# regicide211212/multi-style-transfer-gan

Hardware: AMD Instinct MI355X
Metric: train-step images/sec (fwd+bwd+loss), 256x256 batch32 (higher is better)
Workload: dtype f32; 1 GPU; config 3: reference CycleGAN train_step (2x EnhancedGenerator + 2x EnhancedDiscriminator, channels=16, num_transformer_blocks=0), 32 image pairs/GPU at 256x256, fwd+bwd+loss+Adam; per_gpu_batch=32, size=256, channels=16, parallelism=dp1, collective=none, losses_finite=True

## Files before the change

### include/mstg_hip.h

```cpp
#ifndef MSTG_HIP_H
#define MSTG_HIP_H

#include <stddef.h>
#include <stdint.h>

#ifdef __cplusplus
extern "C" {
#endif

#define MSTG_OK 0
#define MSTG_E_BADARG (-1)
#define MSTG_E_ALIGN (-2)
#define MSTG_E_LAUNCH (-3)
#define MSTG_E_WORKSPACE (-4)
#define MSTG_E_UNSUPPORTED (-5)

#define MSTG_ACT_NONE 0
#define MSTG_ACT_RELU 1
#define MSTG_ACT_LEAKY02 2
#define MSTG_ACT_TANH 3
#define MSTG_ACT_GELU 4

const char* mstg_version(void);
const char* mstg_arch(void);
const char* mstg_last_error(void);
void mstg_env_refresh(void);

int mstg_prof_enable(int on);
int mstg_prof_count(void);
int mstg_prof_get(int i, char* name, size_t name_cap, float* ms);

typedef struct mstg_conv_desc {
    int32_t N, H, W, Cin;
    int32_t Ho, Wo, Cout;
    int32_t KH, KW, stride, pad, dil;
    int32_t transposed;
    int32_t x_nchw, y_nchw;
    int32_t x_ctot, x_coff;
    int32_t y_ctot, y_coff;
    int32_t act;
    int32_t accumulate;
} mstg_conv_desc;

int mstg_conv2d_dgrad_bsums_supported(const mstg_conv_desc* d);
size_t mstg_conv2d_dgrad_bsums_workspace_bytes(const mstg_conv_desc* d);
int mstg_conv2d_dgrad_bsums(const mstg_conv_desc* d, const float* dy, const float* w, float* dx, const float* x_raw, const float* x_stats,
                            float* sums, void* workspace, size_t workspace_bytes, int workspace_packed, void* stream);

int mstg_conv2d_fwd_cached(const mstg_conv_desc* d, const float* x, const float* w, const float* bias, float* y, void* workspace,
                           size_t workspace_bytes, int workspace_packed, void* stream);
int mstg_conv2d_fwd_norm_cached(const mstg_conv_desc* d, const float* x, const float* in_stats, const float* w, const float* bias,
                                float* y, float* out_stats, void* workspace, size_t workspace_bytes, int workspace_packed, void* stream);
int mstg_conv2d_dgrad_cached(const mstg_conv_desc* d, const float* dy, const float* w, float* dx, void* workspace, size_t workspace_bytes,
                             int workspace_packed, void* stream);
int mstg_msblock_fwd_cached(const float* x, const float* w1, const float* b1, const float* w2, const float* b2, const float* w3,
                            const float* b3, const float* w4, const float* b4, float* y, int N, int H, int W, int CH, void* workspace,
                            size_t workspace_bytes, int workspace_packed, void* stream);
int mstg_msblock_dgrad_cached(const float* dy, const float* w1, const float* w2, const float* w3, const float* w4, const float* dres,
                              float* dx, int N, int H, int W, int CH, void* workspace, size_t workspace_bytes, int workspace_packed,
                              void* stream);

const char* mstg_conv2d_kernel_name(const mstg_conv_desc* d, int pass);
size_t mstg_conv2d_workspace_bytes(const mstg_conv_desc* d);
int mstg_conv2d_fwd(const mstg_conv_desc* d, const float* x, const float* w, const float* bias ,
                    float* y, void* workspace, size_t workspace_bytes, void* stream);
int mstg_conv2d_wgrad_norm_supported(const mstg_conv_desc* d);
int mstg_conv2d_wgrad_norm(const mstg_conv_desc* d, const float* x_raw, const float* in_stats, const float* dy, float* dw, float* dbias,
                           void* workspace, size_t workspace_bytes, void* stream);
int mstg_conv2d_fwd_norm_supported(const mstg_conv_desc* d);
int mstg_conv2d_fwd_stats_pays(const mstg_conv_desc* d);
size_t mstg_conv2d_fwd_norm_workspace_bytes(const mstg_conv_desc* d);
int mstg_conv2d_fwd_norm(const mstg_conv_desc* d, const float* x, const float* in_stats, const float* w, const float* bias, float* y,
                         float* out_stats, void* workspace, size_t workspace_bytes, void* stream);
int mstg_conv2d_dgrad(const mstg_conv_desc* d, const float* dy, const float* w, float* dx, void* workspace,
                      size_t workspace_bytes, void* stream);
size_t mstg_conv2d_wgrad_workspace_bytes(const mstg_conv_desc* d);
int mstg_conv2d_wgrad(const mstg_conv_desc* d, const float* x, const float* dy, float* dw, float* dbias ,
                      void* workspace, size_t workspace_bytes, void* stream);

size_t mstg_norm_workspace_bytes(int N, int HW, int C);
int mstg_norm_act_fwd(const float* x, const float* residual , float* y, float* stats ,
                      int N, int HW, int C, int act, int batch_stats, const float* gamma, const float* beta,
                      float* running_mean, float* running_var, void* workspace, size_t workspace_bytes, void* stream);
int mstg_norm_act_bwd(const float* x, const float* stats, const float* dy, float* dx, int N, int HW, int C, int act,
                      int batch_stats, const float* gamma, const float* beta, float* dgamma, float* dbeta,
                      void* workspace, size_t workspace_bytes, void* stream);
int mstg_norm_apply_fwd(const float* x, const float* stats, const float* residual , float* y, int N, int HW, int C, int act,
                        void* stream);
int mstg_norm_stats(const float* x, float* stats, int N, int HW, int C, void* workspace, size_t workspace_bytes, void* stream);
int mstg_norm_bwd_apply(const float* x, const float* stats, const float* dy, const float* sums ,
                        int sums_split, float* dx, int N, int HW, int C, int act, void* stream);

int mstg_window_attn_core_fwd(const float* qkv, float* o, int N, int H, int W, int C, void* stream);
int mstg_window_attn_core_bwd(const float* qkv, const float* d_o, float* dqkv, int N, int H, int W, int C, void* stream);

int mstg_window_attn_ws_supported(int C, int ws);
int mstg_window_attn_ws_fwd(const float* qkv, float* o, int N, int H, int W, int C, int ws, void* stream);
int mstg_window_attn_ws_bwd(const float* qkv, const float* d_o, float* dqkv, int N, int H, int W, int C, int ws, void* stream);

int mstg_window_attn_fused_supported(int C);
int mstg_window_attn_fwd(const float* x, const float* wqkv, const float* bqkv, const float* wproj, const float* bproj,
                         float* y, int N, int H, int W, int C, void* stream);
int mstg_window_attn_bwd_direct(const float* x, const float* wqkv, const float* bqkv, const float* wproj, const float* bproj, const float* dy,
                                float* dx, float* dwqkv, float* dbqkv, float* dwproj, float* dbproj, int accumulate, int N, int H, int W, int C,
                                void* workspace, size_t workspace_bytes, void* stream);
int mstg_window_attn_norm_bwd_direct(const float* x_raw, const float* in_stats, const float* wqkv, const float* bqkv, const float* wproj,
                                     const float* bproj, const float* dy, float* dz, float* dwqkv, float* dbqkv, float* dwproj,
                                     float* dbproj, int accumulate, float* norm_sums, int N, int H, int W, int C, void* workspace,
                                     size_t workspace_bytes, void* stream);
int mstg_window_attn_norm_sums_split(void);
int mstg_window_attn_norm_fwd(const float* x_raw, const float* in_stats, const float* wqkv, const float* bqkv, const float* wproj,
                              const float* bproj, float* y, int N, int H, int W, int C, void* stream);
size_t mstg_window_attn_norm_bwd_workspace_bytes(int N, int H, int W, int C);
int mstg_window_attn_norm_bwd(const float* x_raw, const float* in_stats, const float* wqkv, const float* bqkv, const float* wproj,
                              const float* bproj, const float* dy, float* dz, float* dparams, float* norm_sums, int N, int H, int W,
                              int C, void* workspace, size_t workspace_bytes, void* stream);
size_t mstg_window_attn_bwd_workspace_bytes(int N, int H, int W, int C);
int mstg_window_attn_bwd(const float* x, const float* wqkv, const float* bqkv, const float* wproj, const float* bproj,
                         const float* dy, float* dx, float* dparams, int N, int H, int W, int C, void* workspace,
                         size_t workspace_bytes, void* stream);

int mstg_act_fwd(const float* x, float* y, size_t n, int act, void* stream);
int mstg_act_bwd(const float* x_or_y, const float* dy, float* dx, size_t n, int act, void* stream);
size_t mstg_loss_workspace_bytes(size_t n);
int mstg_loss_mean_fwd(const float* a, const float* b, float bconst, size_t n, int kind, float* out, void* workspace,
                       size_t workspace_bytes, void* stream);
int mstg_loss_mean_bwd(const float* a, const float* b, float bconst, size_t n, int kind, const float* gscale, float scale,
                       float* da, float* db, void* stream);
int mstg_add(const float* a, const float* b, float* y, size_t n, void* stream);
int mstg_weighted_sum_fwd(const float* const* terms, const float* weights, int n, int nout, float* out, void* stream);
int mstg_weighted_sum_bwd(const float* g, const float* weights, int n, float* dterms, void* stream);
int mstg_masked_l1_mean_fwd(const float* a, const float* b, const float* m, size_t n, float* out, void* workspace,
                            size_t workspace_bytes, void* stream);
int mstg_masked_l1_mean_bwd(const float* a, const float* b, const float* m, size_t n, const float* gscale, float* da, void* stream);
int mstg_clip_grad_norm(float* g, size_t n, float max_norm, float* norm_out, void* workspace, size_t workspace_bytes, void* stream);
size_t mstg_channel_sum_workspace_bytes(size_t P, int C);
int mstg_channel_sum(const float* x, size_t P, int ctot, int coff, int C, float scale, float* out, void* workspace,
                     size_t workspace_bytes, void* stream);
size_t mstg_plane_sum_workspace_bytes(int N, int C, size_t HW);
int mstg_plane_sum(const float* x, int N, int C, size_t HW, float scale, float* out, void* workspace,
                   size_t workspace_bytes, void* stream);
int mstg_segment_mean_fwd(const float* x, int S, size_t P, int C, float* out, void* stream);
int mstg_segment_mean_bwd(const float* dy, int S, size_t P, int C, float* dx, void* stream);
int mstg_adam_step_flat(float* p, const float* g, float* m, float* v, size_t n, float lr, float beta1, float beta2,
                        float eps, int step, const unsigned char* mask , void* stream);

int mstg_msblock_fused_supported(int CH);
size_t mstg_msblock_fwd_workspace_bytes(int CH);
int mstg_msblock_fwd(const float* x, const float* w1, const float* b1, const float* w2, const float* b2, const float* w3,
                     const float* b3, const float* w4, const float* b4, float* y, int N, int H, int W, int CH, void* workspace,
                     size_t workspace_bytes, void* stream);
size_t mstg_msblock_dgrad_workspace_bytes(int CH);
int mstg_msblock_dgrad(const float* dy, const float* w1, const float* w2, const float* w3, const float* w4, const float* dres,
                       float* dx, int N, int H, int W, int CH, void* workspace, size_t workspace_bytes, void* stream);
size_t mstg_msblock_wgrad_workspace_bytes(int N, int H, int W, int CH);
int mstg_msblock_wgrad(const float* x, const float* dy, float* dw1, float* db1, float* dw2, float* db2, float* dw3, float* db3,
                       float* dw4, float* db4, int accumulate , int N, int H, int W,
                       int CH, void* workspace, size_t workspace_bytes, void* stream);

size_t mstg_spectral_norm_workspace_bytes(int M, int K);
int mstg_spectral_norm_fwd(const float* w, float* u, float* v, float* w_out, float* sigma, float* u_save, float* v_save, int M,
                           int K, float eps, int training, void* workspace, size_t workspace_bytes, void* stream);
int mstg_spectral_norm_bwd(const float* dwn, const float* w, const float* u, const float* v, const float* sigma, float* dw,
                           int accumulate , int M, int K, void* workspace, size_t workspace_bytes, void* stream);
int mstg_spectral_norm_group_max(void);
size_t mstg_spectral_norm_group_workspace_bytes(int count, const int* M, const int* K);
int mstg_spectral_norm_group_fwd(int count, const float* const* w, float* const* u, float* const* v, float* const* w_out, float* sigma,
                                 float* const* u_save, float* const* v_save, const int* M, const int* K, float eps, int training,
                                 void* workspace, size_t workspace_bytes, void* stream);
int mstg_spectral_norm_group_bwd(int count, const float* const* dwn, const float* const* w, const float* const* u,
                                 const float* const* v, const float* const* sigma, float* const* dw, const int* accumulate, const int* M,
                                 const int* K, void* workspace, size_t workspace_bytes, void* stream);

int mstg_maxpool2x2_fwd(const float* x, float* y, unsigned char* idx, int N, int H, int W, int C, void* stream);
int mstg_maxpool2x2_bwd(const float* dy, const unsigned char* idx, float* dx, int N, int H, int W, int C, void* stream);
size_t mstg_gram_workspace_bytes(int N, int HW, int C);
int mstg_gram_fwd(const float* f, float* g, int N, int HW, int C, float scale, void* workspace, size_t workspace_bytes,
                  void* stream);
int mstg_gram_bwd(const float* f, const float* dg, float* df, int N, int HW, int C, float scale, void* stream);

typedef struct mstg_f16_conv_desc {
    int32_t kind;
    int32_t N, H, W, Cin;
    int32_t Ho, Wo, Cout;
    int32_t K, stride, pad, dil;
    int32_t src_nchw_f32;
    int32_t dst_nchw;
    int32_t act;
} mstg_f16_conv_desc;
size_t mstg_f16_conv_plan_bytes(const mstg_f16_conv_desc* d);
int mstg_f16_conv_pack(const mstg_f16_conv_desc* d, const float* w0, const float* b0, const float* w1, const float* b1,
                       const float* w2, const float* b2, const float* w3, const float* b3, void* blob, size_t blob_bytes,
                       void* stream);
size_t mstg_f16_conv_partial_bytes(const mstg_f16_conv_desc* d);
int mstg_f16_conv_fwd(const mstg_f16_conv_desc* d, const void* blob, const void* x, const float* in_stats , void* y,
                      float* out_stats , void* workspace, size_t workspace_bytes, void* stream);
int mstg_f16_conv_fwd_res(const mstg_f16_conv_desc* d, const void* blob, const void* x, const float* in_stats,
                          const void* residual , void* y, float* out_stats , void* workspace,
                          size_t workspace_bytes, void* stream);
int mstg_f16_norm_residual(const void* x, const void* residual, const float* stats, void* y, int N, int HW, int C, void* stream);
size_t mstg_f16_attn_plan_bytes(int C);
int mstg_f16_attn_pack(const float* wqkv, const float* bqkv, const float* wproj, const float* bproj, int C, void* blob,
                       size_t blob_bytes, void* stream);
int mstg_f16_attn_fwd(const void* x, const float* in_stats , const void* blob, void* y, int N, int H, int W, int C,
                      void* stream);

typedef struct mstg_f16_plain_desc {
// ... 259 lines not shown
```

### multi-style-transfer-gan_amd/mstg_hip/_lib.py

```python
from __future__ import annotations

import ctypes as C
import os

HERE = os.path.dirname(os.path.abspath(__file__))
LIB_PATH = os.environ.get("MSTG_LIB") or os.path.join(HERE, "libmstg_hip.so")

ACT_NONE, ACT_RELU, ACT_LEAKY02, ACT_TANH, ACT_GELU = 0, 1, 2, 3, 4
LOSS_L1, LOSS_MSE = 0, 1


class ConvDesc(C.Structure):
    _fields_ = [(n, C.c_int32) for n in (
        "N", "H", "W", "Cin", "Ho", "Wo", "Cout", "KH", "KW", "stride", "pad", "dil", "transposed",
        "x_nchw", "y_nchw", "x_ctot", "x_coff", "y_ctot", "y_coff", "act", "accumulate")]


class F16ConvDesc(C.Structure):
    _fields_ = [(n, C.c_int32) for n in (
        "kind", "N", "H", "W", "Cin", "Ho", "Wo", "Cout", "K", "stride", "pad", "dil", "src_nchw_f32", "dst_nchw", "act")]


class F16PlainDesc(C.Structure):
    _fields_ = [(n, C.c_int32) for n in (
        "kind", "N", "H", "W", "Cin", "Ho", "Wo", "Cout", "K", "src_nchw_f32", "dst_nchw", "act")]


class ImgDesc(C.Structure):
    _fields_ = ([("src", C.c_void_p)] + [(n, C.c_int32) for n in (
        "src_h", "src_w", "box_y", "box_x", "box_h", "box_w", "rs_h", "rs_w", "filter", "win_y", "win_x", "win_h", "win_w",
        "dst_y", "dst_x", "fill", "ks_h", "ks_v", "y_first", "irows", "ipitch")] + [(n, C.c_int64) for n in (
            "kk_h", "bounds_h", "kk_v", "bounds_v", "inter_off", "out_off")] + [("grid", C.c_uint64)])


IMG_PASS_H, IMG_PASS_V_TENSOR, IMG_PASS_V_U8 = 0, 1, 2

_vp, _fp, _sz, _i, _f = C.c_void_p, C.c_void_p, C.c_size_t, C.c_int, C.c_float
_dp = C.POINTER(ConvDesc)
_hp = C.POINTER(F16ConvDesc)
_pp = C.POINTER(F16PlainDesc)

SIGNATURES = {
    "mstg_version": (C.c_char_p, []),
    "mstg_arch": (C.c_char_p, []),
    "mstg_last_error": (C.c_char_p, []),
    "mstg_env_refresh": (None, []),
    "mstg_prof_enable": (_i, [_i]),
    "mstg_prof_count": (_i, []),
    "mstg_prof_get": (_i, [_i, C.c_char_p, _sz, C.POINTER(C.c_float)]),
    "mstg_conv2d_kernel_name": (C.c_char_p, [_dp, _i]),
    "mstg_conv2d_workspace_bytes": (_sz, [_dp]),
    "mstg_conv2d_fwd": (_i, [_dp, _fp, _fp, _fp, _fp, _vp, _sz, _vp]),
    "mstg_conv2d_dgrad": (_i, [_dp, _fp, _fp, _fp, _vp, _sz, _vp]),
    "mstg_conv2d_dgrad_bsums_supported": (_i, [_dp]),
    "mstg_conv2d_dgrad_bsums_workspace_bytes": (_sz, [_dp]),
    "mstg_conv2d_dgrad_bsums": (_i, [_dp, _fp, _fp, _fp, _fp, _fp, _fp, _vp, _sz, _i, _vp]),
    "mstg_conv2d_fwd_cached": (_i, [_dp, _fp, _fp, _fp, _fp, _vp, _sz, _i, _vp]),
    "mstg_conv2d_fwd_norm_cached": (_i, [_dp, _fp, _fp, _fp, _fp, _fp, _fp, _vp, _sz, _i, _vp]),
    "mstg_conv2d_dgrad_cached": (_i, [_dp, _fp, _fp, _fp, _vp, _sz, _i, _vp]),
    "mstg_msblock_fwd_cached": (_i, [_fp] * 10 + [_i, _i, _i, _i, _vp, _sz, _i, _vp]),
    "mstg_msblock_dgrad_cached": (_i, [_fp] * 7 + [_i, _i, _i, _i, _vp, _sz, _i, _vp]),
    "mstg_conv2d_wgrad_workspace_bytes": (_sz, [_dp]),
    "mstg_conv2d_wgrad": (_i, [_dp, _fp, _fp, _fp, _fp, _vp, _sz, _vp]),
    "mstg_norm_workspace_bytes": (_sz, [_i, _i, _i]),
    "mstg_norm_act_fwd": (_i, [_fp, _fp, _fp, _fp, _i, _i, _i, _i, _i, _fp, _fp, _fp, _fp, _vp, _sz, _vp]),
    "mstg_norm_act_bwd": (_i, [_fp, _fp, _fp, _fp, _i, _i, _i, _i, _i, _fp, _fp, _fp, _fp, _vp, _sz, _vp]),
    "mstg_window_attn_core_fwd": (_i, [_fp, _fp, _i, _i, _i, _i, _vp]),
    "mstg_window_attn_core_bwd": (_i, [_fp, _fp, _fp, _i, _i, _i, _i, _vp]),
    "mstg_window_attn_ws_supported": (_i, [_i, _i]),
    "mstg_window_attn_ws_fwd": (_i, [_fp, _fp, _i, _i, _i, _i, _i, _vp]),
    "mstg_window_attn_ws_bwd": (_i, [_fp, _fp, _fp, _i, _i, _i, _i, _i, _vp]),
    "mstg_window_attn_fused_supported": (_i, [_i]),
    "mstg_window_attn_fwd": (_i, [_fp, _fp, _fp, _fp, _fp, _fp, _i, _i, _i, _i, _vp]),
    "mstg_window_attn_bwd_workspace_bytes": (_sz, [_i, _i, _i, _i]),
    "mstg_conv2d_wgrad_norm_supported": (_i, [_dp]),
    "mstg_conv2d_wgrad_norm": (_i, [_dp, _fp, _fp, _fp, _fp, _fp, _vp, _sz, _vp]),
    "mstg_conv2d_fwd_norm_supported": (_i, [_dp]),
    "mstg_conv2d_fwd_stats_pays": (_i, [_dp]),
    "mstg_conv2d_fwd_norm_workspace_bytes": (_sz, [_dp]),
    "mstg_conv2d_fwd_norm": (_i, [_dp, _fp, _fp, _fp, _fp, _fp, _fp, _vp, _sz, _vp]),
    "mstg_window_attn_norm_fwd": (_i, [_fp, _fp, _fp, _fp, _fp, _fp, _fp, _i, _i, _i, _i, _vp]),
    "mstg_window_attn_norm_bwd_workspace_bytes": (_sz, [_i, _i, _i, _i]),
    "mstg_window_attn_norm_bwd": (_i, [_fp, _fp, _fp, _fp, _fp, _fp, _fp, _fp, _fp, _fp, _i, _i, _i, _i, _vp, _sz, _vp]),
    "mstg_norm_apply_fwd": (_i, [_fp, _fp, _fp, _fp, _i, _i, _i, _i, _vp]),
    "mstg_norm_stats": (_i, [_fp, _fp, _i, _i, _i, _vp, _sz, _vp]),
    "mstg_norm_bwd_apply": (_i, [_fp, _fp, _fp, _fp, _i, _fp, _i, _i, _i, _i, _vp]),
    "mstg_window_attn_norm_sums_split": (_i, []),
    "mstg_window_attn_bwd_direct": (_i, [_fp] * 11 + [_i, _i, _i, _i, _i, _vp, _sz, _vp]),
    "mstg_window_attn_norm_bwd_direct": (_i, [_fp] * 12 + [_i, _fp, _i, _i, _i, _i, _vp, _sz, _vp]),
    "mstg_window_attn_bwd": (_i, [_fp, _fp, _fp, _fp, _fp, _fp, _fp, _fp, _i, _i, _i, _i, _vp, _sz, _vp]),
    "mstg_act_fwd": (_i, [_fp, _fp, _sz, _i, _vp]),
    "mstg_act_bwd": (_i, [_fp, _fp, _fp, _sz, _i, _vp]),
    "mstg_loss_workspace_bytes": (_sz, [_sz]),
    "mstg_loss_mean_fwd": (_i, [_fp, _fp, _f, _sz, _i, _fp, _vp, _sz, _vp]),
    "mstg_loss_mean_bwd": (_i, [_fp, _fp, _f, _sz, _i, _fp, _f, _fp, _fp, _vp]),
    "mstg_channel_sum_workspace_bytes": (_sz, [_sz, _i]),
    "mstg_channel_sum": (_i, [_fp, _sz, _i, _i, _i, _f, _fp, _vp, _sz, _vp]),
    "mstg_plane_sum_workspace_bytes": (_sz, [_i, _i, _sz]),
    "mstg_plane_sum": (_i, [_fp, _i, _i, _sz, _f, _fp, _vp, _sz, _vp]),
    "mstg_segment_mean_fwd": (_i, [_fp, _i, _sz, _i, _fp, _vp]),
    "mstg_segment_mean_bwd": (_i, [_fp, _i, _sz, _i, _fp, _vp]),
    "mstg_maxpool2x2_fwd": (_i, [_fp, _fp, _vp, _i, _i, _i, _i, _vp]),
    "mstg_maxpool2x2_bwd": (_i, [_fp, _vp, _fp, _i, _i, _i, _i, _vp]),
    "mstg_gram_workspace_bytes": (_sz, [_i, _i, _i]),
    "mstg_gram_fwd": (_i, [_fp, _fp, _i, _i, _i, _f, _vp, _sz, _vp]),
    "mstg_gram_bwd": (_i, [_fp, _fp, _fp, _i, _i, _i, _f, _vp]),
    "mstg_adam_step_flat": (_i, [_fp, _fp, _fp, _fp, _sz, _f, _f, _f, _f, _i, _vp, _vp]),
    "mstg_msblock_fused_supported": (_i, [_i]),
    "mstg_msblock_fwd_workspace_bytes": (_sz, [_i]),
    "mstg_msblock_fwd": (_i, [_fp] * 10 + [_i, _i, _i, _i, _vp, _sz, _vp]),
    "mstg_msblock_dgrad_workspace_bytes": (_sz, [_i]),
    "mstg_msblock_dgrad": (_i, [_fp] * 7 + [_i, _i, _i, _i, _vp, _sz, _vp]),
    "mstg_msblock_wgrad_workspace_bytes": (_sz, [_i, _i, _i, _i]),
    "mstg_msblock_wgrad": (_i, [_fp] * 10 + [_i, _i, _i, _i, _i, _vp, _sz, _vp]),
    "mstg_spectral_norm_workspace_bytes": (_sz, [_i, _i]),
    "mstg_spectral_norm_fwd": (_i, [_fp] * 7 + [_i, _i, _f, _i, _vp, _sz, _vp]),
    "mstg_spectral_norm_bwd": (_i, [_fp, _fp, _fp, _fp, _fp, _fp, _i, _i, _i, _vp, _sz, _vp]),
    "mstg_spectral_norm_group_max": (_i, []),
    "mstg_spectral_norm_group_workspace_bytes": (_sz, [_i, _vp, _vp]),
    "mstg_spectral_norm_group_fwd": (_i, [_i, _vp, _vp, _vp, _vp, _fp, _vp, _vp, _vp, _vp, _f, _i, _vp, _sz, _vp]),
    "mstg_spectral_norm_group_bwd": (_i, [_i, _vp, _vp, _vp, _vp, _vp, _vp, _vp, _vp, _vp, _vp, _sz, _vp]),
    "mstg_f16_conv_plan_bytes": (_sz, [_hp]),
    "mstg_f16_conv_pack": (_i, [_hp] + [_fp] * 8 + [_vp, _sz, _vp]),
    "mstg_f16_conv_partial_bytes": (_sz, [_hp]),
    "mstg_f16_conv_fwd": (_i, [_hp, _vp, _vp, _fp, _vp, _fp, _vp, _sz, _vp]),
    "mstg_f16_conv_fwd_res": (_i, [_hp, _vp, _vp, _fp, _vp, _vp, _fp, _vp, _sz, _vp]),
    "mstg_f16_norm_residual": (_i, [_vp, _vp, _fp, _vp, _i, _i, _i, _vp]),
    "mstg_f16_attn_plan_bytes": (_sz, [_i]),
    "mstg_f16_attn_pack": (_i, [_fp, _fp, _fp, _fp, _i, _vp, _sz, _vp]),
    "mstg_f16_attn_fwd": (_i, [_vp, _fp, _vp, _vp, _i, _i, _i, _i, _vp]),
    "mstg_f16_plain_plan_bytes": (_sz, [_pp]),
    "mstg_f16_plain_pack": (_i, [_pp, _fp, _fp, _fp, _vp, _sz, _vp]),
    "mstg_f16_plain_fwd": (_i, [_pp, _vp, _vp, _vp, _vp]),
    "mstg_f16_train_image_nhwc8": (_i, [_fp, _vp, _i, _i, _i, _vp]),
    "mstg_f16_train_bn_workspace_bytes": (_sz, [_sz, _i]),
    "mstg_f16_train_bn_fwd": (_i, [_vp, _fp, _fp, _sz, _i, _i, _f, _f, _fp, _fp, _fp, _fp, _vp, _vp, _sz, _vp]),
    "mstg_f16_train_bn_bwd": (_i, [_vp, _vp, _fp, _fp, _fp, _fp, _sz, _i, _i, _fp, _fp, _fp, _vp, _vp, _sz, _vp]),
    "mstg_f16_train_act_bwd": (_i, [_vp, _vp, _vp, _sz, _i, _vp]),
    "mstg_f16_train_loss_workspace_bytes": (_sz, [_i, _i, _i]),
    "mstg_f16_train_head_loss_bwd": (_i, [_vp, _fp, _fp, _i, _i, _i, _fp, _fp, _vp, _vp, _sz, _vp]),
    "mstg_f16_train_wgrad_workspace_bytes": (_sz, [_i, _i, _i, _i, _i, _i]),
    "mstg_f16_train_wgrad": (_i, [_vp, _vp, _i, _i, _i, _i, _i, _i, _fp, _fp, _vp, _sz, _vp]),
    "mstg_f16_train_bias_grad": (_i, [_vp, _sz, _i, _i, _fp, _fp, _vp, _sz, _vp]),
    "mstg_f16_train_scale_update": (_i, [_fp, _fp, _vp, _vp]),
    "mstg_f16_train_adam": (_i, [_fp, _fp, _fp, _fp, _sz, _f, _f, _f, _f, _i, _vp, _vp]),
    "mstg_f16_linear_plan_bytes": (_sz, [_i, _i]),
    "mstg_f16_linear_pack": (_i, [_fp, _fp, _i, _i, _vp, _sz, _vp]),
    "mstg_f16_linear_fwd": (_i, [_vp, _vp, _fp, _vp, _i, _i, _i, _i, _i, _i, _vp]),
    "mstg_f16_ln_mod_fwd": (_i, [_vp, _i, _fp, _fp, _fp, _fp, _fp, _fp, _fp, _vp, _i, _i, _i, _f, _vp]),
    "mstg_f16_token_mean_workspace_bytes": (_sz, [_i, _i, _i]),
    "mstg_f16_token_mean": (_i, [_vp, _fp, _i, _i, _i, _vp, _sz, _vp]),
    "mstg_f16_flash_attn_fwd": (_i, [_vp, _vp, _i, _i, _i, _i, _vp]),
    "mstg_add": (_i, [_fp, _fp, _fp, _sz, _vp]),
    "mstg_weighted_sum_fwd": (_i, [C.POINTER(C.c_void_p), C.POINTER(C.c_float), _i, _i, _fp, _vp]),
    "mstg_weighted_sum_bwd": (_i, [_fp, C.POINTER(C.c_float), _i, _fp, _vp]),
    "mstg_masked_l1_mean_fwd": (_i, [_fp, _fp, _fp, _sz, _fp, _vp, _sz, _vp]),
    "mstg_masked_l1_mean_bwd": (_i, [_fp, _fp, _fp, _sz, _fp, _fp, _vp]),
    "mstg_clip_grad_norm": (_i, [_fp, _sz, _f, _fp, _vp, _sz, _vp]),
    "mstg_structure_map": (_i, [_fp, _fp, _i, _i, _i, _vp]),
    "mstg_ln_mod_fwd": (_i, [_fp] * 7 + [_i, _i, _i, _f, _vp]),
    "mstg_ln_mod_bwd_workspace_bytes": (_sz, [_i, _i, _i]),
    "mstg_ln_mod_bwd": (_i, [_fp] * 11 + [_i, _i, _i, _i, _vp, _sz, _vp]),
    "mstg_flash_attn_fwd": (_i, [_fp, _fp, _fp, _i, _i, _i, _i, _vp]),
    "mstg_flash_attn_bwd": (_i, [_fp, _fp, _fp, _fp, _fp, _fp, _i, _i, _i, _i, _vp]),
    "mstg_resample_ksize": (_i, [_i, _i, _i]),
    "mstg_resample_coeffs": (_i, [_i, _i, _i, _vp, _vp]),
    "mstg_resample_h_u8": (_i, [_vp, _vp, _i, _i, _i, _i, _i, _vp, _vp, _vp]),
    "mstg_resample_v_u8": (_i, [_vp, _vp, _i, _i, _i, _vp, _vp, _vp]),
    "mstg_paste_u8": (_i, [_vp, _i, _i, _i, _i, _i, _i, _vp, _i, _i, _i, _i, _i, _vp]),
    "mstg_u8_to_tensor": (_i, [_vp, _i, _i, _i, _i, _i, _i, _fp, _fp, _fp, C.c_ulonglong, _i, _vp]),
    "mstg_tensor_to_u8": (_i, [_fp, _i, _i, _vp, _vp]),
    "mstg_blend_u8": (_i, [_vp, _vp, C.c_double, C.c_double, _vp, _vp, _i, _i, _vp]),
    "mstg_img_batch_validate": (_i, [_vp, _i, _vp, _sz, _sz, _i, _sz]),
    "mstg_img_batch_tiles": (_i, [_vp, _i, _vp, _sz, _i, _i, _vp, _sz]),
    "mstg_img_batch_resample_h": (_i, [_vp, _i, _vp, _sz, _vp, _vp, _i, _vp, _vp, _sz, _vp]),
    "mstg_img_batch_resample_v_tensor": (_i, [_vp, _i, _vp, _sz, _vp, _vp, _i, _vp, _vp, _sz, _i, _fp, _fp, _fp, _vp, _i, _vp]),
    "mstg_img_batch_resample_v_u8": (_i, [_vp, _i, _vp, _sz, _vp, _vp, _i, _vp, _vp, _sz, _vp, _sz, _vp]),
    "mstg_img_batch_tensor_to_u8": (_i, [_vp, _i, _i, _i, _i, _vp, _vp]),
    "mstg_image_metrics_workspace_bytes": (_sz, [_i, _i, _i]),
    "mstg_image_metrics_u8": (_i, [_vp, _vp, _i, _i, _i, _vp, _vp, _sz, _vp]),
    "mstg_local_style_workspace_bytes": (_sz, [_i, _i, _i]),
    "mstg_local_style_prepare": (_i, [_vp, _i, _i, _i, _vp, _vp, _vp, _vp, _vp]),
    "mstg_local_style_hysteresis": (_i, [_vp, _i, _i, _i, _vp, _vp]),
    "mstg_local_style_weights": (_i, [_vp, _vp, _vp, _i, _i, _i, C.c_double, C.c_double, C.c_double, _vp, _vp, _vp]),
    "mstg_local_style_weight_map": (_i, [_vp, _i, _i, _i, C.c_double, C.c_double, C.c_double, _vp, _vp, _sz, _vp]),
    "mstg_local_style_finish": (_i, [_vp, _vp, _vp, _vp, _i, _i, _i, _i, _i, _vp, _vp]),
    "mstg_local_style_enhanced_workspace_bytes": (_sz, [_i, _i, _i]),
    "mstg_local_style_enhanced": (_i, [_vp, _vp, _i, _i, _i, C.c_double, C.c_double, C.c_double, _i, _i, _vp, _vp, _sz, _vp]),
    "mstg_bilateral_tables": (_i, [_i, C.c_double, C.c_double, _vp]),
    "mstg_standard_color_lut": (_i, [_i, _vp]),
    "mstg_median3_u8": (_i, [_vp, _i, _i, _i, _vp, _vp]),
    "mstg_bilateral_u8": (_i, [_vp, _i, _i, _i, _i, _vp, _vp, _vp]),
    "mstg_lut_u8": (_i, [_vp, _i, _i, _i, _vp, _vp, _vp]),
    "mstg_gaussian_u8": (_i, [_vp, _i, _i, _i, _i, _vp, _vp]),
    "mstg_standard_finish_workspace_bytes": (_sz, [_i, _i, _i]),
    "mstg_standard_finish": (_i, [_vp, _vp, _i, _i, _i, C.c_double, C.c_double, _i, _i, _vp, _vp, _i, _vp, _vp, _sz, _vp]),
    "mstg_gaussian_kernel_f64": (_i, [_i, C.c_double, _vp]),
    "mstg_app_sky_mask": (_i, [_vp, _i, _i, _i, _vp, _vp]),
    "mstg_app_edge_weight": (_i, [_vp, _i, _i, _i, _vp, C.c_double, _vp, _vp]),
    "mstg_app_chain": (_i, [_vp, _vp, _i, _i, _i, _vp, _vp, _i, C.c_double, C.c_double, _vp, _vp, _vp]),
    "mstg_app_local_style_workspace_bytes": (_sz, [_i, _i, _i]),
    "mstg_app_local_style_finish": (_i, [_vp, _vp, _i, _i, _i, _i, _i, _i, _i, C.c_double, C.c_double, C.c_double, _vp, _vp, _vp, _vp, _vp,
                                         _sz, _vp]),
    "mstg_lab_tables": (_i, [_vp]),
    "mstg_bilateral_wide_tables": (_i, [_i, C.c_double, C.c_double, _vp]),
    "mstg_color_block_mask": (_i, [_vp, _i, _i, _i, _vp, _f, _i, _vp, _vp, _sz, _vp]),
    "mstg_color_correct_u8": (_i, [_vp, _vp, _i, _i, _i, _i, _vp, _vp, _sz, _vp]),
    "mstg_bilateral_wide_u8": (_i, [_vp, _i, _i, _i, _i, _vp, _vp, _vp]),
    "mstg_detail_blend_u8": (_i, [_vp, _vp, _i, _i, _i, _vp, _i, C.c_double, C.c_double, C.c_double, _vp, _vp, _sz, _vp]),
    "mstg_color_block_fix_workspace_bytes": (_sz, [_i, _i, _i, _i]),
    "mstg_color_block_fix": (_i, [_vp, _vp, _i, _i, _i, _vp, _f, _i, _i, _i, _vp, _vp, _i, C.c_double, C.c_double, C.c_double, _vp, _vp,
                                  _sz, _vp]),
# ... 78 lines not shown
```

### multi-style-transfer-gan_amd/mstg_hip/csrc/conv_igemm.hip

```cpp
#include "common.h"
#include "igemm_args.h"
#include <stdlib.h>

namespace mstg {


constexpr int TILE_H = 8, TILE_W = 16;

#ifdef MSTG_STAMPS
__device__ unsigned long long g_dbg_stamps[64 * 8];
#define MSTG_STAMP(k)                                                                                      \
    if (threadIdx.x == 0 && (blockIdx.x % 11) == 0 && blockIdx.x / 11 < 64 && blockIdx.y == 0 && blockIdx.z == 0) \
        g_dbg_stamps[(blockIdx.x / 11) * 8 + (k)] = __builtin_amdgcn_s_memtime();
#else
#define MSTG_STAMP(k)
#endif
constexpr int W_BUDGET_FLOATS = 6144;

template <int V> struct Frag;
template <> struct Frag<1> { typedef float T; };
template <> struct Frag<2> { typedef f32x2 T; };
template <> struct Frag<4> { typedef f32x4 T; };
template <int V> __device__ __forceinline__ float frag_get(const typename Frag<V>::T& f, int j);
template <> __device__ __forceinline__ float frag_get<1>(const float& f, int) { return f; }
template <> __device__ __forceinline__ float frag_get<2>(const f32x2& f, int j) { return f[j]; }
template <> __device__ __forceinline__ float frag_get<4>(const f32x4& f, int j) { return f[j]; }

template <int V> __host__ __device__ constexpr int ckp_of() { return V == 4 ? 20 : (V == 2 ? 12 : 4); }
template <int V> __host__ __device__ constexpr int ckp_heavy_of() { return V == 4 ? 24 : ckp_of<V>(); }

__global__ void pack_filter_kernel(const IGemmArgs a, float* __restrict__ wp, int CK, int CoP, int nchunks, int ncls) {
    const int total = ncls * nchunks * a.ntaps * CoP * CK;
    for (int idx = blockIdx.x * blockDim.x + threadIdx.x; idx < total; idx += gridDim.x * blockDim.x) {
        const int ci = idx % CK;
        int rest = idx / CK;
        const int co = rest % CoP; rest /= CoP;
        const int t = rest % a.ntaps; rest /= a.ntaps;
        const int chunk = rest % nchunks, cls = rest / nchunks;
        int widx, oc = co;
        bool ok = true;
        if (a.phase) {
            const int pa = cls >> 1, pb = cls & 1, u = t >> 1, v = t & 1;
            widx = ((1 - pa) + 2 * u) * 4 + ((1 - pb) + 2 * v);
        } else if (a.dpack) {
            const int delta = co >> 2, kx = 4 * (t % a.tapsx) + 3 - delta, real = (t / a.tapsx) * a.KW + kx;
            oc = co & 3;
            ok = co < 16 && kx >= 0 && kx < a.KW;
            widx = a.flip ? (a.KH * a.KW - 1 - real) : real;
        } else {
            widx = a.flip ? (a.ntaps - 1 - t) : t;
        }
        const int cr = chunk * CK + ci;
        wp[idx] = (ok && oc < a.Co && cr < a.Cr) ? a.w[(size_t)oc * a.w_so + (size_t)cr * a.w_sr + widx] : 0.f;
    }
}

__device__ __forceinline__ int tap_patch_offset(const IGemmArgs& a, int t, int pa, int pb, int ckp) {
    int pro, pco;
    if (a.phase) {
        pro = 1 + pa - (t >> 1);
        pco = 1 + pb - (t & 1);
    } else if (a.dpack) {
        pro = t / a.tapsx;
        pco = 4 * (t % a.tapsx) + 3;
    } else {
        pro = (t / a.KW) * a.dil;
        pco = (t % a.KW) * a.dil;
    }
    return (pro * a.PW + pco) * ckp;
}

template <int NFW, int PF = 2>
__device__ __forceinline__ void igemm_epilogue(const IGemmArgs& a, const f32x4 (&acc)[NFW][PF], int n, int ty0, int tx0, int co0, int pa,
                                               int pb, int wave, int i, int g) {
#pragma unroll
    for (int pf = 0; pf < PF; ++pf) {
        const int gy = ty0 * (4 * PF) + PF * wave + pf, gx = tx0 * TILE_W + i;
        if (gy >= a.Gh || gx >= a.Gw) continue;
        const int oy = a.phase ? 2 * gy + pa : gy, ox = a.phase ? 2 * gx + pb : gx;
#pragma unroll
        for (int wf = 0; wf < NFW; ++wf) {
            const int co = co0 + 16 * wf + 4 * g;
            if (co >= a.Co) continue;
            f32x4 v = acc[wf][pf];
            if (!a.y_nchw && co + 3 < a.Co && ((a.y_ctot | a.y_coff) & 3) == 0) {
                float* p = a.y + (((size_t)n * a.Ho + oy) * a.Wo + ox) * a.y_ctot + a.y_coff + co;
                if (a.bias) v += *reinterpret_cast<const f32x4*>(a.bias + co);
                if (a.accumulate) v += *reinterpret_cast<const f32x4*>(p);
                if (a.act != MSTG_ACT_NONE) {
#pragma unroll
                    for (int e = 0; e < 4; ++e) v[e] = apply_act(v[e], a.act);
                }
                *reinterpret_cast<f32x4*>(p) = v;
            } else {
#pragma unroll
                for (int e = 0; e < 4; ++e) {
                    if (co + e >= a.Co) continue;
                    float* p = a.y_nchw ? a.y + (((size_t)n * a.y_ctot + a.y_coff + co + e) * a.Ho + oy) * a.Wo + ox
                                        : a.y + (((size_t)n * a.Ho + oy) * a.Wo + ox) * a.y_ctot + a.y_coff + co + e;
                    float val = v[e] + (a.bias ? a.bias[co + e] : 0.f);
                    if (a.accumulate) val += *p;
                    *p = apply_act(val, a.act);
                }
            }
        }
    }
}

template <int V, int NFW, int PF>
__global__ __launch_bounds__(256) void igemm_light_kernel(const IGemmArgs a, const float* __restrict__ wp, const int CoP) {
    constexpr int CK = 4 * V, CKP = ckp_of<V>(), BN = 16 * NFW, TH = 4 * PF;
    typedef typename Frag<V>::T frag_t;
    extern __shared__ __attribute__((aligned(16))) float smem[];
    float* patch = smem;
    float* wl = smem + ((a.PH * a.PW * CKP + 3) & ~3);
    int* tapo = reinterpret_cast<int*>(wl + (a.wglob ? 0 : a.TG * BN * CKP));

    const int tid = threadIdx.x, lane = tid & 63, wave = tid >> 6, i = lane & 15, g = lane >> 4;
    const int tile = xcd_swizzle(blockIdx.x, gridDim.x);
    const int tx0 = tile % a.tiles_x, ty0 = (tile / a.tiles_x) % a.tiles_y, n = tile / (a.tiles_x * a.tiles_y);
    const int co0 = blockIdx.y * BN;
    const int cls = blockIdx.z, pa = cls >> 1, pb = cls & 1;
    const int s = a.phase ? 1 : a.stride;
    const int y0 = a.phase ? ty0 * TH - 1 : ty0 * TH * s - a.pad;
    const int x0 = a.phase ? tx0 * TILE_W - 1 : (a.dpack ? tx0 * 13 - 3 - a.pad : tx0 * TILE_W * s - a.pad);
    const int nchunks = (a.Cr + CK - 1) / CK;
    const unsigned m_pw = magic_u32(a.PW);
    MSTG_STAMP(0)
    if (tid < a.ntaps) tapo[tid] = tap_patch_offset(a, tid, pa, pb, CKP);

    f32x4 acc[NFW][PF];
#pragma unroll
    for (int wf = 0; wf < NFW; ++wf)
#pragma unroll
        for (int pf = 0; pf < PF; ++pf) acc[wf][pf] = f32x4{0.f, 0.f, 0.f, 0.f};

    for (int chunk = 0; chunk < nchunks; ++chunk) {
        if (chunk) __syncthreads();
        if (a.x_nchw) {
            stage_window_c4(a.x + ((size_t)n * a.x_ctot + a.x_coff) * a.H * a.W, patch, a.PH, a.PW, m_pw, y0, x0, a.H, a.W, (unsigned)a.W, 1u,
                            (unsigned)(a.H * a.W), a.Cr, tid);
        } else if (((a.x_ctot | a.x_coff | a.Cr) & 3) == 0) {
            stage_window(a.x + (size_t)n * a.H * a.W * a.x_ctot + a.x_coff + chunk * CK, patch, a.PH, a.PW, V, m_pw, 0xFFFFFFFFu / V + 1u, y0,
                         x0, a.H, a.W, a.x_ctot, min(V, (a.Cr - chunk * CK) >> 2), CKP, tid);
        } else {
            for (int pr = wave; pr < a.PH; pr += 4) {
                const int iy = y0 + pr;
                for (int e = lane; e < a.PW * V; e += 64) {
                    const int pc = e / V, q = e % V;
                    const int ix = x0 + pc;
                    const bool inb = (unsigned)iy < (unsigned)a.H && (unsigned)ix < (unsigned)a.W;
                    f32x4 v = {0.f, 0.f, 0.f, 0.f};
                    const int c0 = chunk * CK + 4 * q;
                    if (inb && c0 < a.Cr) {
                        const float* src = a.x + (((size_t)n * a.H + iy) * a.W + ix) * a.x_ctot + a.x_coff + c0;
#pragma unroll
                        for (int c = 0; c < 4; ++c)
                            if (c0 + c < a.Cr) v[c] = src[c];
                    }
                    *reinterpret_cast<f32x4*>(&patch[(pr * a.PW + pc) * CKP + 4 * q]) = v;
                }
            }
        }
        MSTG_STAMP(1)
        if (a.wglob) {
            __syncthreads();
            const float* wb = wp + ((size_t)((cls * nchunks + chunk) * a.ntaps) * CoP + co0 + i) * CK + V * g;
            const int wts = CoP * CK;
            const int bbase0 = ((PF * wave) * s * a.PW + i * s) * CKP + V * g, bstep = s * a.PW * CKP;
            frag_t a0[NFW], a1[NFW], a2[NFW], bf[PF], bfn[PF];
#pragma unroll
            for (int wf = 0; wf < NFW; ++wf) {
                a0[wf] = *reinterpret_cast<const frag_t*>(wb + 16 * wf * CK);
                a1[wf] = *reinterpret_cast<const frag_t*>(wb + min(1, a.ntaps - 1) * wts + 16 * wf * CK);
            }
            {
                const int po = tapo[0];
#pragma unroll
                for (int pf = 0; pf < PF; ++pf) bf[pf] = *reinterpret_cast<const frag_t*>(&patch[bbase0 + pf * bstep + po]);
            }
            for (int tl = 0; tl < a.ntaps; ++tl) {
                const int t2 = min(tl + 2, a.ntaps - 1), t1 = min(tl + 1, a.ntaps - 1);
#pragma unroll
                for (int wf = 0; wf < NFW; ++wf) a2[wf] = *reinterpret_cast<const frag_t*>(wb + t2 * wts + 16 * wf * CK);
                const int po = tapo[t1];
#pragma unroll
                for (int pf = 0; pf < PF; ++pf) bfn[pf] = *reinterpret_cast<const frag_t*>(&patch[bbase0 + pf * bstep + po]);
#pragma unroll
                for (int j = 0; j < V; ++j)
#pragma unroll
                    for (int wf = 0; wf < NFW; ++wf)
#pragma unroll
                        for (int pf = 0; pf < PF; ++pf)
                            acc[wf][pf] = mfma16(frag_get<V>(a0[wf], j), frag_get<V>(bf[pf], j), acc[wf][pf]);
#pragma unroll
                for (int wf = 0; wf < NFW; ++wf) { a0[wf] = a1[wf]; a1[wf] = a2[wf]; }
#pragma unroll
                for (int pf = 0; pf < PF; ++pf) bf[pf] = bfn[pf];
            }
            continue;
        }
        for (int t0 = 0; t0 < a.ntaps; t0 += a.TG) {
            __syncthreads();
            MSTG_STAMP(2)
            const int tn = min(a.TG, a.ntaps - t0);
            const float* base = wp + ((size_t)((cls * nchunks + chunk) * a.ntaps + t0) * CoP + co0) * CK;
            for (int e0 = 0; e0 < tn * BN * V; e0 += 1024) {
                f32x4 wv[4];
#pragma unroll
                for (int k = 0; k < 4; ++k) {
                    const int e = min(e0 + 256 * k + tid, tn * BN * V - 1);
                    const int row = e / V, q = e % V, tl = row / BN, col = row % BN;
                    wv[k] = *reinterpret_cast<const f32x4*>(base + (unsigned)((tl * CoP + col) * CK + 4 * q));
                }
#pragma unroll
                for (int k = 0; k < 4; ++k) {
                    const int e = e0 + 256 * k + tid;
                    if (e < tn * BN * V) *reinterpret_cast<f32x4*>(&wl[(e / V) * CKP + 4 * (e % V)]) = wv[k];
                }
            }
            MSTG_STAMP(3)
            __syncthreads();
            MSTG_STAMP(4)
            const int bbase0 = ((PF * wave) * s * a.PW + i * s) * CKP + V * g, bstep = s * a.PW * CKP;
            frag_t af[NFW], bf[PF], afn[NFW], bfn[PF];
            {
                const int po = tapo[t0];
#pragma unroll
                for (int wf = 0; wf < NFW; ++wf) af[wf] = *reinterpret_cast<const frag_t*>(&wl[(16 * wf + i) * CKP + V * g]);
#pragma unroll
                for (int pf = 0; pf < PF; ++pf) bf[pf] = *reinterpret_cast<const frag_t*>(&patch[bbase0 + pf * bstep + po]);
            }
            for (int tl = 0; tl < ((a.dbg & 1) ? 1 : tn); ++tl) {
                const int tnx = min(tl + 1, tn - 1);
                const int po = tapo[t0 + tnx];
#pragma unroll
                for (int wf = 0; wf < NFW; ++wf) afn[wf] = *reinterpret_cast<const frag_t*>(&wl[(tnx * BN + 16 * wf + i) * CKP + V * g]);
#pragma unroll
                for (int pf = 0; pf < PF; ++pf) bfn[pf] = *reinterpret_cast<const frag_t*>(&patch[bbase0 + pf * bstep + po]);
#pragma unroll
                for (int j = 0; j < V; ++j)
#pragma unroll
                    for (int wf = 0; wf < NFW; ++wf)
#pragma unroll
                        for (int pf = 0; pf < PF; ++pf)
                            acc[wf][pf] = mfma16(frag_get<V>(af[wf], j), frag_get<V>(bf[pf], j), acc[wf][pf]);
#pragma unroll
                for (int wf = 0; wf < NFW; ++wf) af[wf] = afn[wf];
#pragma unroll
                for (int pf = 0; pf < PF; ++pf) bf[pf] = bfn[pf];
            }
        }
    }
    MSTG_STAMP(5)
    if (!a.dpack) {
        igemm_epilogue<NFW, PF>(a, acc, n, ty0, tx0, co0, pa, pb, wave, i, g);
        MSTG_STAMP(6)
        return;
    }
    __syncthreads();
    float* comb = smem + wave * (256 * PF);
#pragma unroll
    for (int pf = 0; pf < PF; ++pf) *reinterpret_cast<f32x4*>(&comb[((pf * 4 + g) * 16 + i) * 4]) = acc[0][pf];
    __syncthreads();
    if (g < PF && i < 13) {
        const int pf = g;
        f32x4 v = {0.f, 0.f, 0.f, 0.f};
#pragma unroll
        for (int d = 0; d < 4; ++d) v += *reinterpret_cast<const f32x4*>(&comb[((pf * 4 + d) * 16 + i + 3 - d) * 4]);
        const int oy = ty0 * TH + PF * wave + pf, ox = tx0 * 13 + i;
        if (oy < a.Gh && ox < a.Gw) {
            if (!a.y_nchw && a.Co == 4 && ((a.y_ctot | a.y_coff) & 3) == 0) {
                float* p = a.y + (((size_t)n * a.Ho + oy) * a.Wo + ox) * a.y_ctot + a.y_coff;
                if (a.bias) v += *reinterpret_cast<const f32x4*>(a.bias);
                if (a.accumulate) v += *reinterpret_cast<const f32x4*>(p);
#pragma unroll
                for (int e = 0; e < 4; ++e) v[e] = apply_act(v[e], a.act);
                *reinterpret_cast<f32x4*>(p) = v;
            } else {
#pragma unroll
                for (int e = 0; e < 4; ++e) {
                    if (e >= a.Co) continue;
                    float* p = a.y_nchw ? a.y + (((size_t)n * a.y_ctot + a.y_coff + e) * a.Ho + oy) * a.Wo + ox
                                        : a.y + (((size_t)n * a.Ho + oy) * a.Wo + ox) * a.y_ctot + a.y_coff + e;
                    float val = v[e] + (a.bias ? a.bias[e] : 0.f);
                    if (a.accumulate) val += *p;
                    *p = apply_act(val, a.act);
                }
            }
        }
    }
    MSTG_STAMP(6)
}

constexpr int SNB = 8;

template <int V, int NFW, int PF, int SRC>
__global__ __launch_bounds__(256) void igemm_stream_kernel(const IGemmArgs a, const float* __restrict__ wp, const int CoP) {
    constexpr int CK = 4 * V, CKP = ckp_of<V>(), BN = 16 * NFW, TH = 4 * PF;
    typedef typename Frag<V>::T frag_t;
    extern __shared__ __attribute__((aligned(16))) float smem[];
    const int nchunks = (a.Cr + CK - 1) / CK;
    const int wsz = nchunks * a.ntaps * BN * CKP;
    float* patch = smem;
    float* wl = smem + a.psz;
    int* tapo = reinterpret_cast<int*>(wl + wsz);

    const int tid = threadIdx.x, lane = tid & 63, wave = tid >> 6, i = lane & 15, g = lane >> 4;
    const int co0 = blockIdx.y * BN;
    const int cls = blockIdx.z, pa = cls >> 1, pb = cls & 1;
    const int s = a.phase ? 1 : a.stride;
    const int ntiles = a.N * a.tiles_x * a.tiles_y;
    const int my_tiles = ((int)blockIdx.x < ntiles) ? (ntiles - 1 - (int)blockIdx.x) / (int)gridDim.x + 1 : 0;
    const int total = my_tiles * nchunks;
    if (total == 0) return;

    if (tid < a.ntaps) tapo[tid] = tap_patch_offset(a, tid, pa, pb, CKP);
    {
        const int nrow = nchunks * a.ntaps * BN;
        const float* base = wp + (size_t)cls * nchunks * a.ntaps * CoP * CK + (size_t)co0 * CK;
        for (int e0 = 0; e0 < nrow * V; e0 += 1024) {
            f32x4 wv[4];
#pragma unroll
            for (int k = 0; k < 4; ++k) {
                const int e = min(e0 + 256 * k + tid, nrow * V - 1);
                const int row = e / V, q = e % V, ct = row / BN, col = row % BN;
                wv[k] = *reinterpret_cast<const f32x4*>(base + (unsigned)((ct * CoP + col) * CK + 4 * q));
            }
#pragma unroll
            for (int k = 0; k < 4; ++k) {
                const int e = e0 + 256 * k + tid;
                if (e < nrow * V) *reinterpret_cast<f32x4*>(&wl[(e / V) * CKP + 4 * (e % V)]) = wv[k];
            }
        }
    }
    const int npatch = a.PH * a.PW * V;
    const unsigned m_pw = magic_u32(a.PW);
    int p_lds[SNB], p_rc[SNB];
    unsigned p_off[SNB], used = 0;
#pragma unroll
    for (int j = 0; j < SNB; ++j) {
        const int e = tid + 256 * j;
        const int pp = e / V, q = e % V;
        const int r = (int)__umulhi((unsigned)pp, m_pw), c = pp - r * a.PW;
        const bool u = e < npatch;
        p_lds[j] = u ? pp * CKP + 4 * q : -1;
        p_rc[j] = r | (c << 8) | (q << 16);
        p_off[j] = !u ? 0u : (SRC == 2 ? (unsigned)(r * a.W + c) : (unsigned)(r * a.W + c) * (unsigned)a.x_ctot + 4u * q);
        used |= u ? (1u << j) : 0u;
    }
    const unsigned plane = (unsigned)(a.H * a.W);
    f32x4 breg[NFW];
    unsigned cok = 0;
#pragma unroll
    for (int wf = 0; wf < NFW; ++wf) {
        const int co = a.dpack ? 0 : co0 + 16 * wf + 4 * g;
#pragma unroll
        for (int e = 0; e < 4; ++e) breg[wf][e] = (a.bias && co + e < a.Co) ? a.bias[co + e] : 0.f;
        cok |= (co + 3 < a.Co) ? (1u << wf) : 0u;
    }
    const bool yvec = !a.y_nchw && ((a.y_ctot | a.y_coff) & 3) == 0;
    const int yrs = a.phase ? 2 * a.Wo : a.Wo, ycs = a.phase ? 2 : 1;
    const unsigned y_lane = (unsigned)((PF * wave) * yrs + i * ycs) * (unsigned)a.y_ctot + 4u * g;

    auto tile_of = [&](int seq, int& tx0, int& ty0, int& n) {
        const int tile = xcd_swizzle((int)blockIdx.x + seq * (int)gridDim.x, ntiles);
        tx0 = tile % a.tiles_x;
        ty0 = (tile / a.tiles_x) % a.tiles_y;
        n = tile / (a.tiles_x * a.tiles_y);
    };
    f32x4 preg[SNB];
    unsigned pmask = 0;
    auto load_stage = [&](int seq, int chunk) {
        int tx0, ty0, n;
        tile_of(seq, tx0, ty0, n);
        const int y0 = a.phase ? ty0 * TH - 1 : ty0 * TH * s - a.pad;
        const int x0 = a.phase ? tx0 * TILE_W - 1 : (a.dpack ? tx0 * 13 - 3 - a.pad : tx0 * TILE_W * s - a.pad);
        pmask = 0;
        const bool interior = y0 >= 0 && x0 >= 0 && y0 + a.PH <= a.H && x0 + a.PW <= a.W;
        if (interior && SRC == 2) {
            const float* base = a.x + ((size_t)n * a.x_ctot + a.x_coff) * plane + (unsigned)(y0 * a.W + x0);
            pmask = used;
#pragma unroll
            for (int j = 0; j < SNB; ++j) {
#pragma unroll
                for (int ch = 0; ch < 4; ++ch) preg[j][ch] = base[p_off[j] + (ch < a.Cr ? ch * plane : 0u)];
            }
        } else if (interior && SRC == 0 && (a.Cr - chunk * CK) >= CK) {
            const float* base = a.x + ((size_t)n * plane + (unsigned)(y0 * a.W + x0)) * a.x_ctot + a.x_coff + chunk * CK;
            pmask = used;
#pragma unroll
            for (int j = 0; j < SNB; ++j) preg[j] = *reinterpret_cast<const f32x4*>(base + p_off[j]);
        } else if (SRC == 2) {
            const float* img = a.x + ((size_t)n * a.x_ctot + a.x_coff) * plane;
#pragma unroll
            for (int j = 0; j < SNB; ++j) {
                const int iy = y0 + (p_rc[j] & 255), ix = x0 + ((p_rc[j] >> 8) & 255);
                const bool ok = p_lds[j] >= 0 && (unsigned)iy < (unsigned)a.H && (unsigned)ix < (unsigned)a.W;
                const unsigned off = ok ? (unsigned)(iy * a.W + ix) : 0u;
                pmask |= ok ? (1u << j) : 0u;
#pragma unroll
                for (int ch = 0; ch < 4; ++ch) preg[j][ch] = img[off + (ch < a.Cr ? ch * plane : 0u)];
            }
        } else {
            const float* img = a.x + (size_t)n * plane * a.x_ctot + a.x_coff + chunk * CK;
            const int nqv = min(V, (a.Cr - chunk * CK) >> 2);
#pragma unroll
            for (int j = 0; j < SNB; ++j) {
                const int iy = y0 + (p_rc[j] & 255), ix = x0 + ((p_rc[j] >> 8) & 255), q = p_rc[j] >> 16;
                const bool ok = p_lds[j] >= 0 && (unsigned)iy < (unsigned)a.H && (unsigned)ix < (unsigned)a.W && q < nqv;
                const unsigned off = ok ? (unsigned)(iy * a.W + ix) * (unsigned)a.x_ctot + 4u * q : 0u;
                pmask |= ok ? (1u << j) : 0u;
                preg[j] = *reinterpret_cast<const f32x4*>(img + off);
            }
        }
    };
    auto store_stage = [&]() {
#pragma unroll
        for (int j = 0; j < SNB; ++j) {
            if (p_lds[j] >= 0) {
                f32x4 v = preg[j];
                if (!((pmask >> j) & 1u)) v = f32x4{0.f, 0.f, 0.f, 0.f};
// ... 417 lines not shown
    }
    if (p.heavy) {
        p.TG = a.TG = tgh;
        p.CKP = ckp_heavy;
        p.lds = lds_heavy;
    } else {
        p.stream = 0;
        {
            const char* e = env_get(ENV_STREAM);
            const bool allow = (e && e[0] == '1') && (p.src == 0 || (p.src == 2 && p.V == 1));
            const size_t wsz = (size_t)p.nchunks * a.ntaps * p.BN * p.CKP;
            const int ny = p.CoP / p.BN;
            const char* epf = env_get(ENV_PF);
            const int force = epf ? atoi(epf) : 0;
            for (int th = 16; allow && th >= 8 && !p.stream; th -= 8) {
                if ((th == 16 && force == 2) || (th == 8 && force == 4)) continue;
                if (a.Gh < th) continue;
                igemm_geometry(a, th);
                const int pf = th / 4;
                size_t psz = (size_t)((a.PH * a.PW * p.CKP + 3) & ~3);
                if (a.dpack && psz < (size_t)1024 * pf) psz = (size_t)1024 * pf;
                const size_t lds = (psz + wsz + 64) * sizeof(float);
                const long ntiles = (long)a.N * a.tiles_x * a.tiles_y;
                int per_cu = (int)((160 * 1024) / lds);
                if (per_cu > 6) per_cu = 6;
                if (a.PH * a.PW * p.V > SNB * 256 || a.PH > 255 || a.PW > 255 || wsz * sizeof(float) > 28 * 1024 || per_cu < 3) continue;
                int gx = (256 * per_cu) / (ny * p.ncls);
                gx = gx < 8 ? 8 : (gx & ~7);
                if (ntiles < 3L * gx && !(e && e[1] == 'f')) continue;
                p.stream = 1; p.pf = pf; p.gx = gx; a.psz = (int)psz; p.lds = lds;
            }
            if (!p.stream) igemm_geometry(a, TILE_H);
        }
        if (p.stream) return MSTG_OK;
        {
            const char* e = env_get(ENV_PF);
            const int force = e ? atoi(e) : 0;
            const int ph16 = a.phase ? 18 : (a.dpack ? 15 + a.KH : 15 * a.stride + (a.KH - 1) * a.dil + 1);
            const char* ew = env_get(ENV_WGLOB);
            const int wg16 = ew ? atoi(ew) : (p.V == 4 ? 1 : 0);
            const size_t lds16 = ((size_t)((ph16 * a.PW * p.CKP + 3) & ~3) + (wg16 ? 0 : (size_t)tg * p.BN * p.CKP) + 64) * sizeof(float);
            const long blocks16 = (long)a.N * a.tiles_x * cdiv(a.Gh, 16) * (p.CoP / p.BN) * p.ncls;
            if (force == 4 || (force != 2 && lds16 <= 52 * 1024 && blocks16 >= 1024 && a.Gh >= 16)) {
                p.pf = 4;
                igemm_geometry(a, 16);
            }
        }
        const size_t patch_floats_l = (size_t)((a.PH * a.PW * p.CKP + 3) & ~3);
        p.TG = a.TG = tg;
        {
            const char* e = env_get(ENV_WGLOB);
            a.wglob = e ? atoi(e) : (p.V == 4 ? 1 : 0);
        }
        p.lds = (patch_floats_l + (a.wglob ? 0 : (size_t)tg * p.BN * p.CKP) + 64) * sizeof(float);
        if (a.dpack && p.lds < (size_t)4 * 256 * p.pf * sizeof(float)) p.lds = (size_t)4 * 256 * p.pf * sizeof(float);
        if (p.lds > 160 * 1024) return fail_arg(MSTG_E_UNSUPPORTED, "conv: LDS patch too large for this geometry");
    }
    return MSTG_OK;
}

static int launch_pack(IGemmArgs& a, const IGemmPlan& p, float* wp, hipStream_t st) {
    const int npack = p.ncls * p.nchunks * a.ntaps * p.CoP * p.CK;
    const int nb = cdiv(npack, 256) > 256 ? 256 : cdiv(npack, 256);
    MSTG_PACK_LAUNCH(pack_filter_kernel, dim3(nb), dim3(256), 0, st, a, wp, p.CK, p.CoP, p.nchunks, p.ncls);
    MSTG_CHECK_LAUNCH("pack_filter_kernel");
    return MSTG_OK;
}

template <int V, int NFW, int PF>
static int launch_light_t(IGemmArgs& a, const IGemmPlan& p, float* wp, hipStream_t st) {
    static bool attr_set = false;
    if (!attr_set) {
        hipError_t e = hipFuncSetAttribute(reinterpret_cast<const void*>(&igemm_light_kernel<V, NFW, PF>),
                                           hipFuncAttributeMaxDynamicSharedMemorySize, 160 * 1024);
        if (e != hipSuccess) return fail_launch(e, "hipFuncSetAttribute(igemm_light)");
        attr_set = true;
    }
    dim3 grid(a.N * a.tiles_x * a.tiles_y, p.CoP / p.BN, p.ncls);
    MSTG_LAUNCH((igemm_light_kernel<V, NFW, PF>), grid, dim3(256), p.lds, st, a, (const float*)wp, p.CoP);
    MSTG_CHECK_LAUNCH("igemm_light_kernel");
    return MSTG_OK;
}

template <int V, int NFW, int PF, int SRC>
static int launch_stream_t(IGemmArgs& a, const IGemmPlan& p, float* wp, hipStream_t st) {
    static bool attr_set = false;
    if (!attr_set) {
        hipError_t e = hipFuncSetAttribute(reinterpret_cast<const void*>(&igemm_stream_kernel<V, NFW, PF, SRC>),
                                           hipFuncAttributeMaxDynamicSharedMemorySize, 160 * 1024);
        if (e != hipSuccess) return fail_launch(e, "hipFuncSetAttribute(igemm_stream)");
        attr_set = true;
    }
    dim3 grid(p.gx, p.CoP / p.BN, p.ncls);
    MSTG_LAUNCH((igemm_stream_kernel<V, NFW, PF, SRC>), grid, dim3(256), p.lds, st, a, (const float*)wp, p.CoP);
    MSTG_CHECK_LAUNCH("igemm_stream_kernel");
    return MSTG_OK;
}

template <int V, int NFW, int SRC>
static int launch_heavy_t(IGemmArgs& a, const IGemmPlan& p, float* wp, hipStream_t st) {
    static bool attr_set = false;
    if (!attr_set) {
        hipError_t e = hipFuncSetAttribute(reinterpret_cast<const void*>(&igemm_heavy_kernel<V, NFW, SRC>),
                                           hipFuncAttributeMaxDynamicSharedMemorySize, 160 * 1024);
        if (e != hipSuccess) return fail_launch(e, "hipFuncSetAttribute(igemm_heavy)");
        attr_set = true;
    }
    const int ntiles = a.N * a.tiles_x * a.tiles_y, ny = p.CoP / p.BN, nz = p.ncls;
    int per_cu = p.lds <= 80 * 1024 ? 2 : 1;
    { const char* e = env_get(ENV_HEAVY_PER_CU); if (e) per_cu = atoi(e); }
    int gx = (256 * per_cu) / (ny * nz);
    gx = gx < 8 ? 8 : (gx & ~7);
    if (gx > ntiles) gx = ntiles;
    dim3 grid(gx, ny, nz);
    MSTG_LAUNCH((igemm_heavy_kernel<V, NFW, SRC>), grid, dim3(256), p.lds, st, a, (const float*)wp, p.CoP);
    MSTG_CHECK_LAUNCH("igemm_heavy_kernel");
    return MSTG_OK;
}

enum IGemmKind {
    IG_NONE,
    IG_IMG_DGRAD,
    IG_P32,
    IG_IGEMM
};
struct IGemmRoute {
    IGemmKind kind;
    int rc;
    P32Route p32;
    IGemmPlan plan;
    size_t ws_bytes;
};

static IGemmRoute route_igemm(IGemmArgs& a) {
    IGemmRoute r;
    r.p32 = p32_route(a);
    r.rc = plan_igemm(a, r.plan);
    r.ws_bytes = r.rc ? 0 : (r.plan.ws_bytes > r.p32.pack_bytes ? r.plan.ws_bytes : r.p32.pack_bytes);
    r.kind = img_dgrad_eligible(a) ? IG_IMG_DGRAD : (r.p32.kind != P32_NONE ? IG_P32 : (r.rc ? IG_NONE : IG_IGEMM));
    return r;
}

int launch_igemm(IGemmArgs& a, void* workspace, size_t workspace_bytes, hipStream_t st) {
    IGemmRoute r = route_igemm(a);
    if (r.kind == IG_IMG_DGRAD) return launch_img_dgrad(a, st);
    if (r.kind == IG_P32) return launch_p32(a, r.p32, nullptr, nullptr, nullptr, nullptr, workspace, workspace_bytes, st);
    if (r.kind == IG_NONE) return r.rc;
    a.dbg = 0;
    IGemmPlan& p = r.plan;
    { const char* e = env_get(ENV_DBG); if (e) a.dbg = atoi(e); }
    { const char* e = env_get(ENV_DBG_LDS_KB); if (e && !p.heavy) p.lds += (size_t)atoi(e) * 1024; }
    if (!workspace || workspace_bytes < p.ws_bytes) return fail_arg(MSTG_E_WORKSPACE, "conv: workspace too small for the packed filter");
    float* wp = (float*)workspace;
    if (int rc = launch_pack(a, p, wp, st)) return rc;
#define MSTG_DISPATCH(VV, NN)                                                              \
    if (p.V == VV && p.nfw == NN) {                                                        \
        if (p.stream && p.src == 0 && p.pf == 4) return launch_stream_t<VV, NN, 4, 0>(a, p, wp, st); \
        if (p.stream && p.src == 0) return launch_stream_t<VV, NN, 2, 0>(a, p, wp, st);   \
        if (VV == 1 && p.stream && p.src == 2 && p.pf == 4) return launch_stream_t<1, NN, 4, 2>(a, p, wp, st); \
        if (VV == 1 && p.stream && p.src == 2) return launch_stream_t<1, NN, 2, 2>(a, p, wp, st); \
        if (!p.heavy && p.pf == 4) return launch_light_t<VV, NN, 4>(a, p, wp, st);          \
        if (!p.heavy) return launch_light_t<VV, NN, 2>(a, p, wp, st);                      \
        if (p.src == 0) return launch_heavy_t<VV, NN, 0>(a, p, wp, st);                    \
        if (p.src == 1) return launch_heavy_t<VV, NN, 1>(a, p, wp, st);                    \
        if (VV == 1 && p.src == 2) return launch_heavy_t<1, NN, 2>(a, p, wp, st);          \
    }
    MSTG_DISPATCH(1, 1) MSTG_DISPATCH(1, 2) MSTG_DISPATCH(1, 4)
    MSTG_DISPATCH(2, 1) MSTG_DISPATCH(2, 2) MSTG_DISPATCH(2, 4)
    MSTG_DISPATCH(4, 1) MSTG_DISPATCH(4, 2) MSTG_DISPATCH(4, 4)
#undef MSTG_DISPATCH
    return fail_arg(MSTG_E_UNSUPPORTED, "conv: no kernel variant");
}

int check_desc(const mstg_conv_desc* d) {
    if (!d) return fail_arg(MSTG_E_BADARG, "conv: null descriptor");
    if (d->N <= 0 || d->H <= 0 || d->W <= 0 || d->Cin <= 0 || d->Cout <= 0 || d->KH <= 0 || d->KW <= 0 || d->stride <= 0 ||
        d->dil <= 0 || d->pad < 0)
        return fail_arg(MSTG_E_BADARG, "conv: non-positive dimension");
    if (d->transposed) {
        if (d->KH != 4 || d->KW != 4 || d->stride != 2 || d->pad != 1 || d->dil != 1)
            return fail_arg(MSTG_E_UNSUPPORTED, "conv_transpose: only k4 s2 p1 is implemented");
        if (d->Ho != 2 * d->H || d->Wo != 2 * d->W) return fail_arg(MSTG_E_BADARG, "conv_transpose: Ho,Wo must be 2H,2W");
    } else {
        const int ho = (d->H + 2 * d->pad - d->dil * (d->KH - 1) - 1) / d->stride + 1;
        const int wo = (d->W + 2 * d->pad - d->dil * (d->KW - 1) - 1) / d->stride + 1;
        if (ho != d->Ho || wo != d->Wo) return fail_arg(MSTG_E_BADARG, "conv: Ho,Wo inconsistent with H,W,k,s,p,d");
        if (d->stride != 1 && !(d->stride == 2 && d->KH == 4 && d->KW == 4 && d->pad == 1 && d->dil == 1 && d->H % 2 == 0 &&
                                d->W % 2 == 0))
            return fail_arg(MSTG_E_UNSUPPORTED, "conv: strided convolution only as k4 s2 p1 on even H,W");
    }
    if (d->x_ctot < d->x_coff + d->Cin || d->y_ctot < d->y_coff + d->Cout) return fail_arg(MSTG_E_BADARG, "conv: channel slice out of range");
    if ((uint64_t)d->H * d->W * d->x_ctot >= (1ull << 30) || (uint64_t)d->Ho * d->Wo * d->y_ctot >= (1ull << 30))
        return fail_arg(MSTG_E_UNSUPPORTED, "conv: one image must stay below 2^30 elements");
    return MSTG_OK;
}

}

using namespace mstg;

void fill_fwd_args(const mstg_conv_desc* d, IGemmArgs& a) {
    const int T = d->KH * d->KW;
    a.N = d->N;
    a.H = d->H; a.W = d->W; a.x_ctot = d->x_ctot; a.x_coff = d->x_coff; a.x_nchw = d->x_nchw; a.Cr = d->Cin;
    a.Ho = d->Ho; a.Wo = d->Wo; a.y_ctot = d->y_ctot; a.y_coff = d->y_coff; a.y_nchw = d->y_nchw; a.Co = d->Cout;
    a.KH = d->KH; a.KW = d->KW; a.stride = d->stride; a.pad = d->pad; a.dil = d->dil; a.flip = 0;
    a.act = d->act; a.accumulate = d->accumulate;
    if (d->transposed) {
        a.phase = 1; a.Gh = d->H; a.Gw = d->W;
        a.w_so = T; a.w_sr = d->Cout * T;
    } else {
        a.phase = 0; a.Gh = d->Ho; a.Gw = d->Wo;
        a.w_so = d->Cin * T; a.w_sr = T;
    }
}

int fill_dgrad_args(const mstg_conv_desc* d, IGemmArgs& a) {
    const int T = d->KH * d->KW;
    a.N = d->N;
    a.H = d->Ho; a.W = d->Wo; a.x_ctot = d->y_ctot; a.x_coff = d->y_coff; a.x_nchw = d->y_nchw; a.Cr = d->Cout;
    a.Ho = d->H; a.Wo = d->W; a.y_ctot = d->x_ctot; a.y_coff = d->x_coff; a.y_nchw = d->x_nchw; a.Co = d->Cin;
    a.KH = d->KH; a.KW = d->KW; a.dil = d->dil;
    a.act = MSTG_ACT_NONE; a.accumulate = d->accumulate;
    if (d->transposed) {
        a.phase = 0; a.Gh = d->H; a.Gw = d->W; a.stride = 2; a.pad = 1; a.flip = 0;
        a.w_so = d->Cout * T; a.w_sr = T;
    } else if (d->stride == 1) {
        a.phase = 0; a.Gh = d->H; a.Gw = d->W; a.stride = 1; a.pad = d->dil * (d->KH - 1) - d->pad; a.flip = 1;
        if (d->KH != d->KW) return fail_arg(MSTG_E_UNSUPPORTED, "conv_dgrad: square kernels only");
        if (a.pad < 0) return fail_arg(MSTG_E_UNSUPPORTED, "conv_dgrad: pad larger than dil*(k-1)");
        a.w_so = T; a.w_sr = d->Cin * T;
    } else {
        a.phase = 1; a.Gh = d->Ho; a.Gw = d->Wo; a.stride = 2; a.pad = 1; a.flip = 0;
        a.w_so = T; a.w_sr = d->Cin * T;
    }
    return MSTG_OK;
}

namespace {
struct PackedScope {
    explicit PackedScope(int packed) { mstg::t_ws_packed = packed != 0; }
    ~PackedScope() { mstg::t_ws_packed = false; }
};
}

extern "C" size_t mstg_conv2d_workspace_bytes(const mstg_conv_desc* d) {
    if (check_desc(d)) return 0;
    IGemmArgs f{}, b{};
    fill_fwd_args(d, f);
    if (fill_dgrad_args(d, b)) return 0;
    const size_t wf = route_igemm(f).ws_bytes, wb = route_igemm(b).ws_bytes;
    return wf > wb ? wf : wb;
}

extern "C" int mstg_conv2d_fwd(const mstg_conv_desc* d, const float* x, const float* w, const float* bias, float* y,
                               void* workspace, size_t workspace_bytes, void* stream) {
    if (int rc = check_desc(d)) return rc;
    if (!x || !w || !y) return fail_arg(MSTG_E_BADARG, "conv_fwd: null pointer");
    IGemmArgs a{};
    fill_fwd_args(d, a);
    a.x = x; a.y = y; a.w = w; a.bias = bias;
    return launch_igemm(a, workspace, workspace_bytes, (hipStream_t)stream);
}

static P32Route fwd_norm_route(const mstg_conv_desc* d, IGemmArgs& a) {
    if (check_desc(d)) return P32Route{};
    fill_fwd_args(d, a);
    const IGemmRoute r = route_igemm(a);
    return r.kind == IG_P32 && r.p32.kind == P32_GENERIC ? r.p32 : P32Route{};
}

extern "C" int mstg_conv2d_fwd_norm_supported(const mstg_conv_desc* d) {
    IGemmArgs a{};
    return fwd_norm_route(d, a).kind == P32_GENERIC ? 1 : 0;
}

extern "C" int mstg_conv2d_fwd_stats_pays(const mstg_conv_desc* d) {
    IGemmArgs a{};
    const P32Route r = fwd_norm_route(d, a);
    const char* e = env_get(ENV_BSUMS_ALL);
    return r.kind == P32_GENERIC && ((e && e[0] == '1') || r.stats_pays()) ? 1 : 0;
}

extern "C" size_t mstg_conv2d_fwd_norm_workspace_bytes(const mstg_conv_desc* d) {
    IGemmArgs a{};
    return fwd_norm_route(d, a).stats_bytes;
}

extern "C" int mstg_conv2d_fwd_norm(const mstg_conv_desc* d, const float* x, const float* in_stats, const float* w, const float* bias,
                                    float* y, float* out_stats, void* workspace, size_t workspace_bytes, void* stream) {
    if (int rc = check_desc(d)) return rc;
    if (!x || !w || !y) return fail_arg(MSTG_E_BADARG, "conv_fwd_norm: null pointer");
    IGemmArgs a{};
    const P32Route r = fwd_norm_route(d, a);
    a.x = x; a.y = y; a.w = w; a.bias = bias;
    if (r.kind != P32_GENERIC) return fail_arg(MSTG_E_UNSUPPORTED, "conv_fwd_norm: only the layers mstg_conv2d_fwd_norm_supported() reports");
    return launch_p32(a, r, in_stats, out_stats, nullptr, nullptr, workspace, workspace_bytes, (hipStream_t)stream);
}

extern "C" int mstg_conv2d_dgrad(const mstg_conv_desc* d, const float* dy, const float* w, float* dx, void* workspace,
                                 size_t workspace_bytes, void* stream) {
    if (int rc = check_desc(d)) return rc;
    if (!dy || !w || !dx) return fail_arg(MSTG_E_BADARG, "conv_dgrad: null pointer");
    IGemmArgs a{};
    if (int rc = fill_dgrad_args(d, a)) return rc;
    a.x = dy; a.y = dx; a.w = w; a.bias = nullptr;
    return launch_igemm(a, workspace, workspace_bytes, (hipStream_t)stream);
}

static P32Route dgrad_bsums_route(const mstg_conv_desc* d, IGemmArgs& a) {
    if (check_desc(d) || fill_dgrad_args(d, a)) return P32Route{};
    const IGemmRoute r = route_igemm(a);
    if (!(r.kind == IG_P32 && r.p32.kind == P32_GENERIC && !d->accumulate && d->x_ctot == d->Cin && d->x_coff == 0)) return P32Route{};
    const char* e = env_get(ENV_BSUMS_ALL);
    return (e && e[0] == '1') || r.p32.bsums_pays() ? r.p32 : P32Route{};
}

extern "C" int mstg_conv2d_dgrad_bsums_supported(const mstg_conv_desc* d) {
    IGemmArgs a{};
    return dgrad_bsums_route(d, a).kind == P32_GENERIC ? 1 : 0;
}

extern "C" size_t mstg_conv2d_dgrad_bsums_workspace_bytes(const mstg_conv_desc* d) {
    IGemmArgs a{};
    return dgrad_bsums_route(d, a).stats_bytes;
}

extern "C" int mstg_conv2d_dgrad_bsums(const mstg_conv_desc* d, const float* dy, const float* w, float* dx, const float* x_raw,
                                       const float* x_stats, float* sums, void* workspace, size_t workspace_bytes, int workspace_packed,
                                       void* stream) {
    if (int rc = check_desc(d)) return rc;
    if (!dy || !w || !dx || !x_raw || !x_stats || !sums) return fail_arg(MSTG_E_BADARG, "conv_dgrad_bsums: null pointer");
    IGemmArgs a{};
    const P32Route r = dgrad_bsums_route(d, a);
    if (r.kind != P32_GENERIC) return fail_arg(MSTG_E_UNSUPPORTED, "conv_dgrad_bsums: only the layers mstg_conv2d_dgrad_bsums_supported() reports");
    a.x = dy; a.y = dx; a.w = w; a.bias = nullptr;
    PackedScope scope(workspace_packed);
    return launch_p32(a, r, nullptr, sums, x_raw, x_stats, workspace, workspace_bytes, (hipStream_t)stream);
}

extern "C" int mstg_conv2d_fwd_cached(const mstg_conv_desc* d, const float* x, const float* w, const float* bias, float* y, void* workspace,
                                      size_t workspace_bytes, int workspace_packed, void* stream) {
    PackedScope scope(workspace_packed);
    return mstg_conv2d_fwd(d, x, w, bias, y, workspace, workspace_bytes, stream);
}
extern "C" int mstg_conv2d_fwd_norm_cached(const mstg_conv_desc* d, const float* x, const float* in_stats, const float* w, const float* bias,
                                           float* y, float* out_stats, void* workspace, size_t workspace_bytes, int workspace_packed,
                                           void* stream) {
    PackedScope scope(workspace_packed);
    return mstg_conv2d_fwd_norm(d, x, in_stats, w, bias, y, out_stats, workspace, workspace_bytes, stream);
}
extern "C" int mstg_conv2d_dgrad_cached(const mstg_conv_desc* d, const float* dy, const float* w, float* dx, void* workspace,
                                        size_t workspace_bytes, int workspace_packed, void* stream) {
    PackedScope scope(workspace_packed);
    return mstg_conv2d_dgrad(d, dy, w, dx, workspace, workspace_bytes, stream);
}

const char* igemm_kernel_name(const mstg_conv_desc* d, int pass) {
    static thread_local char name[64];
    IGemmArgs a{};
    if (check_desc(d)) return "";
    if (pass == 0) fill_fwd_args(d, a);
    else if (fill_dgrad_args(d, a)) return "";
    const IGemmRoute r = route_igemm(a);
    const IGemmPlan& p = r.plan;
    if (r.kind == IG_NONE) return "";
    if (r.kind == IG_P32) return p32_kernel_name(r.p32);
    if (r.kind == IG_IMG_DGRAD) snprintf(name, sizeof(name), "conv_img_dgrad_kernel<%d>", a.Co);
    else if (p.stream) snprintf(name, sizeof(name), "igemm_stream_kernel<%d, %d, %d, %d>", p.V, p.nfw, p.pf, p.src);
    else if (p.heavy) snprintf(name, sizeof(name), "igemm_heavy_kernel<%d, %d, %d>", p.V, p.nfw, p.src);
    else snprintf(name, sizeof(name), "igemm_light_kernel<%d, %d, %d>", p.V, p.nfw, p.pf);
    return name;
}

#ifdef MSTG_STAMPS
extern "C" int mstg_debug_stamps(unsigned long long* out) {
    return (int)hipMemcpyFromSymbol(out, HIP_SYMBOL(mstg::g_dbg_stamps), sizeof(unsigned long long) * 64 * 8);
}
#endif
```

### multi-style-transfer-gan_amd/mstg_hip/csrc/conv_img.hip

```cpp
#include "common.h"
#include "igemm_args.h"

namespace mstg {

constexpr int IMG_T = 16;

template <int CI>
__global__ __launch_bounds__(256) void conv_img_dgrad_kernel(const float* __restrict__ dy, const float* __restrict__ w, float* __restrict__ dx,
                                                             int N, int Ho, int Wo, int Cr, int x_ctot, int x_coff, int w_so, int w_sr) {
    extern __shared__ __attribute__((aligned(16))) float wl[];
    const int tid = threadIdx.x;
    for (int e = tid; e < IMG_T * CI * Cr; e += 256) {
        const int cr = e % Cr, r = e / Cr, ci = r % CI, t = r / CI;
        wl[e] = w[(size_t)cr * w_sr + (size_t)ci * w_so + t];
    }
    __syncthreads();
    const long total = (long)N * Ho * Wo;
    const int H = 2 * Ho, W = 2 * Wo;
    const size_t plane = (size_t)H * W;
    for (long idx = (long)blockIdx.x * 256 + tid; idx < total; idx += (long)gridDim.x * 256) {
        const int qx = (int)(idx % Wo), qy = (int)((idx / Wo) % Ho), n = (int)(idx / ((long)Wo * Ho));
        float acc[2][2][CI];
#pragma unroll
        for (int a = 0; a < 2; ++a)
#pragma unroll
            for (int b = 0; b < 2; ++b)
#pragma unroll
                for (int ci = 0; ci < CI; ++ci) acc[a][b][ci] = 0.f;
#pragma unroll
        for (int dr = 0; dr < 3; ++dr) {
            const int oy = qy + dr - 1;
#pragma unroll
            for (int dc = 0; dc < 3; ++dc) {
                const int ox = qx + dc - 1;
                const bool ok = (unsigned)oy < (unsigned)Ho && (unsigned)ox < (unsigned)Wo;
                if (!ok) continue;
                const float* src = dy + (((size_t)n * Ho + oy) * Wo + ox) * x_ctot + x_coff;
                for (int c4 = 0; c4 < Cr; c4 += 4) {
                    const f32x4 v = *reinterpret_cast<const f32x4*>(src + c4);
#pragma unroll
                    for (int a = 0; a < 2; ++a) {
                        const int ky = a == 0 ? (dr == 0 ? 3 : (dr == 1 ? 1 : -1)) : (dr == 1 ? 2 : (dr == 2 ? 0 : -1));
                        if (ky < 0) continue;
#pragma unroll
                        for (int b = 0; b < 2; ++b) {
                            const int kx = b == 0 ? (dc == 0 ? 3 : (dc == 1 ? 1 : -1)) : (dc == 1 ? 2 : (dc == 2 ? 0 : -1));
                            if (kx < 0) continue;
#pragma unroll
                            for (int ci = 0; ci < CI; ++ci) {
                                const f32x4 wv = *reinterpret_cast<const f32x4*>(&wl[((4 * ky + kx) * CI + ci) * Cr + c4]);
                                acc[a][b][ci] += (v[0] * wv[0] + v[1] * wv[1]) + (v[2] * wv[2] + v[3] * wv[3]);
                            }
                        }
                    }
                }
            }
        }
        float* img = dx + (size_t)n * CI * plane + (size_t)(2 * qy) * W + 2 * qx;
#pragma unroll
        for (int ci = 0; ci < CI; ++ci)
#pragma unroll
            for (int a = 0; a < 2; ++a) {
                float2 o;
                o.x = acc[a][0][ci];
                o.y = acc[a][1][ci];
                *reinterpret_cast<float2*>(img + ci * plane + (size_t)a * W) = o;
            }
    }
}

static bool img_on() {
    const char* e = env_get(ENV_CONV_IMG);
    return !(e && e[0] == '0');
}

static bool img_k4s2(const IGemmArgs& a) {
    return a.KH == 4 && a.KW == 4 && a.stride == 2 && a.pad == 1 && a.dil == 1 && !a.flip && !a.accumulate;
}

bool img_dgrad_eligible(const IGemmArgs& a) {
    return img_on() && img_k4s2(a) && a.phase && !a.x_nchw && a.y_nchw && a.Co >= 1 && a.Co <= 3 && a.y_coff == 0 && a.y_ctot == a.Co &&
           a.Cr % 4 == 0 && a.Cr <= 64 && (a.x_coff & 3) == 0 && (a.x_ctot & 3) == 0 && a.act == MSTG_ACT_NONE && !a.bias &&
           a.Ho == 2 * a.H && a.Wo == 2 * a.W && (a.Wo & 1) == 0;
}

static unsigned img_grid(long total) {
    long g = (total + 255) / 256;
    const long cap = 256L * 16;
    return (unsigned)(g > cap ? cap : (g < 1 ? 1 : g));
}

int launch_img_dgrad(const IGemmArgs& a, hipStream_t st) {
    const long total = (long)a.N * a.H * a.W;
    const size_t lds = (size_t)IMG_T * a.Co * a.Cr * sizeof(float);
#define MSTG_IMG_DGRAD(CI_)                                                                                                   \
    MSTG_LAUNCH(conv_img_dgrad_kernel<CI_>, dim3(img_grid(total)), dim3(256), lds, st, a.x, a.w, a.y, a.N, a.H, a.W, a.Cr, a.x_ctot, \
                a.x_coff, a.w_so, a.w_sr)
    if (a.Co == 3) MSTG_IMG_DGRAD(3);
    else if (a.Co == 2) MSTG_IMG_DGRAD(2);
    else MSTG_IMG_DGRAD(1);
#undef MSTG_IMG_DGRAD
    MSTG_CHECK_LAUNCH("conv_img_dgrad_kernel");
    return MSTG_OK;
}

}
```

### multi-style-transfer-gan_amd/mstg_hip/csrc/conv_p32.hip

```cpp
#include <stdlib.h>

#include "igemm_args.h"
#include "lanes.h"

namespace mstg {

struct P32True { static constexpr bool value = true; };
struct P32False { static constexpr bool value = false; };

constexpr int P32_TW = 16;
constexpr int P32_TABLE_BYTES = P32_MAX_STEPS * 4 + P32_MAX_SEG * 16;

struct P32Args {
    const float* x;
    float* y;
    const float* wpk;
    const float* bias;
    const float* in_stats;
    float* partial;
    const float* aux;
    const float* aux_stats;
    int N, H, W, Cin, Ho, Wo, Cout, Gh, Gw, tiles_x, tiles_y, dbg;
};

__global__ void p32_pack_kernel(const P32Plan p, const float* __restrict__ w, const float* __restrict__ bias, int w_so, int w_sr,
                                int Cout, int Cin, float* __restrict__ wpk, float* __restrict__ bpk) {
    const int total = p.nsteps * p.NF * 64 * 4;
    for (int e = blockIdx.x * blockDim.x + threadIdx.x; e < total; e += gridDim.x * blockDim.x) {
        const int j = e & 3, lane = (e >> 2) & 63, sf = e >> 8, f = sf % p.NF, s = sf / p.NF;
        const int co = 16 * f + (lane & 15), ci = p.tcb[s] + 4 * (lane >> 4) + j;
        float v = 0.f;
        if (co < Cout && ci < Cin) v = w[(size_t)co * w_so + (size_t)ci * w_sr + p.tky[s] * p.KW + p.tkx[s]];
        wpk[e] = v;
    }
    for (int c = blockIdx.x * blockDim.x + threadIdx.x; c < 16 * p.NF; c += gridDim.x * blockDim.x) bpk[c] = (bias && c < Cout) ? bias[c] : 0.f;
}

template <int NPF>
struct P32Regs {
    f32x4 v[NPF];
    unsigned okmask;
};

__device__ __forceinline__ int p32_tile(int it, int b, int G) { return it * G + (b & 7) * (G >> 3) + (b >> 3); }

template <int NPF>
__device__ __forceinline__ void p32_fetch(const P32Args& a, const P32Plan& p, int t, int TH, int tid, const unsigned (&rel)[NPF],
                                          unsigned vmask, P32Regs<NPF>& R) {
    const int ntile = a.tiles_x * a.tiles_y;
    const int n = ntile == 1 ? t : (int)__umulhi((unsigned)t, p.m_ntile), tt = t - n * ntile;
    const int ty = a.tiles_x == 1 ? tt : (int)__umulhi((unsigned)tt, p.m_tx), tx = tt - ty * a.tiles_x;
    const int sy0 = ty * TH * p.stride + p.oy0, sx0 = tx * P32_TW * p.stride + p.ox0;
    const bool interior = sy0 >= 0 && sx0 >= 0 && sy0 + p.PH <= a.H && sx0 + p.PW <= a.W;
    const char* img = reinterpret_cast<const char*>(a.x) + (size_t)n * a.H * a.W * a.Cin * 4;
    if (interior) {
        const char* org = img + ((size_t)sy0 * a.W + sx0) * a.Cin * 4;
        R.okmask = vmask;
#pragma unroll
        for (int k = 0; k < NPF; ++k) R.v[k] = *reinterpret_cast<const f32x4*>(org + (((vmask >> k) & 1) ? rel[k] : 0u));
    } else {
        R.okmask = 0;
        const long org = ((long)sy0 * a.W + sx0) * a.Cin * 4;
        const int quads = a.Cin >> 2, sh = quads == 4 ? 2 : (quads == 8 ? 3 : 4);
#pragma unroll
        for (int k = 0; k < NPF; ++k) {
            const int pix = (256 * k + tid) >> sh;
            const int r = (int)__umulhi((unsigned)pix, p.m_pw), c = pix - r * p.PW;
            const int iy = sy0 + r, ix = sx0 + c;
            const bool ok = ((vmask >> k) & 1) && (unsigned)iy < (unsigned)a.H && (unsigned)ix < (unsigned)a.W;
            R.okmask |= (unsigned)ok << k;
            R.v[k] = *reinterpret_cast<const f32x4*>(img + (ok ? org + (long)rel[k] : 0L));
        }
    }
}

template <int RPW, int NF, int NPF, bool WLDS, int STATS>
__global__ __launch_bounds__(256) void conv_p32_kernel(const P32Args a, const P32Plan p) {
    extern __shared__ __attribute__((aligned(16))) unsigned char smem[];
    constexpr int TH = 4 * RPW;
    const int tid = threadIdx.x, lane = tid & 63, wv = tid >> 6, nl = lane & 15, g = lane >> 4;
    const int ntile = a.tiles_x * a.tiles_y, total_tiles = a.N * ntile, G = gridDim.x;
    unsigned char* wl = smem + P32_TABLE_BYTES;
    unsigned char* patch = wl + (WLDS ? (size_t)p.nsteps * NF * 1024 : 0);
    if (tid < P32_MAX_STEPS) {
        reinterpret_cast<unsigned*>(smem)[tid] = p.koff[tid];
    } else if (tid < P32_MAX_STEPS + P32_MAX_SEG) {
        const int c = tid - P32_MAX_STEPS;
        int* e = reinterpret_cast<int*>(smem + 4 * P32_MAX_STEPS + 16 * c);
        e[0] = p.seg[c].s0; e[1] = p.seg[c].s1; e[2] = p.seg[c].oy; e[3] = p.seg[c].ox;
    }
    if (WLDS) {
        const int nchunk = p.nsteps * NF * 64;
        for (int e = tid; e < nchunk; e += 256) reinterpret_cast<f32x4*>(wl)[e] = reinterpret_cast<const f32x4*>(a.wpk)[e];
    }
    const f32x4* wglob = reinterpret_cast<const f32x4*>(a.wpk) + lane;
    const unsigned char* wlds_lane = wl + 16 * lane;
    const int nseg = p.nseg, up = p.up;
    unsigned base[RPW];
#pragma unroll
    for (int r = 0; r < RPW; ++r) base[r] = (unsigned)(((RPW * wv + r) * p.stride * p.PW + nl * p.stride) * p.pixstride + 16 * g);
    f32x4 b4[NF];
#pragma unroll
    for (int f = 0; f < NF; ++f) b4[f] = *reinterpret_cast<const f32x4*>(a.bias + 16 * f + 4 * g);

    const int quads = a.Cin >> 2, o = tid & (quads - 1), sh = quads == 4 ? 2 : (quads == 8 ? 3 : 4);
    unsigned rel[NPF], vmask = 0;
    {
        const int total = p.PH * p.PW * quads;
#pragma unroll
        for (int k = 0; k < NPF; ++k) {
            const int e = 256 * k + tid, pix = e >> sh;
            const int r = (int)__umulhi((unsigned)pix, p.m_pw), c = pix - r * p.PW;
            if (e < total) vmask |= 1u << k;
            rel[k] = (unsigned)(((r * a.W + c) * a.Cin + 4 * o) * 4);
        }
    }
    float ssum[STATS ? NF : 1][4], ssq[STATS ? NF : 1][4];
#pragma unroll
    for (int f = 0; f < (STATS ? NF : 1); ++f)
#pragma unroll
        for (int q = 0; q < 4; ++q) ssum[f][q] = ssq[f][q] = 0.f;
    const int lb = STATS ? xcd_swizzle((int)blockIdx.x, G) : (int)blockIdx.x;
    auto flush_stats = [&](int n_img) {
        float* red = reinterpret_cast<float*>(patch);
#pragma unroll
        for (int f = 0; f < (STATS ? NF : 1); ++f)
#pragma unroll
            for (int q = 0; q < 4; ++q) {
                const float s1 = row16_sum(ssum[f][q]), s2 = row16_sum(ssq[f][q]);
                if (nl == 0) {
                    red[(wv * 2 + 0) * 16 * NF + 16 * f + 4 * g + q] = s1;
                    red[(wv * 2 + 1) * 16 * NF + 16 * f + 4 * g + q] = s2;
                }
                ssum[f][q] = ssq[f][q] = 0.f;
            }
        __syncthreads();
        if (tid < 2 * 16 * NF)
            a.partial[((size_t)n_img * G + lb) * 2 * 16 * NF + tid] = red[tid] + red[2 * 16 * NF + tid] + red[4 * 16 * NF + tid] + red[6 * 16 * NF + tid];
        __syncthreads();
    };
    int cur_n = -1;
    f32x4 amu[STATS == 2 ? NF : 1], ars[STATS == 2 ? NF : 1];
    float nsc[4], nnb[4];
    int cur_in = -1;
    const size_t out_row = (size_t)(up ? 2 : 1) * a.Wo * a.Cout * 4;
    P32Regs<NPF> R;
    int it = 0;
    const int chunk = STATS ? (total_tiles + G - 1) / G : 0;
    const int t_end = STATS ? min(total_tiles, (lb + 1) * chunk) : total_tiles;
    auto tile_of = [&](int i) { return STATS ? lb * chunk + i : p32_tile(i, blockIdx.x, G); };
    int t = tile_of(it);
    if (t < t_end) p32_fetch<NPF>(a, p, t, TH, tid, rel, vmask, R);
    while (t < t_end) {
        const int n = ntile == 1 ? t : (int)__umulhi((unsigned)t, p.m_ntile), tt = t - n * ntile;
        const int ty = a.tiles_x == 1 ? tt : (int)__umulhi((unsigned)tt, p.m_tx), tx = tt - ty * a.tiles_x;
        const int gy0 = ty * TH, gx0 = tx * P32_TW;
        if (STATS && n != cur_n) {
            if (cur_n >= 0) flush_stats(cur_n);
            cur_n = n;
            if (STATS == 2) {
#pragma unroll
                for (int f = 0; f < (STATS == 2 ? NF : 1); ++f) {
                    const float* st = a.aux_stats + ((size_t)n * a.Cout + 16 * f + 4 * g) * 2;
                    const f32x4 s0 = *reinterpret_cast<const f32x4*>(st), s1_ = *reinterpret_cast<const f32x4*>(st + 4);
                    amu[f] = f32x4{s0[0], s0[2], s1_[0], s1_[2]};
                    ars[f] = f32x4{s0[1], s0[3], s1_[1], s1_[3]};
                }
            }
        }
        if (a.in_stats && n != cur_in) {
            const float* st = a.in_stats + ((size_t)n * a.Cin + 4 * o) * 2;
#pragma unroll
            for (int c = 0; c < 4; ++c) { nsc[c] = st[2 * c + 1]; nnb[c] = st[2 * c]; }
            cur_in = n;
        }
#pragma unroll
        for (int k = 0; k < NPF; ++k)
            if (((vmask >> k) & 1) && !(a.dbg & 8)) {
                f32x4 w = R.v[k];
                if (a.in_stats) {
#pragma unroll
                    for (int c = 0; c < 4; ++c) w[c] = fmaxf((w[c] - nnb[c]) * nsc[c], 0.f);
                }
                if (!((R.okmask >> k) & 1)) w = f32x4{0.f, 0.f, 0.f, 0.f};
                *reinterpret_cast<f32x4*>(patch + (unsigned)(((256 * k + tid) >> sh) * p.pixstride + 16 * o)) = w;
            }
        __syncthreads();
        const int tnext = tile_of(it + 1);
        if (tnext < t_end && !(a.dbg & 4)) p32_fetch<NPF>(a, p, tnext, TH, tid, rel, vmask, R);

        for (int sg = 0; sg < nseg; ++sg) {
            const int4 ci = *reinterpret_cast<const int4*>(smem + 4 * P32_MAX_STEPS + 16 * sg);
            const int s0 = __builtin_amdgcn_readfirstlane(ci.x), s1 = __builtin_amdgcn_readfirstlane(ci.y);
            const int oyc = __builtin_amdgcn_readfirstlane(ci.z), oxc = __builtin_amdgcn_readfirstlane(ci.w);
            f32x4 acc[RPW][NF];
            const int mul = up ? 2 : 1;
            const bool full_tile = gy0 + TH <= a.Gh && gx0 + P32_TW <= a.Gw && (a.Cout & 15) == 0;
            const size_t ybyte = ((((size_t)n * a.Ho + gy0 * mul + oyc) * a.Wo + gx0 * mul + oxc) * a.Cout) * 4;
            const unsigned out_off0 = (unsigned)(((RPW * wv * mul) * a.Wo + nl * mul) * a.Cout + 4 * g) * 4u;
            f32x4 av[STATS == 2 ? RPW : 1][STATS == 2 ? NF : 1];
            if (STATS == 2 && full_tile && !(a.dbg & 2)) {
                const char* abase = reinterpret_cast<const char*>(a.aux) + ybyte;
#pragma unroll
                for (int r = 0; r < RPW; ++r)
#pragma unroll
                    for (int f = 0; f < NF; ++f) av[STATS == 2 ? r : 0][STATS == 2 ? f : 0] = *reinterpret_cast<const f32x4*>(abase + r * out_row + out_off0 + 64 * f);
            }
            auto load_ko = [&](int s) -> unsigned { return reinterpret_cast<const unsigned*>(smem)[s]; };
            auto load_ops = [&](unsigned ko, int s, f32x4 (&bf)[RPW], f32x4 (&af)[NF]) {
#pragma unroll
                for (int r = 0; r < RPW; ++r) bf[r] = *reinterpret_cast<const f32x4*>(patch + base[r] + ko);
#pragma unroll
                for (int f = 0; f < NF; ++f) {
                    if (WLDS) af[f] = *reinterpret_cast<const f32x4*>(wlds_lane + (size_t)(s * NF + f) * 1024);
                    else af[f] = wglob[(size_t)(s * NF + f) * 64];
                }
            };
            auto mma_step = [&](const f32x4 (&bf)[RPW], const f32x4 (&af)[NF], auto from_bias) {
#pragma unroll
                for (int j = 0; j < 4; ++j)
#pragma unroll
                    for (int f = 0; f < NF; ++f)
#pragma unroll
                        for (int r = 0; r < RPW; ++r)
                            acc[r][f] = __builtin_amdgcn_mfma_f32_16x16x4f32(af[f][j], bf[r][j],
                                                                             (decltype(from_bias)::value && j == 0) ? b4[f] : acc[r][f], 0, 0, 0);
            };
            auto clip = [&](int s) { return s < s1 ? s : s1 - 1; };
            f32x4 bA[RPW], aA[NF], bB[RPW], aB[NF];
            unsigned k0 = load_ko(s0), k1 = load_ko(clip(s0 + 1));
            load_ops(k0, s0, bA, aA);
            k0 = load_ko(clip(s0 + 2));
            load_ops(k1, clip(s0 + 1), bB, aB);
            mma_step(bA, aA, P32True{});
            int s = s0 + 1;
            if (a.dbg & 1) s = s1;
            for (; s + 1 < s1; s += 2) {
                k1 = load_ko(clip(s + 2));
                load_ops(k0, s + 1, bA, aA);
                mma_step(bB, aB, P32False{});
                k0 = load_ko(clip(s + 3));
                load_ops(k1, clip(s + 2), bB, aB);
                mma_step(bA, aA, P32False{});
            }
            if (s < s1) mma_step(bB, aB, P32False{});
            if (a.dbg & 2) continue;
            if (full_tile) {
                char* ybase = reinterpret_cast<char*>(a.y) + ybyte;
#pragma unroll
                for (int r = 0; r < RPW; ++r)
#pragma unroll
                    for (int f = 0; f < NF; ++f) {
                        if (STATS == 1) {
#pragma unroll
                            for (int q = 0; q < 4; ++q) { const float dv = acc[r][f][q] - b4[f][q]; ssum[f][q] += dv; ssq[f][q] += dv * dv; }
                        }
                        *reinterpret_cast<f32x4*>(ybase + r * out_row + out_off0 + 64 * f) = acc[r][f];
                    }
                if (STATS == 2) {
#pragma unroll
                    for (int r = 0; r < RPW; ++r)
#pragma unroll
                        for (int f = 0; f < NF; ++f) {
                            const f32x4 xh = (av[STATS == 2 ? r : 0][STATS == 2 ? f : 0] - amu[STATS == 2 ? f : 0]) * ars[STATS == 2 ? f : 0];
#pragma unroll
                            for (int q = 0; q < 4; ++q) {
                                const float gg = xh[q] > 0.f ? acc[r][f][q] : 0.f;
                                ssum[f][q] += gg;
                                ssq[f][q] += gg * xh[q];
                            }
                        }
                }
            } else {
#pragma unroll
                for (int r = 0; r < RPW; ++r) {
                    const int gy = gy0 + RPW * wv + r, gx = gx0 + nl;
                    if (gy < a.Gh && gx < a.Gw) {
                        const int oy = gy * mul + oyc, ox = gx * mul + oxc;
#pragma unroll
                        for (int f = 0; f < NF; ++f)
                            if (16 * f + 4 * g < a.Cout) {
                                const size_t oe = (((size_t)n * a.Ho + oy) * a.Wo + ox) * a.Cout + 16 * f + 4 * g;
                                if (STATS == 1) {
#pragma unroll
                                    for (int q = 0; q < 4; ++q) { const float dv = acc[r][f][q] - b4[f][q]; ssum[f][q] += dv; ssq[f][q] += dv * dv; }
                                }
                                if (STATS == 2) {
                                    const f32x4 xh = (*reinterpret_cast<const f32x4*>(a.aux + oe) - amu[STATS == 2 ? f : 0]) * ars[STATS == 2 ? f : 0];
#pragma unroll
                                    for (int q = 0; q < 4; ++q) {
                                        const float gg = xh[q] > 0.f ? acc[r][f][q] : 0.f;
                                        ssum[f][q] += gg;
                                        ssq[f][q] += gg * xh[q];
                                    }
                                }
                                *reinterpret_cast<f32x4*>(a.y + oe) = acc[r][f];
                            }
                    }
                }
            }
        }
        __syncthreads();
        ++it;
        t = tnext;
    }
    if (STATS && cur_n >= 0) flush_stats(cur_n);
}

__global__ __launch_bounds__(256) void p32_norm_finalize_kernel(const float* __restrict__ partial, float* __restrict__ stats, int G, int CP,
                                                                int C, float count, int ntile, int chunk, const float* __restrict__ pivot) {
    __shared__ double red[256 * 2];
    const int n = blockIdx.x, tid = threadIdx.x;
    const int per_c = 256 / CP, c = tid % CP, sub = tid / CP;
    const int b_lo = (int)(((long)n * ntile) / chunk), b_hi = (int)((((long)n + 1) * ntile - 1) / chunk);
    double s1 = 0.0, s2 = 0.0;
    {
        const int b_end = (b_hi < G - 1 ? b_hi : G - 1) + 1;
        int b = b_lo + sub;
        for (; b + 7 * per_c < b_end; b += 8 * per_c) {
            float u[8], w[8];
#pragma unroll
            for (int k = 0; k < 8; ++k) {
                const float* pp = partial + ((size_t)n * G + b + k * per_c) * 2 * CP;
                u[k] = pp[c];
                w[k] = pp[CP + c];
            }
#pragma unroll
            for (int k = 0; k < 8; ++k) {
                s1 += (double)u[k];
                s2 += (double)w[k];
            }
        }
        for (; b < b_end; b += per_c) {
            const float* pp = partial + ((size_t)n * G + b) * 2 * CP;
            s1 += (double)pp[c];
            s2 += (double)pp[CP + c];
        }
    }
    red[tid * 2] = s1;
    red[tid * 2 + 1] = s2;
    __syncthreads();
    if (sub == 0 && c < C) {
        for (int k = 1; k < per_c; ++k) { s1 += red[(k * CP + c) * 2]; s2 += red[(k * CP + c) * 2 + 1]; }
        const double e1 = s1 / count;
        double var = s2 / count - e1 * e1;
        if (var < 0.0) var = 0.0;
        stats[((size_t)n * C + c) * 2] = (float)((double)pivot[c] + e1);
        stats[((size_t)n * C + c) * 2 + 1] = (float)(1.0 / sqrt(var + 1e-5));
    }
}

__global__ __launch_bounds__(256) void p32_bsum_finalize_kernel(const float* __restrict__ partial, float* __restrict__ sums, int G, int CP,
                                                                int C, int ntile, int chunk) {
    __shared__ double red[256 * 2];
    const int n = blockIdx.x, tid = threadIdx.x;
    const int per_c = 256 / CP, c = tid % CP, sub = tid / CP;
    const int b_lo = (int)(((long)n * ntile) / chunk), b_hi = (int)((((long)n + 1) * ntile - 1) / chunk);
    double s1 = 0.0, s2 = 0.0;
    {
        const int b_end = (b_hi < G - 1 ? b_hi : G - 1) + 1;
        int b = b_lo + sub;
        for (; b + 7 * per_c < b_end; b += 8 * per_c) {
            float u[8], w[8];
#pragma unroll
            for (int k = 0; k < 8; ++k) {
                const float* pp = partial + ((size_t)n * G + b + k * per_c) * 2 * CP;
                u[k] = pp[c];
                w[k] = pp[CP + c];
            }
#pragma unroll
            for (int k = 0; k < 8; ++k) {
                s1 += (double)u[k];
                s2 += (double)w[k];
            }
        }
        for (; b < b_end; b += per_c) {
            const float* pp = partial + ((size_t)n * G + b) * 2 * CP;
            s1 += (double)pp[c];
            s2 += (double)pp[CP + c];
        }
    }
    red[tid * 2] = s1;
    red[tid * 2 + 1] = s2;
    __syncthreads();
    if (sub == 0 && c < C) {
        for (int k = 1; k < per_c; ++k) { s1 += red[(k * CP + c) * 2]; s2 += red[(k * CP + c) * 2 + 1]; }
        sums[(size_t)n * 2 * C + c] = (float)s1;
        sums[(size_t)n * 2 * C + C + c] = (float)s2;
    }
}

constexpr int P32I_MAX_STEPS = 16, P32I_TH = 16, P32I_NPX = 2;

struct P32iPlan {
    int nsteps, K, pad, PH, PW, flip;
    unsigned koff[P32I_MAX_STEPS][4];
    unsigned m_pw, m_ntile, m_tx;
};

__global__ void p32i_pack_kernel(const P32iPlan p, const float* __restrict__ w, const float* __restrict__ bias, int w_so, int w_sr, int Cin,
                                 float* __restrict__ wpk, float* __restrict__ bpk) {
    const int total = p.nsteps * 64 * 4, T = p.K * p.K;
    for (int e = blockIdx.x * blockDim.x + threadIdx.x; e < total; e += gridDim.x * blockDim.x) {
        const int j = e & 3, lane = (e >> 2) & 63, s = e >> 8;
        const int co = lane & 15, t = 4 * s + (lane >> 4);
        float v = 0.f;
        if (t < T && j < Cin) v = w[(size_t)co * w_so + (size_t)j * w_sr + (p.flip ? T - 1 - t : t)];
        wpk[e] = v;
    }
    for (int c = blockIdx.x * blockDim.x + threadIdx.x; c < 16; c += gridDim.x * blockDim.x) bpk[c] = bias ? bias[c] : 0.f;
}

struct P32iRegs {
    float v[P32I_NPX][3];
    unsigned okmask;
};

__device__ __forceinline__ void p32i_fetch(const P32Args& a, const P32iPlan& p, int t, int tid, P32iRegs& R) {
    const int ntile = a.tiles_x * a.tiles_y;
    const int n = ntile == 1 ? t : (int)__umulhi((unsigned)t, p.m_ntile), tt = t - n * ntile;
    const int ty = a.tiles_x == 1 ? tt : (int)__umulhi((unsigned)tt, p.m_tx), tx = tt - ty * a.tiles_x;
    const int sy0 = ty * P32I_TH - p.pad, sx0 = tx * P32_TW - p.pad;
    const size_t plane = (size_t)a.H * a.W;
    const float* img = a.x + (size_t)n * a.Cin * plane;
    R.okmask = 0;
#pragma unroll
    for (int k = 0; k < P32I_NPX; ++k) {
        const int e = 256 * k + tid;
        const int r = (int)__umulhi((unsigned)e, p.m_pw), c = e - r * p.PW;
        const int iy = sy0 + r, ix = sx0 + c;
        const bool ok = e < p.PH * p.PW && (unsigned)iy < (unsigned)a.H && (unsigned)ix < (unsigned)a.W;
        R.okmask |= (unsigned)ok << k;
        const unsigned off = ok ? (unsigned)(iy * a.W + ix) : 0u;
#pragma unroll
        for (int ch = 0; ch < 3; ++ch) R.v[k][ch] = img[off + (ch < a.Cin ? ch * plane : 0)];
    }
}

__global__ __launch_bounds__(256) void conv_p32i_kernel(const P32Args a, const P32iPlan p) {
    extern __shared__ __attribute__((aligned(16))) unsigned char smem[];
    constexpr int RPW = P32I_TH / 4, TH = P32I_TH;
    const int tid = threadIdx.x, lane = tid & 63, wv = tid >> 6, nl = lane & 15, g = lane >> 4;
    const int ntile = a.tiles_x * a.tiles_y, total_tiles = a.N * ntile, G = gridDim.x;
    unsigned char* wl = smem + P32I_MAX_STEPS * 16;
    unsigned char* patch = wl + (size_t)p.nsteps * 1024;
    if (tid < P32I_MAX_STEPS * 4) reinterpret_cast<unsigned*>(smem)[tid] = p.koff[tid >> 2][tid & 3];
    for (int e = tid; e < p.nsteps * 64; e += 256) reinterpret_cast<f32x4*>(wl)[e] = reinterpret_cast<const f32x4*>(a.wpk)[e];
    const unsigned char* wlds_lane = wl + 16 * lane;
    unsigned base[RPW];
#pragma unroll
    for (int r = 0; r < RPW; ++r) base[r] = (unsigned)(((RPW * wv + r) * p.PW + nl) * 16);
    const f32x4 b4 = *reinterpret_cast<const f32x4*>(a.bias + 4 * g);
    const size_t out_row = (size_t)a.Wo * 16 * 4;
    P32iRegs R;
    int it = 0;
    int t = p32_tile(it, blockIdx.x, G);
    if (t < total_tiles) p32i_fetch(a, p, t, tid, R);
    const int nsteps = p.nsteps;
    while (t < total_tiles) {
// ... 109 lines not shown
template <int RPW, int NPF>
__global__ __launch_bounds__(256) void conv_p32d_kernel(const P32Args a, const P32dPlan p, const int act) {
    extern __shared__ __attribute__((aligned(16))) unsigned char smem[];
    constexpr int TH = 4 * RPW;
    const int tid = threadIdx.x, lane = tid & 63, wv = tid >> 6, nl = lane & 15, g = lane >> 4;
    const int ntile = a.tiles_x * a.tiles_y, total_tiles = a.N * ntile, G = gridDim.x;
    unsigned char* wl = smem + 4 * P32_MAX_STEPS;
    unsigned char* patch = wl + (size_t)p.nsteps * 1024;
    if (tid < P32_MAX_STEPS) reinterpret_cast<unsigned*>(smem)[tid] = p.koff[tid];
    for (int e = tid; e < p.nsteps * 64; e += 256) reinterpret_cast<f32x4*>(wl)[e] = reinterpret_cast<const f32x4*>(a.wpk)[e];
    const unsigned char* wlds_lane = wl + 16 * lane;
    unsigned base[RPW];
#pragma unroll
    for (int r = 0; r < RPW; ++r) base[r] = (unsigned)(((RPW * wv + r) * p.PW + nl) * p.pixstride + 16 * g);
    const int quads = a.Cin >> 2, o = tid & (quads - 1), sh = quads == 4 ? 2 : (quads == 8 ? 3 : 4), total = p.PH * p.PW * quads;
    const f32x4 b4 = *reinterpret_cast<const f32x4*>(a.bias);
    const int nsteps = p.nsteps;
    P32Regs<NPF> R;
    int it = 0;
    int t = p32_tile(it, blockIdx.x, G);
    if (t < total_tiles) p32d_fetch<NPF>(a, p, t, TH, tid, R);
    while (t < total_tiles) {
        const int n = ntile == 1 ? t : (int)__umulhi((unsigned)t, p.m_ntile), tt = t - n * ntile;
        const int ty = a.tiles_x == 1 ? tt : (int)__umulhi((unsigned)tt, p.m_tx), tx = tt - ty * a.tiles_x;
#pragma unroll
        for (int k = 0; k < NPF; ++k) {
            const int e = 256 * k + tid;
            if (e < total) *reinterpret_cast<f32x4*>(patch + (unsigned)((e >> sh) * p.pixstride + 16 * o)) = ((R.okmask >> k) & 1) ? R.v[k] : f32x4{0.f, 0.f, 0.f, 0.f};
        }
        __syncthreads();
        const int tnext = p32_tile(it + 1, blockIdx.x, G);
        if (tnext < total_tiles) p32d_fetch<NPF>(a, p, tnext, TH, tid, R);

        f32x4 acc[RPW];
#pragma unroll
        for (int r = 0; r < RPW; ++r) acc[r] = f32x4{0.f, 0.f, 0.f, 0.f};
        auto load_ko = [&](int s) -> unsigned { return reinterpret_cast<const unsigned*>(smem)[s]; };
        auto load_ops = [&](unsigned ko, int s, f32x4 (&bf)[RPW], f32x4& af) {
#pragma unroll
            for (int r = 0; r < RPW; ++r) bf[r] = *reinterpret_cast<const f32x4*>(patch + base[r] + ko);
            af = *reinterpret_cast<const f32x4*>(wlds_lane + (size_t)s * 1024);
        };
        auto mma_step = [&](const f32x4 (&bf)[RPW], const f32x4& af) {
#pragma unroll
            for (int j = 0; j < 4; ++j)
#pragma unroll
                for (int r = 0; r < RPW; ++r) acc[r] = __builtin_amdgcn_mfma_f32_16x16x4f32(af[j], bf[r][j], acc[r], 0, 0, 0);
        };
        auto clip = [&](int s) { return s < nsteps ? s : nsteps - 1; };
        f32x4 bA[RPW], bB[RPW], aA, aB;
        unsigned k0 = load_ko(0), k1 = load_ko(clip(1));
        load_ops(k0, 0, bA, aA);
        k0 = load_ko(clip(2));
        load_ops(k1, clip(1), bB, aB);
        mma_step(bA, aA);
        int s = 1;
        for (; s + 1 < nsteps; s += 2) {
            k1 = load_ko(clip(s + 2));
            load_ops(k0, s + 1, bA, aA);
            mma_step(bB, aB);
            k0 = load_ko(clip(s + 3));
            load_ops(k1, clip(s + 2), bB, aB);
            mma_step(bA, aA);
        }
        if (s < nsteps) mma_step(bB, aB);
        __syncthreads();
        float* comb = reinterpret_cast<float*>(patch) + wv * (256 * RPW);
#pragma unroll
        for (int r = 0; r < RPW; ++r) *reinterpret_cast<f32x4*>(&comb[((r * 4 + g) * 16 + nl) * 4]) = acc[r];
        __syncthreads();
        if (g < RPW && nl < 13) {
            f32x4 v = b4;
#pragma unroll
            for (int d = 0; d < 4; ++d) v += *reinterpret_cast<const f32x4*>(&comb[((g * 4 + d) * 16 + nl + 3 - d) * 4]);
            const int oy = ty * TH + RPW * wv + g, ox = tx * 13 + nl;
            if (oy < a.Ho && ox < a.Wo) {
#pragma unroll
                for (int e = 0; e < 4; ++e)
                    if (e < a.Cout) a.y[(((size_t)n * a.Cout + e) * a.Ho + oy) * a.Wo + ox] = apply_act(v[e], act);
            }
        }
        __syncthreads();
        ++it;
        t = tnext;
    }
}

static bool p32d_eligible(const IGemmArgs& a) {
    if (!(a.y_nchw && !a.x_nchw && a.Co <= 4 && a.y_coff == 0 && a.y_ctot == a.Co && a.x_coff == 0 && a.x_ctot == a.Cr && a.Cr == 16 &&
          a.KH == a.KW && a.KH >= 3 && a.KH <= 7 && a.stride == 1 && a.dil == 1 && !a.phase && !a.accumulate &&
          (a.act == MSTG_ACT_NONE || a.act == MSTG_ACT_TANH)))
        return false;
    const char* e = env_get(ENV_NO_DPACK);
    return !(e && e[0] == '1') && (size_t)a.H * a.W * a.Cr * 4 < ((size_t)1 << 32);
}

static void p32d_plan(const IGemmArgs& a, P32dPlan& p, int TH) {
    memset(&p, 0, sizeof(p));
    p.K = a.KH; p.pad = a.pad; p.flip = a.flip;
    p.tapsx = cdiv(p.K, 4);
    p.PH = TH + p.K - 1;
    p.PW = 15 + 4 * p.tapsx;
    p.pixstride = 4 * a.Cr + 32;
    int s = 0;
    for (int ky = 0; ky < p.K; ++ky)
        for (int j = 0; j < p.tapsx; ++j, ++s) {
            p.koff[s] = (unsigned)((ky * p.PW + 4 * j + 3) * p.pixstride);
            p.tky[s] = (int8_t)ky; p.tj[s] = (int8_t)j; p.tcb[s] = 0;
        }
    p.nsteps = s;
    p.m_pw = magic_u32((unsigned)p.PW);
    p.npf = cdiv(p.PH * p.PW * (a.Cr / 4), 256);
}

template <int RPW, int NPF>
static int p32d_launch_t(const P32Args& a, const P32dPlan& p, int act, size_t lds, long tiles, hipStream_t st) {
    auto kern = conv_p32d_kernel<RPW, NPF>;
    static OccCache occ;
    long g_ = 256L * persistent_occupancy(occ, reinterpret_cast<const void*>(kern), lds);
    if (g_ > tiles) g_ = (tiles + 7) & ~7L;
    MSTG_LAUNCH(kern, dim3((unsigned)g_), dim3(256), lds, st, a, p, act);
    MSTG_CHECK_LAUNCH("conv_p32d_kernel");
    return MSTG_OK;
}

static int launch_p32d(const IGemmArgs& g, const P32Route& r, void* workspace, size_t workspace_bytes, hipStream_t st) {
    const int TH = r.head_th;
    P32dPlan p;
    p32d_plan(g, p, TH);
    if (!workspace || workspace_bytes < r.pack_bytes) return fail_arg(MSTG_E_WORKSPACE, "conv_p32d: workspace too small for the packed filter");
    P32Args a{};
    a.x = g.x; a.y = g.y;
    a.bias = (const float*)workspace;
    a.wpk = (const float*)((const char*)workspace + 256);
    a.N = g.N; a.H = g.H; a.W = g.W; a.Cin = g.Cr; a.Ho = g.Ho; a.Wo = g.Wo; a.Cout = g.Co;
    a.tiles_y = cdiv(g.Ho, TH);
    a.tiles_x = cdiv(g.Wo, 13);
    const long tiles = (long)a.N * a.tiles_x * a.tiles_y;
    if ((unsigned long long)(tiles + 4096) * (unsigned long long)(a.tiles_x * a.tiles_y) >= (1ull << 32))
        return fail_arg(MSTG_E_UNSUPPORTED, "conv_p32d: tensor too large for the 32-bit tile arithmetic");
    p.m_ntile = magic_u32((unsigned)(a.tiles_x * a.tiles_y));
    p.m_tx = magic_u32((unsigned)a.tiles_x);
    MSTG_PACK_LAUNCH(p32d_pack_kernel, dim3(16), dim3(256), 0, st, p, g.w, g.bias, g.w_so, g.w_sr, g.Co, g.Cr, (float*)a.wpk, (float*)a.bias);
    MSTG_CHECK_LAUNCH("p32d_pack_kernel");
    size_t patch = (size_t)p.PH * p.PW * p.pixstride;
    if (patch < (size_t)4 * 256 * (TH / 4) * sizeof(float)) patch = (size_t)4 * 256 * (TH / 4) * sizeof(float);
    const size_t lds = 4 * P32_MAX_STEPS + (size_t)p.nsteps * 1024 + patch;
    if (TH == 16) return p.npf <= 8 ? p32d_launch_t<4, 8>(a, p, g.act, lds, tiles, st) : fail_arg(MSTG_E_UNSUPPORTED, "conv_p32d: patch too large");
    return p.npf <= 6 ? p32d_launch_t<2, 6>(a, p, g.act, lds, tiles, st) : fail_arg(MSTG_E_UNSUPPORTED, "conv_p32d: patch too large");
}

__global__ __launch_bounds__(256) void conv_co1_kernel(const float* __restrict__ x, const float* __restrict__ w, const float* __restrict__ bias,
                                                       float* __restrict__ y, int H, int W, int Cr, int Ho, int Wo, int KH, int KW, int pad,
                                                       int w_sr) {
    extern __shared__ __attribute__((aligned(16))) float sm[];
    const int T = KH * KW, tid = threadIdx.x;
    float* wl = sm;
    float* red = sm + T * Cr;
    for (int e = tid; e < T * Cr; e += 256) {
        const int t = e / Cr, ci = e - t * Cr;
        wl[e] = w[(size_t)ci * w_sr + t];
    }
    __syncthreads();
    const int oy = blockIdx.x, n = blockIdx.y;
    const int per = 256 / T, t = tid % T, slot = tid / T, ky = t / KW, kx = t - ky * KW;
    const float b = bias ? bias[0] : 0.f;
    for (int ox0 = 0; ox0 < Wo; ox0 += per) {
        const int ox = ox0 + slot, iy = oy - pad + ky, ix = ox - pad + kx;
        float acc = 0.f;
        if (slot < per && ox < Wo && (unsigned)iy < (unsigned)H && (unsigned)ix < (unsigned)W) {
            const f32x4* xp = reinterpret_cast<const f32x4*>(x + (((size_t)n * H + iy) * W + ix) * Cr);
            const f32x4* wp = reinterpret_cast<const f32x4*>(wl + t * Cr);
            f32x4 a4 = {0.f, 0.f, 0.f, 0.f};
#pragma unroll 4
            for (int c = 0; c < (Cr >> 2); ++c) a4 += xp[c] * wp[c];
            acc = (a4[0] + a4[1]) + (a4[2] + a4[3]);
        }
        red[tid] = acc;
        __syncthreads();
        if (t == 0 && slot < per && ox < Wo) {
            float sum = b;
            for (int k = 0; k < T; ++k) sum += red[tid + k];
            y[((size_t)n * Ho + oy) * Wo + ox] = sum;
        }
        __syncthreads();
    }
}

static bool co1_eligible(const IGemmArgs& a) {
    return a.Co == 1 && a.y_ctot == 1 && a.y_coff == 0 && !a.x_nchw && a.x_coff == 0 && a.x_ctot == a.Cr && (a.Cr & 3) == 0 && a.Cr >= 16 &&
           a.stride == 1 && a.dil == 1 && !a.phase && !a.flip && !a.accumulate && a.act == MSTG_ACT_NONE && a.KH * a.KW <= 16 &&
           (size_t)(a.KH * a.KW * a.Cr + 256) * sizeof(float) <= 64 * 1024 && a.Ho <= 65535 && a.N <= 65535;
}

static int launch_co1(const IGemmArgs& a, hipStream_t st) {
    const size_t lds = (size_t)(a.KH * a.KW * a.Cr + 256) * sizeof(float);
    MSTG_LAUNCH(conv_co1_kernel, dim3(a.Ho, a.N), dim3(256), lds, st, a.x, a.w, a.bias, a.y, a.H, a.W, a.Cr, a.Ho, a.Wo, a.KH, a.KW,
                       a.pad, a.w_sr);
    MSTG_CHECK_LAUNCH("conv_co1_kernel");
    return MSTG_OK;
}

static bool p32i_eligible(const IGemmArgs& a) {
    return a.x_nchw && !a.y_nchw && a.Cr <= 3 && a.x_coff == 0 && a.x_ctot == a.Cr && a.Co == 16 && a.y_ctot == 16 && a.y_coff == 0 &&
           a.KH == a.KW && a.KH >= 3 && a.KH * a.KW <= 4 * P32I_MAX_STEPS && a.stride == 1 && a.dil == 1 && !a.phase && !a.accumulate &&
           a.act == MSTG_ACT_NONE && (a.KH + P32I_TH - 1) * (a.KW + P32_TW - 1) <= 256 * P32I_NPX && (size_t)a.H * a.W < ((size_t)1 << 30);
}

static void p32i_plan(const IGemmArgs& a, P32iPlan& p) {
    memset(&p, 0, sizeof(p));
    p.K = a.KH; p.pad = a.pad; p.flip = a.flip;
    p.PH = P32I_TH + p.K - 1; p.PW = P32_TW + p.K - 1;
    p.nsteps = cdiv(p.K * p.K, 4);
    for (int s = 0; s < p.nsteps; ++s)
        for (int g = 0; g < 4; ++g) {
            const int t = 4 * s + g < p.K * p.K ? 4 * s + g : 0;
            p.koff[s][g] = (unsigned)(((t / p.K) * p.PW + t % p.K) * 16);
        }
    p.m_pw = magic_u32((unsigned)p.PW);
}

static int launch_p32i(const IGemmArgs& g, const P32Route& r, void* workspace, size_t workspace_bytes, hipStream_t st) {
    P32iPlan p;
    p32i_plan(g, p);
    if (!workspace || workspace_bytes < r.pack_bytes) return fail_arg(MSTG_E_WORKSPACE, "conv_p32i: workspace too small for the packed filter");
    P32Args a{};
    a.x = g.x; a.y = g.y;
    a.bias = (const float*)workspace;
    a.wpk = (const float*)((const char*)workspace + 256);
    a.N = g.N; a.H = g.H; a.W = g.W; a.Cin = g.Cr; a.Ho = g.Ho; a.Wo = g.Wo; a.Cout = g.Co;
    a.Gh = g.Ho; a.Gw = g.Wo;
    a.tiles_y = cdiv(a.Gh, P32I_TH);
    a.tiles_x = cdiv(a.Gw, P32_TW);
    const long tiles = (long)a.N * a.tiles_x * a.tiles_y;
    if ((unsigned long long)(tiles + 4096) * (unsigned long long)(a.tiles_x * a.tiles_y) >= (1ull << 32))
        return fail_arg(MSTG_E_UNSUPPORTED, "conv_p32i: tensor too large for the 32-bit tile arithmetic");
    p.m_ntile = magic_u32((unsigned)(a.tiles_x * a.tiles_y));
    p.m_tx = magic_u32((unsigned)a.tiles_x);
    MSTG_PACK_LAUNCH(p32i_pack_kernel, dim3(16), dim3(256), 0, st, p, g.w, g.bias, g.w_so, g.w_sr, g.Cr, (float*)a.wpk, (float*)a.bias);
    MSTG_CHECK_LAUNCH("p32i_pack_kernel");
    const size_t lds = (size_t)P32I_MAX_STEPS * 16 + (size_t)p.nsteps * 1024 + (size_t)p.PH * p.PW * 16;
    static OccCache occ;
    int occ_ = persistent_occupancy(occ, reinterpret_cast<const void*>(conv_p32i_kernel), lds);
    { const char* e = env_get(ENV_P32_OCC); if (e && atoi(e) >= 1 && atoi(e) < occ_) occ_ = atoi(e); }
    long g_ = 256L * occ_;
    if (g_ > tiles) g_ = (tiles + 7) & ~7L;
    MSTG_LAUNCH(conv_p32i_kernel, dim3((unsigned)g_), dim3(256), lds, st, a, p);
    MSTG_CHECK_LAUNCH("conv_p32i_kernel");
    return MSTG_OK;
}

static int p32_plan(const IGemmArgs& a, P32Plan& p) {
    memset(&p, 0, sizeof(p));
    const int Cin = a.Cr, nchunk = Cin / 16;
    p.NF = a.Co / 16;
    const bool one = a.KH == 1;
    p.KW = a.KW;
    p.up = a.phase ? 1 : 0;
    p.stride = (p.up || one) ? 1 : 2;
    p.pixstride = 4 * Cin + (p.stride == 1 ? 32 : 16);
    const int halo_lo = one ? 0 : -1, halo_hi = one ? 0 : (p.up ? 1 : 2);
    const int ext = halo_hi - halo_lo;
    p.PW = (P32_TW - 1) * p.stride + 1 + ext;
    p.oy0 = p.ox0 = halo_lo;
    int s = 0;
    if (one) {
        p.nseg = 1;
        p.seg[0].s0 = 0;
        for (int c = 0; c < nchunk; ++c, ++s) { p.koff[s] = (unsigned)(64 * c); p.tky[s] = p.tkx[s] = 0; p.tcb[s] = (int16_t)(16 * c); }
        p.seg[0].s1 = s;
    } else if (!p.up) {
        p.nseg = 1;
        p.seg[0].s0 = 0;
        for (int ky = 0; ky < 4; ++ky)
            for (int kx = 0; kx < 4; ++kx)
                for (int c = 0; c < nchunk; ++c, ++s) {
                    p.koff[s] = (unsigned)((ky * p.PW + kx) * p.pixstride + 64 * c);
                    p.tky[s] = (int8_t)ky; p.tkx[s] = (int8_t)kx; p.tcb[s] = (int16_t)(16 * c);
                }
        p.seg[0].s1 = s;
    } else {
        p.nseg = 4;
        for (int cls = 0; cls < 4; ++cls) {
            const int py = cls >> 1, px = cls & 1;
            p.seg[cls].s0 = s; p.seg[cls].oy = py; p.seg[cls].ox = px;
            for (int aa = 0; aa < 2; ++aa)
                for (int bb = 0; bb < 2; ++bb) {
                    const int dyy = py == 0 ? aa - 1 : aa, ky = py == 0 ? (aa == 0 ? 3 : 1) : (aa == 0 ? 2 : 0);
                    const int dxx = px == 0 ? bb - 1 : bb, kx = px == 0 ? (bb == 0 ? 3 : 1) : (bb == 0 ? 2 : 0);
                    for (int c = 0; c < nchunk; ++c, ++s) {
                        p.koff[s] = (unsigned)(((dyy + 1) * p.PW + dxx + 1) * p.pixstride + 64 * c);
                        p.tky[s] = (int8_t)ky; p.tkx[s] = (int8_t)kx; p.tcb[s] = (int16_t)(16 * c);
                    }
                }
            p.seg[cls].s1 = s;
        }
    }
    if (s > P32_MAX_STEPS) return fail_arg(MSTG_E_UNSUPPORTED, "conv_p32: too many K-steps");
    p.nsteps = s;
    const size_t wb = (size_t)p.nsteps * p.NF * 1024;
    auto patch_bytes_of = [&](int th) {
        const int ph = (th - 1) * p.stride + 1 + ext;
        return cdiv(ph * p.PW * (Cin / 4), 256) > 12 ? (size_t)1 << 30 : (size_t)ph * p.PW * p.pixstride;
    };
    int TH = 0, wlds = 0;
    const int cand[3] = {16, 8, 4};
    for (int pass = 0; pass < 2 && !TH; ++pass)
        for (int k = 0; k < 3 && !TH; ++k) {
            const size_t need = P32_TABLE_BYTES + patch_bytes_of(cand[k]) + (pass == 0 ? wb : 0);
            if (need <= 78 * 1024 && !(p.NF == 4 && cand[k] == 16)) { TH = cand[k]; wlds = pass == 0; }
        }
    if (!TH) { TH = 4; wlds = 0; }
    if (a.KH == 1 && a.KW == 1 && p.NF == 2 && TH == 16) TH = 8;
    { const char* e = env_get(ENV_P32_TH); if (e && (atoi(e) == 4 || atoi(e) == 8 || atoi(e) == 16) && !(p.NF == 4 && atoi(e) == 16)) TH = atoi(e); }
    { const char* e = env_get(ENV_P32_WLDS); if (e) wlds = atoi(e) != 0; }
    if (patch_bytes_of(TH) >= ((size_t)1 << 30)) return fail_arg(MSTG_E_UNSUPPORTED, "conv_p32: patch needs more than 12 prefetch registers");
    if (P32_TABLE_BYTES + patch_bytes_of(TH) + (wlds ? wb : 0) > 156 * 1024) return fail_arg(MSTG_E_UNSUPPORTED, "conv_p32: LDS budget");
    p.TH = TH; p.wlds = wlds;
    p.PH = (TH - 1) * p.stride + 1 + ext;
    p.m_pw = magic_u32((unsigned)p.PW);
    p.npf = cdiv(p.PH * p.PW * (Cin / 4), 256);
    return MSTG_OK;
}

P32Route p32_route(const IGemmArgs& a) {
    P32Route r{};
    const char* e = env_get(ENV_P32);
    if (e && e[0] == '0') return r;
    if (co1_eligible(a)) {
        r.kind = P32_CO1;
        r.pack_bytes = 16;
        return r;
    }
    if (p32i_eligible(a)) {
        r.kind = P32_IMG;
        r.pack_bytes = 256 + (size_t)cdiv(a.KH * a.KW, 4) * 1024;
        return r;
    }
    if (p32d_eligible(a)) {
        r.kind = P32_HEAD;
        r.head_th = a.Ho >= 16 ? 16 : 8;
        r.pack_bytes = 256 + (size_t)a.KH * cdiv(a.KW, 4) * 1024;
        return r;
    }
    auto ch_ok = [](int c) { return c == 16 || c == 32 || c == 64; };
    if (a.x_nchw || a.y_nchw || a.x_coff || a.y_coff || a.x_ctot != a.Cr || a.y_ctot != a.Co) return r;
    if (!ch_ok(a.Cr) || !ch_ok(a.Co)) return r;
    if (a.accumulate || a.act != MSTG_ACT_NONE) return r;
    if (a.KH == 1 && a.KW == 1) {
        if (a.phase || a.stride != 1 || a.pad != 0 || a.H != a.Ho || a.W != a.Wo) return r;
    } else {
        if (a.KH != 4 || a.KW != 4 || a.dil != 1 || a.flip) return r;
        if (a.phase ? !(a.Ho == 2 * a.H && a.Wo == 2 * a.W) : !(a.stride == 2 && a.pad == 1 && a.H == 2 * a.Ho && a.W == 2 * a.Wo)) return r;
    }
    if (p32_plan(a, r.plan)) return r;
    r.kind = P32_GENERIC;
    r.pack_bytes = 256 + (size_t)r.plan.nsteps * r.plan.NF * 1024;
    r.stats_bytes = ((r.pack_bytes + 255) & ~(size_t)255) + (size_t)a.N * 1024 * 2 * a.Co * sizeof(float);
    return r;
}

template <int RPW, int NF, int NPF>
static int p32_launch_t(P32Args& a, const P32Plan& p, size_t lds, long tiles, hipStream_t st, float* out_stats) {
    const int mode = !out_stats ? 0 : (a.aux ? 2 : 1);
    auto kern = mode == 2 ? (p.wlds ? conv_p32_kernel<RPW, NF, NPF, true, 2> : conv_p32_kernel<RPW, NF, NPF, false, 2>)
              : mode == 1 ? (p.wlds ? conv_p32_kernel<RPW, NF, NPF, true, 1> : conv_p32_kernel<RPW, NF, NPF, false, 1>)
                          : (p.wlds ? conv_p32_kernel<RPW, NF, NPF, true, 0> : conv_p32_kernel<RPW, NF, NPF, false, 0>);
    static OccCache occ_tab[6];
    int c_occ = persistent_occupancy(occ_tab[(p.wlds ? 1 : 0) + 2 * mode], reinterpret_cast<const void*>(kern), lds);
    { const char* e = env_get(ENV_P32_OCC); if (e && atoi(e) >= 1 && atoi(e) < c_occ) c_occ = atoi(e); }
    long g_ = 256L * c_occ;
    if (g_ > tiles) g_ = (tiles + 7) & ~7L;
    MSTG_LAUNCH(kern, dim3((unsigned)g_), dim3(256), lds, st, a, p);
    MSTG_CHECK_LAUNCH("conv_p32_kernel");
    if (mode == 2) {
        const int ntile = a.tiles_x * a.tiles_y;
        MSTG_LAUNCH(p32_bsum_finalize_kernel, dim3(a.N), dim3(256), 0, st, (const float*)a.partial, out_stats, (int)g_, 16 * NF, a.Cout, ntile,
                    (int)((tiles + g_ - 1) / g_));
        MSTG_CHECK_LAUNCH("p32_bsum_finalize_kernel");
    } else if (out_stats) {
        const int ntile = a.tiles_x * a.tiles_y;
        MSTG_LAUNCH(p32_norm_finalize_kernel, dim3(a.N), dim3(256), 0, st, (const float*)a.partial, out_stats, (int)g_, 16 * NF, a.Cout,
                           (float)((size_t)a.Ho * a.Wo), ntile, (int)((tiles + g_ - 1) / g_), a.bias);
        MSTG_CHECK_LAUNCH("p32_norm_finalize_kernel");
    }
    return MSTG_OK;
}

static int p32_npf_regs(const P32Plan& p) { return p.npf <= 6 ? 6 : (p.npf <= 8 ? 8 : 12); }

template <int RPW, int NF>
static int p32_launch_npf(P32Args& a, const P32Plan& p, size_t lds, long tiles, hipStream_t st, float* out_stats) {
    const int regs = p32_npf_regs(p);
    if (regs == 6) return p32_launch_t<RPW, NF, 6>(a, p, lds, tiles, st, out_stats);
    if (regs == 8) return p32_launch_t<RPW, NF, 8>(a, p, lds, tiles, st, out_stats);
    return p32_launch_t<RPW, NF, 12>(a, p, lds, tiles, st, out_stats);
}

int launch_p32(const IGemmArgs& g, const P32Route& r, const float* in_stats, float* out_stats, const float* aux, const float* aux_stats,
               void* workspace, size_t workspace_bytes, hipStream_t st) {
    if (r.kind != P32_GENERIC) {
        if (in_stats || out_stats) return fail_arg(MSTG_E_UNSUPPORTED, "conv_p32: InstanceNorm folding only in the generic persistent kernel");
        if (r.kind == P32_CO1) return launch_co1(g, st);
        if (r.kind == P32_IMG) return launch_p32i(g, r, workspace, workspace_bytes, st);
        if (r.kind == P32_HEAD) return launch_p32d(g, r, workspace, workspace_bytes, st);
        return fail_arg(MSTG_E_UNSUPPORTED, "conv_p32: not a layer of the persistent kernels");
    }
    P32Plan p = r.plan;
    if (!workspace || workspace_bytes < (out_stats ? r.stats_bytes : r.pack_bytes))
        return fail_arg(MSTG_E_WORKSPACE, "conv_p32: workspace too small for the packed filter");
    P32Args a;
    a.in_stats = in_stats;
    a.aux = aux;
    a.aux_stats = aux_stats;
    a.partial = out_stats ? (float*)((char*)workspace + ((r.pack_bytes + 255) & ~(size_t)255)) : nullptr;
    a.x = g.x; a.y = g.y;
    a.bias = (const float*)workspace;
    a.wpk = (const float*)((const char*)workspace + 256);
    a.N = g.N; a.H = g.H; a.W = g.W; a.Cin = g.Cr; a.Ho = g.Ho; a.Wo = g.Wo; a.Cout = g.Co;
    a.Gh = p.up ? g.H : g.Ho;
    a.Gw = p.up ? g.W : g.Wo;
    a.tiles_y = cdiv(a.Gh, p.TH);
    a.tiles_x = cdiv(a.Gw, P32_TW);
    { const char* e = env_get(ENV_P32_DBG); a.dbg = e ? atoi(e) : 0; }
    const long tiles = (long)a.N * a.tiles_x * a.tiles_y;
    if ((unsigned long long)(tiles + 4096) * (unsigned long long)(a.tiles_x * a.tiles_y) >= (1ull << 32) || (size_t)g.H * g.W * g.Cr * 4 >= (1ull << 32))
        return fail_arg(MSTG_E_UNSUPPORTED, "conv_p32: tensor too large for the 32-bit tile / offset arithmetic");
    p.m_ntile = magic_u32((unsigned)(a.tiles_x * a.tiles_y));
    p.m_tx = magic_u32((unsigned)a.tiles_x);
    MSTG_PACK_LAUNCH(p32_pack_kernel, dim3(32), dim3(256), 0, st, p, g.w, g.bias, g.w_so, g.w_sr, g.Co, g.Cr, (float*)a.wpk, (float*)a.bias);
    MSTG_CHECK_LAUNCH("p32_pack_kernel");
    size_t lds = P32_TABLE_BYTES + (size_t)p.PH * p.PW * p.pixstride + (p.wlds ? (size_t)p.nsteps * p.NF * 1024 : 0);
    lds = (lds + 15) & ~(size_t)15;
    if (out_stats && lds < (size_t)P32_TABLE_BYTES + (p.wlds ? (size_t)p.nsteps * p.NF * 1024 : 0) + 8 * 16 * p.NF * sizeof(float)) lds += 8 * 16 * p.NF * sizeof(float);
#define MSTG_P32_CASE(R_, F_) if (p.TH == 4 * R_ && p.NF == F_) return p32_launch_npf<R_, F_>(a, p, lds, tiles, st, out_stats);
    MSTG_P32_CASE(1, 1) MSTG_P32_CASE(2, 1) MSTG_P32_CASE(4, 1)
    MSTG_P32_CASE(1, 2) MSTG_P32_CASE(2, 2) MSTG_P32_CASE(4, 2)
    MSTG_P32_CASE(1, 4) MSTG_P32_CASE(2, 4)
#undef MSTG_P32_CASE
    return fail_arg(MSTG_E_UNSUPPORTED, "conv_p32: no kernel variant");
}

const char* p32_kernel_name(const P32Route& r) {
    static thread_local char name[64];
    if (r.kind == P32_CO1) return "conv_co1_kernel";
    if (r.kind == P32_IMG) return "conv_p32i_kernel";
    if (r.kind == P32_HEAD) return r.head_th == 16 ? "conv_p32d_kernel<4, 8>" : "conv_p32d_kernel<2, 6>";
    if (r.kind != P32_GENERIC) return "";
    snprintf(name, sizeof(name), "conv_p32_kernel<%d, %d, %d, %s, 0>", r.plan.TH / 4, r.plan.NF, p32_npf_regs(r.plan),
             r.plan.wlds ? "true" : "false");
    return name;
}

}
```

### multi-style-transfer-gan_amd/mstg_hip/csrc/igemm_args.h

```cpp
#pragma once
#include "common.h"

namespace mstg {

struct IGemmArgs {
    const float* x;
    float* y;
    const float* w;
    const float* bias;
    int N;
    int H, W, x_ctot, x_coff, x_nchw;
    int Cr;
    int Ho, Wo, y_ctot, y_coff, y_nchw;
    int Co;
    int Gh, Gw;
    int tiles_x, tiles_y;
    int KH, KW, stride, pad, dil, flip, phase;
    int w_so, w_sr;
    int PH, PW;
    int TG;
    int ntaps;
    int act, accumulate;
    int dbg;
    int psz;
    int wglob;
    int TH;
    int dpack, tapsx;
};

constexpr int P32_MAX_STEPS = 64;
constexpr int P32_MAX_SEG = 4;

struct P32Plan {
    int nsteps, nseg;
    struct Seg { int s0, s1, oy, ox; } seg[P32_MAX_SEG];
    unsigned koff[P32_MAX_STEPS];
    int8_t tky[P32_MAX_STEPS], tkx[P32_MAX_STEPS];
    int16_t tcb[P32_MAX_STEPS];
    int PH, PW, pixstride, oy0, ox0, stride, up, NF, TH, npf, wlds, KW;
    unsigned m_pw, m_ntile, m_tx;
};

enum P32Kind {
    P32_NONE,
    P32_CO1,
    P32_IMG,
    P32_HEAD,
    P32_GENERIC
};
struct P32Route {
    P32Kind kind;
    P32Plan plan;
    int head_th;
    size_t pack_bytes;
    size_t stats_bytes;
    bool stats_pays() const { return kind == P32_GENERIC && plan.npf <= 8; }
    bool bsums_pays() const { return kind == P32_GENERIC && plan.NF <= 2 && plan.npf <= 8; }
};
P32Route p32_route(const IGemmArgs& a);
int launch_p32(const IGemmArgs& a, const P32Route& r, const float* in_stats, float* out_stats, const float* aux, const float* aux_stats,
               void* workspace, size_t workspace_bytes, hipStream_t st);
const char* p32_kernel_name(const P32Route& r);

bool img_dgrad_eligible(const IGemmArgs& a);
int launch_img_dgrad(const IGemmArgs& a, hipStream_t st);

}
```

### multi-style-transfer-gan_amd/mstg_hip/ops.py

```python
from __future__ import annotations

import ctypes as C
from typing import Optional, Tuple

import os

import torch

from . import _lib
from ._lib import ACT_GELU, ACT_LEAKY02, ACT_NONE, ACT_RELU, ACT_TANH, LOSS_L1, LOSS_MSE, ConvDesc

Tensor = torch.Tensor


def refresh_env() -> None:
    _lib.load().mstg_env_refresh()
    bump_pack_epoch()


def _stream() -> int:
    return torch.cuda.current_stream().cuda_stream


def _p(t: Optional[Tensor]):
# ... 35 lines not shown
    def __exit__(self, *exc):
        global _DIRECT_PARAM_GRADS
        _DIRECT_PARAM_GRADS = self.prev
        return False


def _grad_slot(p):
    if not _DIRECT_PARAM_GRADS or not isinstance(p, torch.nn.Parameter) or p.grad is None or not p.grad.is_contiguous():
        return None
    return p.grad


class KernelTimer:
    enabled = False
    calls = []

    @classmethod
    def start(cls):
        _lib.check(_lib.load().mstg_prof_enable(1), "mstg_prof_enable")
        cls.enabled, cls.calls = True, []

    @classmethod
    def stop(cls):
        cls.enabled = False
        _lib.load().mstg_prof_enable(0)

    @classmethod
    def kernels(cls):
        lib = _lib.load()
        out, buf, ms = [], C.create_string_buffer(512), C.c_float()
        for i in range(lib.mstg_prof_count()):
            _lib.check(lib.mstg_prof_get(i, buf, 512, C.byref(ms)), "mstg_prof_get")
            out.append((buf.value.decode(), float(ms.value)))
        return out

    @staticmethod
    def _owner(label, names_ms):
        stem = label.split("<")[0]
        hits = [k for k, (nm, _) in enumerate(names_ms) if nm.split("<")[0] == stem]
        if hits:
            return max(hits, key=lambda k: names_ms[k][1])
        return max(range(len(names_ms)), key=lambda k: names_ms[k][1])

    @classmethod
    def summary(cls, detail=False, by_call=False):
        ks = cls.kernels()
        out = {}

        def row(key):
            return out.setdefault(key, {"launches": 0, "ms": 0.0, "flops": 0.0, "bytes": 0.0})
        covered = [False] * len(ks)
        for label, c0, c1, fl, by, det, split in cls.calls:
            mine = ks[c0:c1]
            if not mine:
                continue
            for k in range(c0, c1):
                covered[k] = True
            if by_call:
                r = row(f"{label} {det}" if detail else label)
                r["launches"] += 1
                r["ms"] += sum(m for _, m in mine)
                r["flops"] += fl
                r["bytes"] += by
                r.setdefault("kernels", set()).update(nm for nm, _ in mine)
                continue
            shares = {}
            if split:
                for k, (nm, _) in enumerate(mine):
                    for stem, (sfl, sby) in split.items():
                        if nm.split("<")[0] == stem.split("<")[0] and (stem.find("<") < 0 or nm.startswith(stem)):
                            shares[k] = (sfl, sby)
            if not shares:
                shares[cls._owner(label, mine)] = (fl, by)
            for k, (nm, m) in enumerate(mine):
                r = row(f"{nm} {det}" if detail else nm)
                r["launches"] += 1
                r["ms"] += m
                sfl, sby = shares.get(k, (0.0, 0.0))
                r["flops"] += sfl
                r["bytes"] += sby
        for k, (nm, m) in enumerate(ks):
            if not covered[k]:
                r = row(nm)
                r["launches"] += 1
                r["ms"] += m
        return out


def _timed(sym, flops, nbytes, fn, detail="", split=None):
    if not KernelTimer.enabled:
        return fn()
    lib = _lib.load()
    c0 = lib.mstg_prof_count()
    fn()
    KernelTimer.calls.append((sym, c0, lib.mstg_prof_count(), float(flops), float(nbytes), detail, split))


def _conv_detail(tag, d: ConvDesc):
    return (f"{tag} N{d.N} {d.H}x{d.W} {d.Cin}->{d.Cout} k{d.KH} s{d.stride} d{d.dil}" + (" T" if d.transposed else "")
            + (f" ycoff{d.y_coff}/{d.y_ctot}" if d.y_ctot != d.Cout else ""))


def _conv_cost(d: ConvDesc):
    T = d.KH * d.KW
    macs = d.N * (d.H * d.W if d.transposed else d.Ho * d.Wo) * d.Cin * d.Cout * T
    nbytes = 4 * (d.N * d.H * d.W * d.Cin + d.N * d.Ho * d.Wo * d.Cout + d.Cin * d.Cout * T)
    return 2 * macs, nbytes


def _kernel_name(d: ConvDesc, which: int) -> str:
    return _lib.load().mstg_conv2d_kernel_name(C.byref(d), which).decode() if KernelTimer.enabled else ""


PACK_EPOCH = [0]


def bump_pack_epoch() -> None:
    PACK_EPOCH[0] += 1


def _pack_stamp(owners):
    return tuple(None if t is None else (id(t), t.data_ptr(), t._version, getattr(getattr(t, "_mstg_flat", None), "_version", -1))
                 for t in owners) + (PACK_EPOCH[0],)


def _pack_storages(owners):
    return tuple(None if t is None else t.data for t in owners)


def _cached_ws(owners, kind, dkey, nbytes: int, device):
    if (not owners or owners[0] is None or os.environ.get("MSTG_NO_PACK_CACHE", "0") == "1"
            or not all(t is None or isinstance(t, torch.nn.Parameter) for t in owners)):
        return _ws(nbytes, device), 0
    packs = owners[0].__dict__.setdefault("_mstg_packs", {})
    key, stream = (kind, dkey), torch.cuda.current_stream().cuda_stream
    stamp = _pack_stamp(owners)
    ent = packs.get(key)
    if ent is not None and ent[2] == stream and ent[0].numel() * 4 >= nbytes:
        if ent[1] == stamp:
            return ent[0], 1
        packs[key] = (ent[0], stamp, stream, _pack_storages(owners))
        return ent[0], 0
    ws = _ws(nbytes, device)
    packs[key] = (ws, stamp, stream, _pack_storages(owners))
    return ws, 0


def _dkey(d: ConvDesc, pass_: int):
    fields = tuple(getattr(d, n) for n, _ in ConvDesc._fields_)
    name = _lib.load().mstg_conv2d_kernel_name(C.byref(d), pass_)
    return (name,) + (fields[1:] if name.startswith(b"conv_p32") else fields)


def conv_fwd_raw(d: ConvDesc, x, w, b, y, owners=None):
    fl, by = _conv_cost(d)
    lib = _lib.load()
    ws, packed = _cached_ws(owners, "fwd", _dkey(d, 0), lib.mstg_conv2d_workspace_bytes(C.byref(d)), x.device)
    _timed(_kernel_name(d, 0), fl, by, lambda: _lib.check(
        lib.mstg_conv2d_fwd_cached(C.byref(d), _p(x), _p(w), _p(b), _p(y), _p(ws), ws.numel() * 4, packed, _stream()), "mstg_conv2d_fwd"),
        _conv_detail("fwd", d))


def conv_dgrad_raw(d: ConvDesc, dy, w, dx, owners=None):
    fl, by = _conv_cost(d)
    lib = _lib.load()
    ws, packed = _cached_ws(owners, "dgrad", _dkey(d, 1), lib.mstg_conv2d_workspace_bytes(C.byref(d)), dy.device)
    _timed(_kernel_name(d, 1), fl, by, lambda: _lib.check(
        lib.mstg_conv2d_dgrad_cached(C.byref(d), _p(dy), _p(w), _p(dx), _p(ws), ws.numel() * 4, packed, _stream()), "mstg_conv2d_dgrad"),
        _conv_detail("dgrad", d))


def norm_bsums_enabled() -> bool:
    return os.environ.get("MSTG_NORM_BSUMS", "1") != "0"


def conv_dgrad_bsums_supported(d: ConvDesc) -> bool:
    return norm_bsums_enabled() and bool(_lib.load().mstg_conv2d_dgrad_bsums_supported(C.byref(d)))


def conv_dgrad_bsums_raw(d: ConvDesc, dy, w, dx, x_raw, x_stats, owners=None):
    fl, by = _conv_cost(d)
    lib = _lib.load()
    sums = torch.empty((d.N, 1, 2, d.Cin), dtype=torch.float32, device=dy.device)
    ws, packed = _cached_ws(owners, "dgrad_bsums", _dkey(d, 1), lib.mstg_conv2d_dgrad_bsums_workspace_bytes(C.byref(d)), dy.device)
    _timed(_kernel_name(d, 1), fl, by + 4 * x_raw.numel(), lambda: _lib.check(
        lib.mstg_conv2d_dgrad_bsums(C.byref(d), _p(dy), _p(w), _p(dx), _p(x_raw), _p(x_stats), _p(sums), _p(ws), ws.numel() * 4, packed,
                                    _stream()), "mstg_conv2d_dgrad_bsums"), _conv_detail("dgrad+bsums", d))
    return sums


class _NormToken:
    __slots__ = ()


def _tag_norm_output(y, x_raw, stats, token):
    if token is not None:
        y._mstg_norm = (x_raw, stats, token)
    return y


def conv_wgrad_raw(d: ConvDesc, x, dy, dw, db=None):
    lib = _lib.load()
    nbytes = lib.mstg_conv2d_wgrad_workspace_bytes(C.byref(d))
    ws = _ws(nbytes, x.device)
    fl, by = _conv_cost(d)
    sym = _kernel_name(d, 2)
    _timed(sym, fl, by, lambda: _lib.check(
        lib.mstg_conv2d_wgrad(C.byref(d), _p(x), _p(dy), _p(dw), _p(db), _p(ws), ws.numel() * 4, _stream()), "mstg_conv2d_wgrad"),
        _conv_detail("wgrad", d))


def channel_sum(x: Tensor, P: int, ctot: int, coff: int, Cn: int, scale: float = 1.0) -> Tensor:
    lib = _lib.load()
    out = torch.empty(Cn, dtype=torch.float32, device=x.device)
    ws = _ws(lib.mstg_channel_sum_workspace_bytes(P, Cn), x.device)
    _lib.check(lib.mstg_channel_sum(_p(x), P, ctot, coff, Cn, scale, _p(out), _p(ws), ws.numel() * 4, _stream()),
               "mstg_channel_sum")
    return out


def plane_sum_nchw(x: Tensor) -> Tensor:
    lib = _lib.load()
    N, Cn, H, W = x.shape
    out = torch.empty(Cn, dtype=torch.float32, device=x.device)
    ws = _ws(lib.mstg_plane_sum_workspace_bytes(N, Cn, H * W), x.device)
    _lib.check(lib.mstg_plane_sum(_p(x), N, Cn, H * W, 1.0, _p(out), _p(ws), ws.numel() * 4, _stream()), "mstg_plane_sum")
    return out


class ConvFn(torch.autograd.Function):

    @staticmethod
    def forward(ctx, x, w, b, cfg):
        k, stride, pad, dil, transposed, x_nchw, y_nchw, act = cfg
        x, w = _req(x, "conv input"), _req(w, "conv weight")
        b = None if b is None else _req(b, "conv bias")
        if x_nchw:
            N, Cin, H, W = x.shape
        else:
            N, H, W, Cin = x.shape
        Cout = w.shape[1] if transposed else w.shape[0]
        if (w.shape[0] if transposed else w.shape[1]) != Cin:
            raise RuntimeError(f"mstg_hip conv: weight {tuple(w.shape)} does not match {Cin} input channels")
        Ho, Wo = conv_out_hw(H, W, k, stride, pad, dil, transposed)
        if Ho <= 0 or Wo <= 0:
            raise RuntimeError(f"mstg_hip conv: input {H}x{W} too small for kernel {k} (stride {stride}, pad {pad}, dil {dil})")
        y = torch.empty((N, Cout, Ho, Wo) if y_nchw else (N, Ho, Wo, Cout), dtype=torch.float32, device=x.device)
        d = make_desc(N, H, W, Cin, Ho, Wo, Cout, k, stride, pad, dil, transposed, x_nchw, y_nchw, act=act)
        conv_fwd_raw(d, x, w, b, y, owners=(w, b))
        ctx.cfg, ctx.dims, ctx.has_bias = cfg, (N, H, W, Cin, Ho, Wo, Cout), b is not None
        ctx.norm_src = getattr(x, "_mstg_norm", None) if not x_nchw else None
        ctx.prefs = (w, b)
        ctx.save_for_backward(x, w, y if act != ACT_NONE else None)
        return y

    @staticmethod
    def backward(ctx, dy):
        k, stride, pad, dil, transposed, x_nchw, y_nchw, act = ctx.cfg
        N, H, W, Cin, Ho, Wo, Cout = ctx.dims
        x, w, y = ctx.saved_tensors
        dy = _req(dy, "conv grad_output")
        if act != ACT_NONE:
            dy = act_bwd_raw(y, dy, act)
        d = make_desc(N, H, W, Cin, Ho, Wo, Cout, k, stride, pad, dil, transposed, x_nchw, y_nchw)
        dx = dw = db = None
        if ctx.needs_input_grad[0]:
            dx = torch.empty_like(x)
            src = getattr(ctx, "norm_src", None)
            if src is not None and conv_dgrad_bsums_supported(d):
                sums = conv_dgrad_bsums_raw(d, dy, w, dx, src[0], src[1], owners=(ctx.prefs[0],))
                dx._mstg_bsums = (sums, src[2], dx._version)
            else:
                conv_dgrad_raw(d, dy, w, dx, owners=(ctx.prefs[0],))
        want_db = ctx.has_bias and ctx.needs_input_grad[2]
        fuse_db = want_db and ctx.needs_input_grad[1] and not transposed
        if ctx.needs_input_grad[1]:
            gw = _grad_slot(ctx.prefs[0])
            gb = _grad_slot(ctx.prefs[1]) if fuse_db else None
            if gw is not None and (gb is not None or not fuse_db):
                d.accumulate = 1
                conv_wgrad_raw(d, x, dy, gw, gb)
                d.accumulate = 0
                if fuse_db:
                    want_db = False
            else:
                dw = torch.empty_like(w)
                if fuse_db:
                    db = torch.empty(Cout, dtype=torch.float32, device=dy.device)
                conv_wgrad_raw(d, x, dy, dw, db if fuse_db else None)
        if want_db and not fuse_db:
            db = plane_sum_nchw(dy) if y_nchw else channel_sum(dy, N * Ho * Wo, Cout, 0, Cout)
        return dx, dw, db, None


def conv_norm_supported(N, H, W, Cin, Cout, k, stride, pad, dil, transposed) -> bool:
    Ho, Wo = conv_out_hw(H, W, k, stride, pad, dil, transposed)
    if Ho * Wo < 256:
        return False
    d = make_desc(N, H, W, Cin, Ho, Wo, Cout, k, stride, pad, dil, transposed)
    return bool(_lib.load().mstg_conv2d_fwd_norm_supported(C.byref(d)))


def conv_stats_pays(N, H, W, Cin, Cout, k, stride, pad, dil, transposed) -> bool:
    if not conv_norm_supported(N, H, W, Cin, Cout, k, stride, pad, dil, transposed):
        return False
    Ho, Wo = conv_out_hw(H, W, k, stride, pad, dil, transposed)
    d = make_desc(N, H, W, Cin, Ho, Wo, Cout, k, stride, pad, dil, transposed)
    return bool(_lib.load().mstg_conv2d_fwd_stats_pays(C.byref(d)))


class ConvStatsFn(torch.autograd.Function):

    @staticmethod
    def forward(ctx, x, w, b, cfg):
        lib = _lib.load()
        k, stride, pad, dil, transposed = cfg
        x, w = _req(x, "conv input"), _req(w, "conv weight")
        b = None if b is None else _req(b, "conv bias")
        N, H, W, Cin = x.shape
        Cout = w.shape[1] if transposed else w.shape[0]
        Ho, Wo = conv_out_hw(H, W, k, stride, pad, dil, transposed)
        y = torch.empty((N, Ho, Wo, Cout), dtype=torch.float32, device=x.device)
        stats = torch.empty((N, Cout, 2), dtype=torch.float32, device=x.device)
        d = make_desc(N, H, W, Cin, Ho, Wo, Cout, k, stride, pad, dil, transposed)
        ws, packed = _cached_ws((w, b), "fwd_norm", _dkey(d, 0), lib.mstg_conv2d_fwd_norm_workspace_bytes(C.byref(d)), x.device)
        fl, by = _conv_cost(d)
        _timed(_kernel_name(d, 0).replace(", 0>", ", 1>"), fl, by, lambda: _lib.check(
            lib.mstg_conv2d_fwd_norm_cached(C.byref(d), _p(x), None, _p(w), _p(b), _p(y), _p(stats), _p(ws), ws.numel() * 4, packed,
                                            _stream()), "mstg_conv2d_fwd_norm"), _conv_detail("fwd", d))
        ctx.cfg, ctx.dims, ctx.has_bias = (k, stride, pad, dil, transposed, 0, 0, ACT_NONE), (N, H, W, Cin, Ho, Wo, Cout), b is not None
        ctx.prefs = (w, b)
        ctx.norm_src = getattr(x, "_mstg_norm", None)
        ctx.save_for_backward(x, w, None)
        ctx.mark_non_differentiable(stats)
        return y, stats

    @staticmethod
    def backward(ctx, dy, _dstats):
        return ConvFn.backward(ctx, dy)


def ms_fusion_supported(N, H, W, Cn) -> bool:
    d = make_desc(N, H, W, Cn, H, W, Cn, 1, 1, 0, 1)
    lib = _lib.load()
    return bool(lib.mstg_conv2d_fwd_norm_supported(C.byref(d))) and bool(lib.mstg_conv2d_wgrad_norm_supported(C.byref(d)))


class MSFusionFn(torch.autograd.Function):

    @staticmethod
    def forward(ctx, cat, w, b, cfg=(1, 1, 0, 1)):
        lib = _lib.load()
        cat, w = _req(cat, "fusion input"), _req(w, "fusion weight")
        b = None if b is None else _req(b, "fusion bias")
        N, H, W, Cn = cat.shape
        Cout = w.shape[0]
        k, stride, pad, dil = cfg
        Ho, Wo = conv_out_hw(H, W, k, stride, pad, dil, False)
        stats = torch.empty((N, Cn, 2), dtype=torch.float32, device=cat.device)
        ws = _ws(lib.mstg_norm_workspace_bytes(N, H * W, Cn), cat.device)
        _timed("norm_partial_kernel<false>", 0, 4 * cat.numel(), lambda: _lib.check(
            lib.mstg_norm_stats(_p(cat), _p(stats), N, H * W, Cn, _p(ws), ws.numel() * 4, _stream()), "mstg_norm_stats"))
        y = torch.empty((N, Ho, Wo, Cout), dtype=torch.float32, device=cat.device)
        ystats = torch.empty((N, Cout, 2), dtype=torch.float32, device=cat.device)
        d = make_desc(N, H, W, Cn, Ho, Wo, Cout, k, stride, pad, dil)
        ws2, packed = _cached_ws((w, b), "fwd_norm", _dkey(d, 0), lib.mstg_conv2d_fwd_norm_workspace_bytes(C.byref(d)), cat.device)
        fl, by = _conv_cost(d)
        _timed(_kernel_name(d, 0).replace(", 0>", ", 1>"), fl, by, lambda: _lib.check(
            lib.mstg_conv2d_fwd_norm_cached(C.byref(d), _p(cat), _p(stats), _p(w), _p(b), _p(y), _p(ystats), _p(ws2), ws2.numel() * 4,
                                            packed, _stream()), "mstg_conv2d_fwd_norm"), _conv_detail("fwd", d))
        ctx.dims, ctx.has_bias, ctx.prefs, ctx.cfg = (N, H, W, Cn, Cout), b is not None, (w, b), tuple(cfg)
        ctx.save_for_backward(cat, stats, w)
        ctx.mark_non_differentiable(ystats)
        return y, ystats

    @staticmethod
    def backward(ctx, dy, _dystats):
        lib = _lib.load()
        N, H, W, Cn, Cout = ctx.dims
        cat, stats, w = ctx.saved_tensors
        dy = _req(dy, "fusion grad_output")
        k, stride, pad, dil = ctx.cfg
        Ho, Wo = conv_out_hw(H, W, k, stride, pad, dil, False)
        d = make_desc(N, H, W, Cn, Ho, Wo, Cout, k, stride, pad, dil)
        dcat = dw = db = None
        if ctx.needs_input_grad[0]:
            dz = torch.empty_like(cat)
            dcat = torch.empty_like(cat)
            if conv_dgrad_bsums_supported(d):
                sums = conv_dgrad_bsums_raw(d, dy, w, dz, cat, stats, owners=(ctx.prefs[0],))
                _timed("norm_apply_kernel<true>", 0, 4 * cat.numel() * 3, lambda: _lib.check(
                    lib.mstg_norm_bwd_apply(_p(cat), _p(stats), _p(dz), _p(sums), 1, _p(dcat), N, H * W, Cn, ACT_RELU, _stream()),
                    "mstg_norm_bwd_apply"))
            else:
                conv_dgrad_raw(d, dy, w, dz, owners=(ctx.prefs[0],))
                ws = _ws(lib.mstg_norm_workspace_bytes(N, H * W, Cn), cat.device)
                _timed("norm_apply_kernel<true>", 0, 4 * cat.numel() * 3, lambda: _lib.check(
                    lib.mstg_norm_act_bwd(_p(cat), _p(stats), _p(dz), _p(dcat), N, H * W, Cn, ACT_RELU, 0, None, None, None, None, _p(ws),
                                          ws.numel() * 4, _stream()), "mstg_norm_act_bwd"))
        if ctx.needs_input_grad[1]:
            want_db = ctx.has_bias and ctx.needs_input_grad[2]
            gw = _grad_slot(ctx.prefs[0])
            gb = _grad_slot(ctx.prefs[1]) if want_db else None
            direct = gw is not None and (gb is not None or not want_db)
            if not direct:
                dw = torch.empty_like(w)
                db = torch.empty(Cout, dtype=torch.float32, device=dy.device) if want_db else None
            d.accumulate = 1 if direct else 0
            out_w, out_b = (gw, gb) if direct else (dw, db)
            wsw = _ws(lib.mstg_conv2d_wgrad_workspace_bytes(C.byref(d)), cat.device)
            fl, by = _conv_cost(d)
            _timed(_kernel_name(d, 2), fl, by, lambda: _lib.check(
                lib.mstg_conv2d_wgrad_norm(C.byref(d), _p(cat), _p(stats), _p(dy), _p(out_w), _p(out_b), _p(wsw), wsw.numel() * 4, _stream()),
                "mstg_conv2d_wgrad_norm"), _conv_detail("wgrad", d))
        elif ctx.has_bias and ctx.needs_input_grad[2]:
            db = channel_sum(dy, N * Ho * Wo, Cout, 0, Cout)
        return dcat, dw, db, None


def norm_conv_supported(N, H, W, Cin, Cout, k, stride, pad, dil) -> bool:
    if not conv_stats_pays(N, H, W, Cin, Cout, k, stride, pad, dil, False):
        return False
    Ho, Wo = conv_out_hw(H, W, k, stride, pad, dil, False)
    d = make_desc(N, H, W, Cin, Ho, Wo, Cout, k, stride, pad, dil)
    return bool(_lib.load().mstg_conv2d_wgrad_norm_supported(C.byref(d)))


def conv2d_stats(x, w, b, k, stride=1, pad=0, dil=1, transposed=False):
    return ConvStatsFn.apply(x, w, b, (k, stride, pad, dil, int(transposed)))


def conv2d(x, w, b, k, stride=1, pad=0, dil=1, transposed=False, x_nchw=False, y_nchw=False, act=ACT_NONE):
    return ConvFn.apply(x, w, b, (k, stride, pad, dil, int(transposed), int(x_nchw), int(y_nchw), act))


class MSBranchesFn(torch.autograd.Function):

    GEOM = ((1, 0, 1), (3, 1, 1), (3, 2, 2), (3, 4, 4))

    @staticmethod
    def forward(ctx, x, *wb):
        x = _req(x, "multi-scale input")
        ws = [_req(t, "branch weight") for t in wb[0::2]]
        bs = [_req(t, "branch bias") for t in wb[1::2]]
        N, H, W, ch = x.shape
        c4 = ws[0].shape[0]
        y = torch.empty((N, H, W, 4 * c4), dtype=torch.float32, device=x.device)
        lib = _lib.load()
        if os.environ.get("MSTG_MS_UNFUSED", "0") != "1" and bool(lib.mstg_msblock_fused_supported(ch)) and 4 * c4 == ch:
            wsb, packed = _cached_ws(tuple(wb), "ms_fwd", (ch, H >= 16), lib.mstg_msblock_fwd_workspace_bytes(ch), x.device)
            wb_ptrs = []
            for j in range(4):
                wb_ptrs += [_p(ws[j]), _p(bs[j])]
            fwd4 = ch == 16 and H >= 16 and os.environ.get("MSTG_MS_FWD4", "1") != "0"
            _timed("ms_fwd4_kernel" if fwd4 else f"ms_fwd_kernel<{ch}>", 2.0 * N * H * W * ch * c4 * 28, 4.0 * (2 * N * H * W * ch),
                   lambda: _lib.check(lib.mstg_msblock_fwd_cached(_p(x), *wb_ptrs, _p(y), N, H, W, ch, _p(wsb), wsb.numel() * 4, packed,
                                                                  _stream()), "mstg_msblock_fwd"), f"ms-fwd N{N} {H}x{W} ch{ch}")
        else:
            for j, (k, pad, dil) in enumerate(MSBranchesFn.GEOM):
                d = make_desc(N, H, W, ch, H, W, c4, k, 1, pad, dil, y_ctot=4 * c4, y_coff=j * c4)
                conv_fwd_raw(d, x, ws[j], bs[j], y)
        ctx.dims = (N, H, W, ch, c4)
        ctx.prefs = tuple(wb)
        ctx.save_for_backward(x, *ws)
        return y, x.view_as(x)

    @staticmethod
    def backward(ctx, dy, dres=None):
        N, H, W, ch, c4 = ctx.dims
        x, *ws = ctx.saved_tensors
        dy = _req(dy, "multi-scale grad_output")
        dres = None if dres is None else _req(dres, "multi-scale residual grad")
        dx = torch.empty_like(x) if ctx.needs_input_grad[0] else None
        lib = _lib.load()
        fused = os.environ.get("MSTG_MS_UNFUSED", "0") != "1" and bool(lib.mstg_msblock_fused_supported(ch)) and 4 * c4 == ch
        grads = []
        if fused and dx is not None:
            wsd, packed = _cached_ws(tuple(ctx.prefs[0::2]), "ms_dgrad", (ch,), lib.mstg_msblock_dgrad_workspace_bytes(ch), x.device)
            _timed(f"ms_dgrad_kernel<{ch}>", 2.0 * N * H * W * ch * c4 * 28, 4.0 * (2 * N * H * W * ch),
                   lambda: _lib.check(lib.mstg_msblock_dgrad_cached(_p(dy), *[_p(t) for t in ws], _p(dres), _p(dx), N, H, W, ch, _p(wsd),
                                                                    wsd.numel() * 4, packed, _stream()), "mstg_msblock_dgrad"),
                   f"ms-dgrad N{N} {H}x{W} ch{ch}")
        for j, (k, pad, dil) in enumerate(MSBranchesFn.GEOM):
            d = make_desc(N, H, W, ch, H, W, c4, k, 1, pad, dil, y_ctot=4 * c4, y_coff=j * c4, accumulate=int(j > 0))
            if dx is not None and not fused:
                conv_dgrad_raw(d, dy, ws[j], dx)
# ... 459 lines not shown
    @staticmethod
    def forward(ctx, x):
        x = _req(x, "pool input")
        N, H, W, Cn = x.shape
        y = torch.empty((N, H // 2, W // 2, Cn), dtype=torch.float32, device=x.device)
        idx = torch.empty((N, H // 2, W // 2, Cn), dtype=torch.uint8, device=x.device)
        _lib.check(_lib.load().mstg_maxpool2x2_fwd(_p(x), _p(y), _p(idx), N, H, W, Cn, _stream()), "mstg_maxpool2x2_fwd")
        ctx.shape = (N, H, W, Cn)
        ctx.save_for_backward(idx)
        ctx.mark_non_differentiable(idx)
        return y, idx

    @staticmethod
    def backward(ctx, dy, _didx):
        (idx,) = ctx.saved_tensors
        N, H, W, Cn = ctx.shape
        dy = _req(dy, "pool grad_output")
        dx = torch.zeros((N, H, W, Cn), dtype=torch.float32, device=dy.device) if (H & 1 or W & 1) else \
            torch.empty((N, H, W, Cn), dtype=torch.float32, device=dy.device)
        _lib.check(_lib.load().mstg_maxpool2x2_bwd(_p(dy), _p(idx), _p(dx), N, H, W, Cn, _stream()), "mstg_maxpool2x2_bwd")
        return dx


def maxpool2x2(x, return_indices=False):
    y, idx = MaxPool2x2Fn.apply(x)
    return (y, idx) if return_indices else y


class GramFn(torch.autograd.Function):

    @staticmethod
    def forward(ctx, f):
        lib = _lib.load()
        f = _req(f, "gram input")
        N, H, W, Cn = f.shape
        scale = 1.0 / (Cn * H * W)
        g = torch.empty((N, Cn, Cn), dtype=torch.float32, device=f.device)
        ws = _ws(lib.mstg_gram_workspace_bytes(N, H * W, Cn), f.device)
        _timed("gram_fwd_kernel", 2.0 * N * H * W * Cn * Cn, 4.0 * (N * H * W * Cn + N * Cn * Cn), lambda: _lib.check(
            lib.mstg_gram_fwd(_p(f), _p(g), N, H * W, Cn, scale, _p(ws), ws.numel() * 4, _stream()), "mstg_gram_fwd"))
        ctx.scale = scale
        ctx.save_for_backward(f)
        return g

    @staticmethod
    def backward(ctx, dg):
        (f,) = ctx.saved_tensors
        dg = _req(dg, "gram grad_output")
        N, H, W, Cn = f.shape
        df = torch.empty_like(f)
        _timed("gram_bwd_kernel", 2.0 * N * H * W * Cn * Cn, 4.0 * 2 * N * H * W * Cn, lambda: _lib.check(
            _lib.load().mstg_gram_bwd(_p(f), _p(dg), _p(df), N, H * W, Cn, ctx.scale, _stream()), "mstg_gram_bwd"))
        return df


def gram_matrix(f):
    return GramFn.apply(f)


class SpectralNormFn(torch.autograd.Function):

    @staticmethod
    def forward(ctx, w, u, v, eps, training):
        w = _req(w, "spectral_norm weight")
        u, v = _req(u, "spectral_norm u"), _req(v, "spectral_norm v")
        M = w.shape[0]
        K = w.numel() // M
        if u.numel() != M or v.numel() != K:
            raise RuntimeError(f"mstg_hip spectral_norm: u/v sizes {u.numel()}/{v.numel()} do not match weight {tuple(w.shape)}")
        out = torch.empty_like(w)
        sigma = torch.empty(1, dtype=torch.float32, device=w.device)
        lib = _lib.load()
        ws = _ws(lib.mstg_spectral_norm_workspace_bytes(M, K), w.device)
        need = ctx.needs_input_grad[0]
        us = torch.empty_like(u) if need else None
        vs = torch.empty_like(v) if need else None
        _lib.check(lib.mstg_spectral_norm_fwd(_p(w), _p(u), _p(v), _p(out), _p(sigma), _p(us), _p(vs), M, K, float(eps),
                                              int(bool(training)), _p(ws), ws.numel() * 4, _stream()), "mstg_spectral_norm_fwd")
        ctx.pref = w
        if need:
            ctx.save_for_backward(w, us, vs, sigma)
        ctx.dims = (M, K)
        return out

    @staticmethod
    def backward(ctx, dwn):
        w, u, v, sigma = ctx.saved_tensors
        M, K = ctx.dims
        dwn = _req(dwn, "spectral_norm grad_output")
        slot = _grad_slot(ctx.pref)
        dw = slot if slot is not None else torch.empty_like(w)
        lib = _lib.load()
        ws = _ws(lib.mstg_spectral_norm_workspace_bytes(M, K), w.device)
        _lib.check(lib.mstg_spectral_norm_bwd(_p(dwn), _p(w), _p(u), _p(v), _p(sigma), _p(dw), int(slot is not None), M, K, _p(ws),
                                              ws.numel() * 4, _stream()), "mstg_spectral_norm_bwd")
        return (None if slot is not None else dw), None, None, None, None


def install_fused_spectral_norm(module, name: str = "weight") -> bool:
    from torch.nn.utils.spectral_norm import SpectralNorm
    for key, hook in list(module._forward_pre_hooks.items()):
        if isinstance(hook, SpectralNorm) and hook.name == name:
            if hook.n_power_iterations != 1 or hook.dim != 0:
                return False
            eps = float(hook.eps)
            del module._forward_pre_hooks[key]

            def pre(mod, inputs, _eps=eps, _name=name):
                if mod.__dict__.pop("_mstg_sn_fresh", False):
                    return
                setattr(mod, _name, SpectralNormFn.apply(getattr(mod, _name + "_orig"), getattr(mod, _name + "_u"),
                                                         getattr(mod, _name + "_v"), _eps, mod.training))

            module.register_forward_pre_hook(pre)
            module._mstg_sn = (name, eps)
            return True
    return False


def _ptr_array(tensors):
    return (C.c_void_p * len(tensors))(*[None if t is None else t.data_ptr() for t in tensors])


def _int_array(values):
    return (C.c_int * len(values))(*[int(v) for v in values])


class SpectralNormGroupFn(torch.autograd.Function):

    @staticmethod
    def forward(ctx, eps, training, n, *tensors):
        lib = _lib.load()
        ws_, us_, vs_ = tensors[:n], tensors[n:2 * n], tensors[2 * n:3 * n]
        ws_ = [_req(w, "spectral_norm weight") for w in ws_]
        Ms = [w.shape[0] for w in ws_]
        Ks = [w.numel() // w.shape[0] for w in ws_]
        for w, u, v, M, K in zip(ws_, us_, vs_, Ms, Ks):
            _req(u, "spectral_norm u"), _req(v, "spectral_norm v")
            if u.numel() != M or v.numel() != K:
                raise RuntimeError(f"mstg_hip spectral_norm: u/v sizes {u.numel()}/{v.numel()} do not match weight {tuple(w.shape)}")
        dev = ws_[0].device
        outs = [torch.empty_like(w) for w in ws_]
        sigma = torch.empty(n, dtype=torch.float32, device=dev)
        need = any(ctx.needs_input_grad[3:3 + n])
        u_sv = [torch.empty_like(u) for u in us_] if need else None
        v_sv = [torch.empty_like(v) for v in vs_] if need else None
        Ma, Ka = _int_array(Ms), _int_array(Ks)
        ws = _ws(lib.mstg_spectral_norm_group_workspace_bytes(n, Ma, Ka), dev)
        _lib.check(lib.mstg_spectral_norm_group_fwd(n, _ptr_array(ws_), _ptr_array(us_), _ptr_array(vs_), _ptr_array(outs), _p(sigma),
                                                    _ptr_array(u_sv) if need else None, _ptr_array(v_sv) if need else None, Ma, Ka,
                                                    float(eps), int(bool(training)), _p(ws), ws.numel() * 4, _stream()),
                   "mstg_spectral_norm_group_fwd")
        ctx.n, ctx.dims, ctx.prefs = n, (Ms, Ks), tuple(ws_)
        ctx.set_materialize_grads(False)
        if need:
            ctx.save_for_backward(sigma, *ws_, *u_sv, *v_sv)
        return tuple(outs)

    @staticmethod
    def backward(ctx, *dwns):
        lib = _lib.load()
        n = ctx.n
        saved = ctx.saved_tensors
        sigma, ws_, us_, vs_ = saved[0], saved[1:1 + n], saved[1 + n:1 + 2 * n], saved[1 + 2 * n:1 + 3 * n]
        Ms, Ks = ctx.dims
        live = [j for j in range(n) if dwns[j] is not None and ctx.needs_input_grad[3 + j]]
        grads = [None] * n
        if live:
            dws, accs, dwn_l = [], [], []
            for j in live:
                slot = _grad_slot(ctx.prefs[j])
                dws.append(slot if slot is not None else torch.empty_like(ws_[j]))
                accs.append(slot is not None)
                dwn_l.append(_req(dwns[j], "spectral_norm grad_output"))
                if slot is None:
                    grads[j] = dws[-1]
            Ma, Ka = _int_array([Ms[j] for j in live]), _int_array([Ks[j] for j in live])
            sig_ptrs = (C.c_void_p * len(live))(*[sigma.data_ptr() + 4 * j for j in live])
            ws = _ws(lib.mstg_spectral_norm_group_workspace_bytes(len(live), Ma, Ka), sigma.device)
            _lib.check(lib.mstg_spectral_norm_group_bwd(len(live), _ptr_array(dwn_l), _ptr_array([ws_[j] for j in live]),
                                                        _ptr_array([us_[j] for j in live]), _ptr_array([vs_[j] for j in live]), sig_ptrs,
                                                        _ptr_array(dws), _int_array(accs), Ma, Ka, _p(ws), ws.numel() * 4, _stream()),
                       "mstg_spectral_norm_group_bwd")
        return (None, None, None, *grads, *([None] * (2 * n)))


def spectral_norm_group(modules) -> None:
    lib = _lib.load()
    cap = lib.mstg_spectral_norm_group_max()
    mods = list(modules)
    for k in range(0, len(mods), cap):
        part = mods[k:k + cap]
        names = [m._mstg_sn[0] for m in part]
        eps = part[0]._mstg_sn[1]
        if any(m._mstg_sn[1] != eps or m.training != part[0].training for m in part):
            raise RuntimeError("mstg_hip spectral_norm_group: the modules of a group share eps and the training flag")
        outs = SpectralNormGroupFn.apply(eps, part[0].training, len(part), *[getattr(m, nm + "_orig") for m, nm in zip(part, names)],
                                         *[getattr(m, nm + "_u") for m, nm in zip(part, names)],
                                         *[getattr(m, nm + "_v") for m, nm in zip(part, names)])
        for m, nm, w in zip(part, names, outs):
            setattr(m, nm, w)
            m.__dict__["_mstg_sn_fresh"] = True


def structure_map(img: Tensor) -> Tensor:
    img = _req(img.detach(), "structure-map image")
    N, _, H, W = img.shape
    out = torch.empty((N, H // 4, W // 4, 4), dtype=torch.float32, device=img.device)
    _lib.check(_lib.load().mstg_structure_map(_p(img), _p(out), N, H, W, _stream()), "mstg_structure_map")
    return out


class LayerNormModFn(torch.autograd.Function):

    @staticmethod
    def forward(ctx, x, gamma, beta, gmod, bmod, eps):
        lib = _lib.load()
        x, gamma, beta = _req(x, "layer-norm input"), _req(gamma, "layer-norm weight"), _req(beta, "layer-norm bias")
        gmod = None if gmod is None else _req(gmod, "modulation scale")
        bmod = None if bmod is None else _req(bmod, "modulation shift")
        N, L, dim = x.shape
        y = torch.empty_like(x)
        stats = torch.empty((N * L, 2), dtype=torch.float32, device=x.device)
        _timed("ln_mod_fwd_kernel", 0, 4.0 * 2 * x.numel(), lambda: _lib.check(
            lib.mstg_ln_mod_fwd(_p(x), _p(gamma), _p(beta), _p(gmod), _p(bmod), _p(y), _p(stats), N, L, dim, float(eps), _stream()),
            "mstg_ln_mod_fwd"))
        ctx.prefs = (gamma, beta)
        ctx.has_mod = gmod is not None
        ctx.save_for_backward(x, stats, gamma, beta, gmod)
        return y

    @staticmethod
    def backward(ctx, dy):
        lib = _lib.load()
        x, stats, gamma, beta, gmod = ctx.saved_tensors
        dy = _req(dy, "layer-norm grad_output")
        N, L, dim = x.shape
        dx = torch.empty_like(x)
        sg, sb = _grad_slot(ctx.prefs[0]), _grad_slot(ctx.prefs[1])
        direct = sg is not None and sb is not None
        dgamma = sg if direct else torch.empty_like(gamma)
        dbeta = sb if direct else torch.empty_like(beta)
        dgm = torch.empty((N, dim), dtype=torch.float32, device=x.device) if ctx.has_mod else None
        dbm = torch.empty((N, dim), dtype=torch.float32, device=x.device) if ctx.has_mod else None
        ws = _ws(lib.mstg_ln_mod_bwd_workspace_bytes(N, L, dim), x.device)
        _timed("ln_mod_bwd_kernel", 0, 4.0 * 3 * x.numel(), lambda: _lib.check(
            lib.mstg_ln_mod_bwd(_p(x), _p(stats), _p(gamma), _p(beta), _p(gmod), _p(dy), _p(dx), _p(dgamma), _p(dbeta), _p(dgm), _p(dbm),
                                int(direct), N, L, dim, _p(ws), ws.numel() * 4, _stream()), "mstg_ln_mod_bwd"))
        return dx, (None if direct else dgamma), (None if direct else dbeta), dgm, dbm, None


def layer_norm_mod(x, gamma, beta, gmod=None, bmod=None, eps=1e-5):
    return LayerNormModFn.apply(x, gamma, beta, gmod, bmod, eps)


class FlashAttnFn(torch.autograd.Function):

    @staticmethod
    def forward(ctx, qkv, heads):
        qkv = _req(qkv, "attention qkv")
        N, L, C3 = qkv.shape
        dim = C3 // 3
        D = dim // heads
        if dim * 3 != C3 or D * heads != dim:
            raise RuntimeError(f"mstg_hip flash attention: {C3} channels do not split into q|k|v x {heads} heads")
        out = torch.empty((N, L, dim), dtype=torch.float32, device=qkv.device)
        lse = torch.empty((N, heads, L), dtype=torch.float32, device=qkv.device)
        _timed(f"flash_fwd_kernel<{D}>", 4.0 * N * heads * L * L * D, 4.0 * (qkv.numel() + out.numel()), lambda: _lib.check(
            _lib.load().mstg_flash_attn_fwd(_p(qkv), _p(out), _p(lse), N, L, heads, D, _stream()), "mstg_flash_attn_fwd"),
            f"N{N} L{L} heads{heads} D{D}")
        ctx.heads = heads
        ctx.save_for_backward(qkv, out, lse)
        return out

    @staticmethod
    def backward(ctx, d_out):
        qkv, out, lse = ctx.saved_tensors
        d_out = _req(d_out, "attention grad_output")
        N, L, C3 = qkv.shape
        heads = ctx.heads
        D = C3 // 3 // heads
        dqkv = torch.empty_like(qkv)
        delta = torch.empty((N, heads, L), dtype=torch.float32, device=qkv.device)
        _timed(f"flash_bwd_dkv_kernel<{D}>", 8.0 * N * heads * L * L * D, 4.0 * (2 * qkv.numel() + 2 * out.numel()), lambda: _lib.check(
            _lib.load().mstg_flash_attn_bwd(_p(qkv), _p(out), _p(lse), _p(d_out), _p(dqkv), _p(delta), N, L, heads, D, _stream()),
            "mstg_flash_attn_bwd"), f"N{N} L{L} heads{heads} D{D}",
            split={f"flash_bwd_dq_kernel<{D}>": (4.0 * N * heads * L * L * D, 4.0 * (qkv.numel() + out.numel())),
                   f"flash_bwd_dkv_kernel<{D}>": (4.0 * N * heads * L * L * D, 4.0 * (qkv.numel() + out.numel()))})
        return dqkv, None


def flash_attention(qkv, heads):
    return FlashAttnFn.apply(qkv, heads)


class AddFn(torch.autograd.Function):

    @staticmethod
    def forward(ctx, a, b):
        a, b = _req(a, "add lhs"), _req(b, "add rhs")
        if a.shape != b.shape:
            raise RuntimeError(f"mstg_hip add: shapes differ {tuple(a.shape)} vs {tuple(b.shape)}")
        y = torch.empty_like(a)
        _lib.check(_lib.load().mstg_add(_p(a), _p(b), _p(y), a.numel(), _stream()), "mstg_add")
        return y

    @staticmethod
    def backward(ctx, dy):
        return dy, dy


def add(a, b):
    return AddFn.apply(a, b)


def linear_tokens(x, weight, bias, act=ACT_NONE):
    squeeze = x.dim() == 2
    x4 = x.reshape(x.shape[0], 1, -1 if not squeeze else 1, x.shape[-1]) if not squeeze else x.reshape(x.shape[0], 1, 1, x.shape[-1])
    y = conv2d(x4, weight.view(weight.shape[0], weight.shape[1], 1, 1), bias, 1, act=act)
    return y.reshape(*x.shape[:-1], weight.shape[0])


def adam_step_flat(p, g, m, v, lr, beta1, beta2, eps, step, mask=None):
    bump_pack_epoch()
    _lib.check(_lib.load().mstg_adam_step_flat(_p(p), _p(g), _p(m), _p(v), p.numel(), lr, beta1, beta2, eps, int(step), _p(mask),
                                               _stream()), "mstg_adam_step_flat")
```

Measured before the change: 1719 images/sec.

## Fold spectral-norm sigma into conv epilogue using raw weights and cached packing

Spectral-normalized convolutions now run on the raw, unnormalized weight parameter, and the kernel epilogues divide by sigma on the device (forward and dgrad for the igemm, p32, co1 and image-dgrad paths). Because the raw parameter keeps a stable identity, the packed-filter workspace cache can be reused across calls instead of repacking the freshly normalized weight every step. It adds a per-output multiply, a new template mode for the p32 kernel, and plumbing through autograd. Some kernel variants (stream, image stem, packed head) are excluded and fall back to the old path.

```diff
diff --git a/include/mstg_hip.h b/include/mstg_hip.h
--- a/include/mstg_hip.h
+++ b/include/mstg_hip.h
@@ -53,6 +53,10 @@
                                 float* y, float* out_stats, void* workspace, size_t workspace_bytes, int workspace_packed, void* stream);
 int mstg_conv2d_dgrad_cached(const mstg_conv_desc* d, const float* dy, const float* w, float* dx, void* workspace, size_t workspace_bytes,
                              int workspace_packed, void* stream);
+int mstg_conv2d_fwd_scaled(const mstg_conv_desc* d, const float* x, const float* w, const float* bias , const float* out_scale,
+                           float* y, void* workspace, size_t workspace_bytes, int workspace_packed, void* stream);
+int mstg_conv2d_dgrad_scaled(const mstg_conv_desc* d, const float* dy, const float* w, const float* out_scale, float* dx, void* workspace,
+                             size_t workspace_bytes, int workspace_packed, void* stream);
 int mstg_msblock_fwd_cached(const float* x, const float* w1, const float* b1, const float* w2, const float* b2, const float* w3,
                             const float* b3, const float* w4, const float* b4, float* y, int N, int H, int W, int CH, void* workspace,
                             size_t workspace_bytes, int workspace_packed, void* stream);
diff --git a/multi-style-transfer-gan_amd/mstg_hip/_lib.py b/multi-style-transfer-gan_amd/mstg_hip/_lib.py
--- a/multi-style-transfer-gan_amd/mstg_hip/_lib.py
+++ b/multi-style-transfer-gan_amd/mstg_hip/_lib.py
@@ -58,6 +58,8 @@
     "mstg_conv2d_fwd_cached": (_i, [_dp, _fp, _fp, _fp, _fp, _vp, _sz, _i, _vp]),
     "mstg_conv2d_fwd_norm_cached": (_i, [_dp, _fp, _fp, _fp, _fp, _fp, _fp, _vp, _sz, _i, _vp]),
     "mstg_conv2d_dgrad_cached": (_i, [_dp, _fp, _fp, _fp, _vp, _sz, _i, _vp]),
+    "mstg_conv2d_fwd_scaled": (_i, [_dp, _fp, _fp, _fp, _fp, _fp, _vp, _sz, _i, _vp]),
+    "mstg_conv2d_dgrad_scaled": (_i, [_dp, _fp, _fp, _fp, _fp, _vp, _sz, _i, _vp]),
     "mstg_msblock_fwd_cached": (_i, [_fp] * 10 + [_i, _i, _i, _i, _vp, _sz, _i, _vp]),
     "mstg_msblock_dgrad_cached": (_i, [_fp] * 7 + [_i, _i, _i, _i, _vp, _sz, _i, _vp]),
     "mstg_conv2d_wgrad_workspace_bytes": (_sz, [_dp]),
diff --git a/multi-style-transfer-gan_amd/mstg_hip/csrc/conv_igemm.hip b/multi-style-transfer-gan_amd/mstg_hip/csrc/conv_igemm.hip
--- a/multi-style-transfer-gan_amd/mstg_hip/csrc/conv_igemm.hip
+++ b/multi-style-transfer-gan_amd/mstg_hip/csrc/conv_igemm.hip
@@ -73,6 +73,7 @@
 template <int NFW, int PF = 2>
 __device__ __forceinline__ void igemm_epilogue(const IGemmArgs& a, const f32x4 (&acc)[NFW][PF], int n, int ty0, int tx0, int co0, int pa,
                                                int pb, int wave, int i, int g) {
+    const float osc = a.out_scale ? 1.f / *a.out_scale : 1.f;
 #pragma unroll
     for (int pf = 0; pf < PF; ++pf) {
         const int gy = ty0 * (4 * PF) + PF * wave + pf, gx = tx0 * TILE_W + i;
@@ -83,6 +84,7 @@
             const int co = co0 + 16 * wf + 4 * g;
             if (co >= a.Co) continue;
             f32x4 v = acc[wf][pf];
+            if (a.out_scale) v = v * osc;
             if (!a.y_nchw && co + 3 < a.Co && ((a.y_ctot | a.y_coff) & 3) == 0) {
                 float* p = a.y + (((size_t)n * a.Ho + oy) * a.Wo + ox) * a.y_ctot + a.y_coff + co;
                 if (a.bias) v += *reinterpret_cast<const f32x4*>(a.bias + co);
@@ -268,6 +270,7 @@
         f32x4 v = {0.f, 0.f, 0.f, 0.f};
 #pragma unroll
         for (int d = 0; d < 4; ++d) v += *reinterpret_cast<const f32x4*>(&comb[((pf * 4 + d) * 16 + i + 3 - d) * 4]);
+        if (a.out_scale) v = v * (1.f / *a.out_scale);
         const int oy = ty0 * TH + PF * wave + pf, ox = tx0 * 13 + i;
         if (oy < a.Gh && ox < a.Gw) {
             if (!a.y_nchw && a.Co == 4 && ((a.y_ctot | a.y_coff) & 3) == 0) {
@@ -991,6 +994,7 @@
     { const char* e = env_get(ENV_DBG_LDS_KB); if (e && !p.heavy) p.lds += (size_t)atoi(e) * 1024; }
     if (!workspace || workspace_bytes < p.ws_bytes) return fail_arg(MSTG_E_WORKSPACE, "conv: workspace too small for the packed filter");
     float* wp = (float*)workspace;
+    if (a.out_scale && p.stream) return fail_arg(MSTG_E_UNSUPPORTED, "conv: the stream kernel takes no output scale");
     if (int rc = launch_pack(a, p, wp, st)) return rc;
 #define MSTG_DISPATCH(VV, NN)                                                              \
     if (p.V == VV && p.nfw == NN) {                                                        \
@@ -1195,6 +1199,27 @@
     return mstg_conv2d_dgrad(d, dy, w, dx, workspace, workspace_bytes, stream);
 }
 
+extern "C" int mstg_conv2d_fwd_scaled(const mstg_conv_desc* d, const float* x, const float* w, const float* bias, const float* out_scale,
+                                      float* y, void* workspace, size_t workspace_bytes, int workspace_packed, void* stream) {
+    if (int rc = check_desc(d)) return rc;
+    if (!x || !w || !y || !out_scale) return fail_arg(MSTG_E_BADARG, "conv_fwd_scaled: null pointer");
+    IGemmArgs a{};
+    fill_fwd_args(d, a);
+    a.x = x; a.y = y; a.w = w; a.bias = bias; a.out_scale = out_scale;
+    PackedScope scope(workspace_packed);
+    return launch_igemm(a, workspace, workspace_bytes, (hipStream_t)stream);
+}
+extern "C" int mstg_conv2d_dgrad_scaled(const mstg_conv_desc* d, const float* dy, const float* w, const float* out_scale, float* dx,
+                                        void* workspace, size_t workspace_bytes, int workspace_packed, void* stream) {
+    if (int rc = check_desc(d)) return rc;
+    if (!dy || !w || !dx || !out_scale) return fail_arg(MSTG_E_BADARG, "conv_dgrad_scaled: null pointer");
+    IGemmArgs a{};
+    if (int rc = fill_dgrad_args(d, a)) return rc;
+    a.x = dy; a.y = dx; a.w = w; a.bias = nullptr; a.out_scale = out_scale;
+    PackedScope scope(workspace_packed);
+    return launch_igemm(a, workspace, workspace_bytes, (hipStream_t)stream);
+}
+
 const char* igemm_kernel_name(const mstg_conv_desc* d, int pass) {
     static thread_local char name[64];
     IGemmArgs a{};
diff --git a/multi-style-transfer-gan_amd/mstg_hip/csrc/conv_img.hip b/multi-style-transfer-gan_amd/mstg_hip/csrc/conv_img.hip
--- a/multi-style-transfer-gan_amd/mstg_hip/csrc/conv_img.hip
+++ b/multi-style-transfer-gan_amd/mstg_hip/csrc/conv_img.hip
@@ -7,7 +7,8 @@
 
 template <int CI>
 __global__ __launch_bounds__(256) void conv_img_dgrad_kernel(const float* __restrict__ dy, const float* __restrict__ w, float* __restrict__ dx,
-                                                             int N, int Ho, int Wo, int Cr, int x_ctot, int x_coff, int w_so, int w_sr) {
+                                                             int N, int Ho, int Wo, int Cr, int x_ctot, int x_coff, int w_so, int w_sr,
+                                                             const float* __restrict__ out_scale) {
     extern __shared__ __attribute__((aligned(16))) float wl[];
     const int tid = threadIdx.x;
     for (int e = tid; e < IMG_T * CI * Cr; e += 256) {
@@ -15,6 +16,7 @@
         wl[e] = w[(size_t)cr * w_sr + (size_t)ci * w_so + t];
     }
     __syncthreads();
+    const float osc = out_scale ? 1.f / out_scale[0] : 1.f;
     const long total = (long)N * Ho * Wo;
     const int H = 2 * Ho, W = 2 * Wo;
     const size_t plane = (size_t)H * W;
@@ -62,8 +64,8 @@
 #pragma unroll
             for (int a = 0; a < 2; ++a) {
                 float2 o;
-                o.x = acc[a][0][ci];
-                o.y = acc[a][1][ci];
+                o.x = out_scale ? acc[a][0][ci] * osc : acc[a][0][ci];
+                o.y = out_scale ? acc[a][1][ci] * osc : acc[a][1][ci];
                 *reinterpret_cast<float2*>(img + ci * plane + (size_t)a * W) = o;
             }
     }
@@ -95,7 +97,7 @@
     const size_t lds = (size_t)IMG_T * a.Co * a.Cr * sizeof(float);
 #define MSTG_IMG_DGRAD(CI_)                                                                                                   \
     MSTG_LAUNCH(conv_img_dgrad_kernel<CI_>, dim3(img_grid(total)), dim3(256), lds, st, a.x, a.w, a.y, a.N, a.H, a.W, a.Cr, a.x_ctot, \
-                a.x_coff, a.w_so, a.w_sr)
+                a.x_coff, a.w_so, a.w_sr, a.out_scale)
     if (a.Co == 3) MSTG_IMG_DGRAD(3);
     else if (a.Co == 2) MSTG_IMG_DGRAD(2);
     else MSTG_IMG_DGRAD(1);
diff --git a/multi-style-transfer-gan_amd/mstg_hip/csrc/conv_p32.hip b/multi-style-transfer-gan_amd/mstg_hip/csrc/conv_p32.hip
--- a/multi-style-transfer-gan_amd/mstg_hip/csrc/conv_p32.hip
+++ b/multi-style-transfer-gan_amd/mstg_hip/csrc/conv_p32.hip
@@ -20,6 +20,7 @@
     float* partial;
     const float* aux;
     const float* aux_stats;
+    const float* out_scale;
     int N, H, W, Cin, Ho, Wo, Cout, Gh, Gw, tiles_x, tiles_y, dbg;
 };
 
@@ -78,6 +79,8 @@
 __global__ __launch_bounds__(256) void conv_p32_kernel(const P32Args a, const P32Plan p) {
     extern __shared__ __attribute__((aligned(16))) unsigned char smem[];
     constexpr int TH = 4 * RPW;
+    constexpr bool SUMS = STATS == 1 || STATS == 2;
+    const float osc = STATS == 3 ? 1.f / *a.out_scale : 1.f;
     const int tid = threadIdx.x, lane = tid & 63, wv = tid >> 6, nl = lane & 15, g = lane >> 4;
     const int ntile = a.tiles_x * a.tiles_y, total_tiles = a.N * ntile, G = gridDim.x;
     unsigned char* wl = smem + P32_TABLE_BYTES;
@@ -115,16 +118,16 @@
             rel[k] = (unsigned)(((r * a.W + c) * a.Cin + 4 * o) * 4);
         }
     }
-    float ssum[STATS ? NF : 1][4], ssq[STATS ? NF : 1][4];
-#pragma unroll
-    for (int f = 0; f < (STATS ? NF : 1); ++f)
+    float ssum[SUMS ? NF : 1][4], ssq[SUMS ? NF : 1][4];
+#pragma unroll
+    for (int f = 0; f < (SUMS ? NF : 1); ++f)
 #pragma unroll
         for (int q = 0; q < 4; ++q) ssum[f][q] = ssq[f][q] = 0.f;
-    const int lb = STATS ? xcd_swizzle((int)blockIdx.x, G) : (int)blockIdx.x;
+    const int lb = SUMS ? xcd_swizzle((int)blockIdx.x, G) : (int)blockIdx.x;
     auto flush_stats = [&](int n_img) {
         float* red = reinterpret_cast<float*>(patch);
 #pragma unroll
-        for (int f = 0; f < (STATS ? NF : 1); ++f)
+        for (int f = 0; f < (SUMS ? NF : 1); ++f)
 #pragma unroll
             for (int q = 0; q < 4; ++q) {
                 const float s1 = row16_sum(ssum[f][q]), s2 = row16_sum(ssq[f][q]);
@@ -146,16 +149,16 @@
     const size_t out_row = (size_t)(up ? 2 : 1) * a.Wo * a.Cout * 4;
     P32Regs<NPF> R;
     int it = 0;
-    const int chunk = STATS ? (total_tiles + G - 1) / G : 0;
-    const int t_end = STATS ? min(total_tiles, (lb + 1) * chunk) : total_tiles;
-    auto tile_of = [&](int i) { return STATS ? lb * chunk + i : p32_tile(i, blockIdx.x, G); };
+    const int chunk = SUMS ? (total_tiles + G - 1) / G : 0;
+    const int t_end = SUMS ? min(total_tiles, (lb + 1) * chunk) : total_tiles;
+    auto tile_of = [&](int i) { return SUMS ? lb * chunk + i : p32_tile(i, blockIdx.x, G); };
     int t = tile_of(it);
     if (t < t_end) p32_fetch<NPF>(a, p, t, TH, tid, rel, vmask, R);
     while (t < t_end) {
         const int n = ntile == 1 ? t : (int)__umulhi((unsigned)t, p.m_ntile), tt = t - n * ntile;
         const int ty = a.tiles_x == 1 ? tt : (int)__umulhi((unsigned)tt, p.m_tx), tx = tt - ty * a.tiles_x;
         const int gy0 = ty * TH, gx0 = tx * P32_TW;
-        if (STATS && n != cur_n) {
+        if (SUMS && n != cur_n) {
             if (cur_n >= 0) flush_stats(cur_n);
             cur_n = n;
             if (STATS == 2) {
@@ -224,7 +227,7 @@
 #pragma unroll
                         for (int r = 0; r < RPW; ++r)
                             acc[r][f] = __builtin_amdgcn_mfma_f32_16x16x4f32(af[f][j], bf[r][j],
-                                                                             (decltype(from_bias)::value && j == 0) ? b4[f] : acc[r][f], 0, 0, 0);
+                                                                             (decltype(from_bias)::value && j == 0) ? (STATS == 3 ? f32x4{0.f, 0.f, 0.f, 0.f} : b4[f]) : acc[r][f], 0, 0, 0);
             };
             auto clip = [&](int s) { return s < s1 ? s : s1 - 1; };
             f32x4 bA[RPW], aA[NF], bB[RPW], aB[NF];
@@ -245,6 +248,12 @@
             }
             if (s < s1) mma_step(bB, aB, P32False{});
             if (a.dbg & 2) continue;
+            if (STATS == 3) {
+#pragma unroll
+                for (int r = 0; r < RPW; ++r)
+#pragma unroll
+                    for (int f = 0; f < NF; ++f) acc[r][f] = acc[r][f] * osc + b4[f];
+            }
             if (full_tile) {
                 char* ybase = reinterpret_cast<char*>(a.y) + ybyte;
 #pragma unroll
@@ -304,7 +313,7 @@
         ++it;
         t = tnext;
     }
-    if (STATS && cur_n >= 0) flush_stats(cur_n);
+    if (SUMS && cur_n >= 0) flush_stats(cur_n);
 }
 
 __global__ __launch_bounds__(256) void p32_norm_finalize_kernel(const float* __restrict__ partial, float* __restrict__ stats, int G, int CP,
@@ -720,7 +729,7 @@
 
 __global__ __launch_bounds__(256) void conv_co1_kernel(const float* __restrict__ x, const float* __restrict__ w, const float* __restrict__ bias,
                                                        float* __restrict__ y, int H, int W, int Cr, int Ho, int Wo, int KH, int KW, int pad,
-                                                       int w_sr) {
+                                                       int w_sr, const float* __restrict__ out_scale) {
     extern __shared__ __attribute__((aligned(16))) float sm[];
     const int T = KH * KW, tid = threadIdx.x;
     float* wl = sm;
@@ -733,6 +742,7 @@
     const int oy = blockIdx.x, n = blockIdx.y;
     const int per = 256 / T, t = tid % T, slot = tid / T, ky = t / KW, kx = t - ky * KW;
     const float b = bias ? bias[0] : 0.f;
+    const float osc = out_scale ? 1.f / out_scale[0] : 1.f;
     for (int ox0 = 0; ox0 < Wo; ox0 += per) {
         const int ox = ox0 + slot, iy = oy - pad + ky, ix = ox - pad + kx;
         float acc = 0.f;
@@ -747,8 +757,9 @@
         red[tid] = acc;
         __syncthreads();
         if (t == 0 && slot < per && ox < Wo) {
-            float sum = b;
+            float sum = out_scale ? 0.f : b;
             for (int k = 0; k < T; ++k) sum += red[tid + k];
+            if (out_scale) sum = sum * osc + b;
             y[((size_t)n * Ho + oy) * Wo + ox] = sum;
         }
         __syncthreads();
@@ -764,7 +775,7 @@
 static int launch_co1(const IGemmArgs& a, hipStream_t st) {
     const size_t lds = (size_t)(a.KH * a.KW * a.Cr + 256) * sizeof(float);
     MSTG_LAUNCH(conv_co1_kernel, dim3(a.Ho, a.N), dim3(256), lds, st, a.x, a.w, a.bias, a.y, a.H, a.W, a.Cr, a.Ho, a.Wo, a.KH, a.KW,
-                       a.pad, a.w_sr);
+                       a.pad, a.w_sr, a.out_scale);
     MSTG_CHECK_LAUNCH("conv_co1_kernel");
     return MSTG_OK;
 }
@@ -930,11 +941,12 @@
 
 template <int RPW, int NF, int NPF>
 static int p32_launch_t(P32Args& a, const P32Plan& p, size_t lds, long tiles, hipStream_t st, float* out_stats) {
-    const int mode = !out_stats ? 0 : (a.aux ? 2 : 1);
-    auto kern = mode == 2 ? (p.wlds ? conv_p32_kernel<RPW, NF, NPF, true, 2> : conv_p32_kernel<RPW, NF, NPF, false, 2>)
+    const int mode = a.out_scale ? 3 : (!out_stats ? 0 : (a.aux ? 2 : 1));
+    auto kern = mode == 3 ? (p.wlds ? conv_p32_kernel<RPW, NF, NPF, true, 3> : conv_p32_kernel<RPW, NF, NPF, false, 3>)
+              : mode == 2 ? (p.wlds ? conv_p32_kernel<RPW, NF, NPF, true, 2> : conv_p32_kernel<RPW, NF, NPF, false, 2>)
               : mode == 1 ? (p.wlds ? conv_p32_kernel<RPW, NF, NPF, true, 1> : conv_p32_kernel<RPW, NF, NPF, false, 1>)
                           : (p.wlds ? conv_p32_kernel<RPW, NF, NPF, true, 0> : conv_p32_kernel<RPW, NF, NPF, false, 0>);
-    static OccCache occ_tab[6];
+    static OccCache occ_tab[8];
     int c_occ = persistent_occupancy(occ_tab[(p.wlds ? 1 : 0) + 2 * mode], reinterpret_cast<const void*>(kern), lds);
     { const char* e = env_get(ENV_P32_OCC); if (e && atoi(e) >= 1 && atoi(e) < c_occ) c_occ = atoi(e); }
     long g_ = 256L * c_occ;
@@ -970,10 +982,12 @@
     if (r.kind != P32_GENERIC) {
         if (in_stats || out_stats) return fail_arg(MSTG_E_UNSUPPORTED, "conv_p32: InstanceNorm folding only in the generic persistent kernel");
         if (r.kind == P32_CO1) return launch_co1(g, st);
+        if (g.out_scale) return fail_arg(MSTG_E_UNSUPPORTED, "conv_p32: the image-stem and packed-head kernels take no output scale");
         if (r.kind == P32_IMG) return launch_p32i(g, r, workspace, workspace_bytes, st);
         if (r.kind == P32_HEAD) return launch_p32d(g, r, workspace, workspace_bytes, st);
         return fail_arg(MSTG_E_UNSUPPORTED, "conv_p32: not a layer of the persistent kernels");
     }
+    if (g.out_scale && (in_stats || out_stats)) return fail_arg(MSTG_E_UNSUPPORTED, "conv_p32: no output scale together with an InstanceNorm fold");
     P32Plan p = r.plan;
     if (!workspace || workspace_bytes < (out_stats ? r.stats_bytes : r.pack_bytes))
         return fail_arg(MSTG_E_WORKSPACE, "conv_p32: workspace too small for the packed filter");
@@ -981,6 +995,7 @@
     a.in_stats = in_stats;
     a.aux = aux;
     a.aux_stats = aux_stats;
+    a.out_scale = g.out_scale;
     a.partial = out_stats ? (float*)((char*)workspace + ((r.pack_bytes + 255) & ~(size_t)255)) : nullptr;
     a.x = g.x; a.y = g.y;
     a.bias = (const float*)workspace;
diff --git a/multi-style-transfer-gan_amd/mstg_hip/csrc/igemm_args.h b/multi-style-transfer-gan_amd/mstg_hip/csrc/igemm_args.h
--- a/multi-style-transfer-gan_amd/mstg_hip/csrc/igemm_args.h
+++ b/multi-style-transfer-gan_amd/mstg_hip/csrc/igemm_args.h
@@ -26,6 +26,7 @@
     int wglob;
     int TH;
     int dpack, tapsx;
+    const float* out_scale;
 };
 
 constexpr int P32_MAX_STEPS = 64;
diff --git a/multi-style-transfer-gan_amd/mstg_hip/ops.py b/multi-style-transfer-gan_amd/mstg_hip/ops.py
--- a/multi-style-transfer-gan_amd/mstg_hip/ops.py
+++ b/multi-style-transfer-gan_amd/mstg_hip/ops.py
@@ -211,22 +211,58 @@
     return (name,) + (fields[1:] if name.startswith(b"conv_p32") else fields)
 
 
-def conv_fwd_raw(d: ConvDesc, x, w, b, y, owners=None):
+def _scaled_name(name: str) -> str:
+    return name.replace(", 0>", ", 3>") if name.startswith("conv_p32_kernel") else name
+
+
+def conv_fwd_raw(d: ConvDesc, x, w, b, y, owners=None, out_scale=None):
     fl, by = _conv_cost(d)
     lib = _lib.load()
     ws, packed = _cached_ws(owners, "fwd", _dkey(d, 0), lib.mstg_conv2d_workspace_bytes(C.byref(d)), x.device)
+    if out_scale is not None:
+        _timed(_scaled_name(_kernel_name(d, 0)), fl, by, lambda: _lib.check(
+            lib.mstg_conv2d_fwd_scaled(C.byref(d), _p(x), _p(w), _p(b), _p(out_scale), _p(y), _p(ws), ws.numel() * 4, packed, _stream()),
+            "mstg_conv2d_fwd_scaled"), _conv_detail("fwd", d))
+        return
     _timed(_kernel_name(d, 0), fl, by, lambda: _lib.check(
         lib.mstg_conv2d_fwd_cached(C.byref(d), _p(x), _p(w), _p(b), _p(y), _p(ws), ws.numel() * 4, packed, _stream()), "mstg_conv2d_fwd"),
         _conv_detail("fwd", d))
 
 
-def conv_dgrad_raw(d: ConvDesc, dy, w, dx, owners=None):
+def conv_dgrad_raw(d: ConvDesc, dy, w, dx, owners=None, out_scale=None):
     fl, by = _conv_cost(d)
     lib = _lib.load()
     ws, packed = _cached_ws(owners, "dgrad", _dkey(d, 1), lib.mstg_conv2d_workspace_bytes(C.byref(d)), dy.device)
+    if out_scale is not None:
+        _timed(_scaled_name(_kernel_name(d, 1)), fl, by, lambda: _lib.check(
+            lib.mstg_conv2d_dgrad_scaled(C.byref(d), _p(dy), _p(w), _p(out_scale), _p(dx), _p(ws), ws.numel() * 4, packed, _stream()),
+            "mstg_conv2d_dgrad_scaled"), _conv_detail("dgrad", d))
+        return
     _timed(_kernel_name(d, 1), fl, by, lambda: _lib.check(
         lib.mstg_conv2d_dgrad_cached(C.byref(d), _p(dy), _p(w), _p(dx), _p(ws), ws.numel() * 4, packed, _stream()), "mstg_conv2d_dgrad"),
         _conv_detail("dgrad", d))
+
+
+_NO_SCALE_KERNELS = (b"igemm_stream_kernel", b"conv_p32i_kernel", b"conv_p32d_kernel")
+
+
+def sn_scale_enabled() -> bool:
+    return os.environ.get("MSTG_SN_SCALE", "1") != "0" and os.environ.get("MSTG_NO_PACK_CACHE", "0") != "1"
+
+
+def sn_scale_route(d: ConvDesc, pass_: int) -> bool:
+    name = _lib.load().mstg_conv2d_kernel_name(C.byref(d), pass_)
+    return bool(name) and not name.startswith(_NO_SCALE_KERNELS)
+
+
+def _sn_raw(w):
+    tag = getattr(w, "_mstg_sn_raw", None)
+    if tag is None or not sn_scale_enabled():
+        return None
+    raw, sigma = tag
+    if not isinstance(raw, torch.nn.Parameter) or raw.shape != w.shape or not raw.is_contiguous() or raw.dtype != torch.float32:
+        return None
+    return raw, sigma
 
 
 def norm_bsums_enabled() -> bool:
@@ -306,18 +342,23 @@
             raise RuntimeError(f"mstg_hip conv: input {H}x{W} too small for kernel {k} (stride {stride}, pad {pad}, dil {dil})")
         y = torch.empty((N, Cout, Ho, Wo) if y_nchw else (N, Ho, Wo, Cout), dtype=torch.float32, device=x.device)
         d = make_desc(N, H, W, Cin, Ho, Wo, Cout, k, stride, pad, dil, transposed, x_nchw, y_nchw, act=act)
-        conv_fwd_raw(d, x, w, b, y, owners=(w, b))
+        sn = _sn_raw(w)
+        if sn is not None and sn_scale_route(d, 0):
+            conv_fwd_raw(d, x, sn[0], b, y, owners=(sn[0], b), out_scale=sn[1])
+        else:
+            conv_fwd_raw(d, x, w, b, y, owners=(w, b))
         ctx.cfg, ctx.dims, ctx.has_bias = cfg, (N, H, W, Cin, Ho, Wo, Cout), b is not None
         ctx.norm_src = getattr(x, "_mstg_norm", None) if not x_nchw else None
+        ctx.sn_scale, ctx.sn_param = (sn[1], sn[0]) if sn is not None else (None, None)
         ctx.prefs = (w, b)
-        ctx.save_for_backward(x, w, y if act != ACT_NONE else None)
+        ctx.save_for_backward(x, w, y if act != ACT_NONE else None, sn[0] if sn is not None else None)
         return y
 
     @staticmethod
     def backward(ctx, dy):
         k, stride, pad, dil, transposed, x_nchw, y_nchw, act = ctx.cfg
         N, H, W, Cin, Ho, Wo, Cout = ctx.dims
-        x, w, y = ctx.saved_tensors
+        x, w, y, w_raw = ctx.saved_tensors
         dy = _req(dy, "conv grad_output")
         if act != ACT_NONE:
             dy = act_bwd_raw(y, dy, act)
@@ -329,6 +370,8 @@
             if src is not None and conv_dgrad_bsums_supported(d):
                 sums = conv_dgrad_bsums_raw(d, dy, w, dx, src[0], src[1], owners=(ctx.prefs[0],))
                 dx._mstg_bsums = (sums, src[2], dx._version)
+            elif w_raw is not None and sn_scale_enabled() and sn_scale_route(d, 1):
+                conv_dgrad_raw(d, dy, w_raw, dx, owners=(ctx.sn_param,), out_scale=ctx.sn_scale)
             else:
                 conv_dgrad_raw(d, dy, w, dx, owners=(ctx.prefs[0],))
         want_db = ctx.has_bias and ctx.needs_input_grad[2]
@@ -390,7 +433,7 @@
         ctx.cfg, ctx.dims, ctx.has_bias = (k, stride, pad, dil, transposed, 0, 0, ACT_NONE), (N, H, W, Cin, Ho, Wo, Cout), b is not None
         ctx.prefs = (w, b)
         ctx.norm_src = getattr(x, "_mstg_norm", None)
-        ctx.save_for_backward(x, w, None)
+        ctx.save_for_backward(x, w, None, None)
         ctx.mark_non_differentiable(stats)
         return y, stats
 
@@ -1156,10 +1199,13 @@
                                                     float(eps), int(bool(training)), _p(ws), ws.numel() * 4, _stream()),
                    "mstg_spectral_norm_group_fwd")
         ctx.n, ctx.dims, ctx.prefs = n, (Ms, Ks), tuple(ws_)
+        SpectralNormGroupFn.last_sigma = sigma
         ctx.set_materialize_grads(False)
         if need:
             ctx.save_for_backward(sigma, *ws_, *u_sv, *v_sv)
         return tuple(outs)
+
+    last_sigma = None
 
     @staticmethod
     def backward(ctx, *dwns):
@@ -1202,7 +1248,10 @@
         outs = SpectralNormGroupFn.apply(eps, part[0].training, len(part), *[getattr(m, nm + "_orig") for m, nm in zip(part, names)],
                                          *[getattr(m, nm + "_u") for m, nm in zip(part, names)],
                                          *[getattr(m, nm + "_v") for m, nm in zip(part, names)])
-        for m, nm, w in zip(part, names, outs):
+        sigma, SpectralNormGroupFn.last_sigma = SpectralNormGroupFn.last_sigma, None
+        for j, (m, nm, w) in enumerate(zip(part, names, outs)):
+            if sigma is not None:
+                w._mstg_sn_raw = (getattr(m, nm + "_orig"), sigma[j:j + 1])
             setattr(m, nm, w)
             m.__dict__["_mstg_sn_fresh"] = True
 
```

New measurement: 1719 images/sec. Within noise of the previous version (-0.0%).
